# fundamentalvision/BEVFormer

Measured on NVIDIA H100. Metric: BEV queries/sec (bevformer_base 200x200x256, 6 cams) fwd+bwd, higher is better.
Workload: dtype bf16

## Files before the change

### bevformer_b200/_lib.py

```python
from __future__ import annotations

import ctypes
import os
import threading

from . import build as _build

_lock = threading.Lock()
_lib = None

c_void_p, c_int, c_int64 = ctypes.c_void_p, ctypes.c_int, ctypes.c_int64

SIGNATURES = {
    "bevf_version": (c_int, []),
    "bevf_last_error": (ctypes.c_char_p, []),
    "bevf_launch_count": (c_int64, []),
    "bevf_msda_forward": (c_int, [c_void_p, c_int, c_void_p, c_void_p, c_void_p, c_void_p,
                                  c_void_p, c_int] + [c_int] * 7 + [c_void_p]),
    "bevf_msda_backward": (c_int, [c_void_p, c_int, c_void_p, c_void_p, c_void_p, c_void_p,
                                   c_void_p, c_int, c_void_p, c_void_p, c_void_p] + [c_int] * 7
                           + [c_void_p]),
    "bevf_msda_rows_forward": (c_int, [c_void_p, c_int, c_void_p, c_void_p, c_void_p, c_void_p,
                                       c_void_p, c_int, c_void_p] + [c_int] * 7 + [c_void_p]),
    "bevf_msda_rows_backward": (c_int, [c_void_p, c_int, c_void_p, c_void_p, c_void_p, c_void_p,
                                        c_void_p, c_int, c_void_p, c_void_p, c_void_p, c_void_p]
                                + [c_int] * 7 + [c_void_p]),
    "bevf_msda_rows_backward_ordered": (c_int, [c_void_p, c_int, c_void_p, c_void_p, c_void_p, c_void_p,
                                                c_void_p, c_int, c_void_p, c_void_p, c_void_p, c_void_p,
                                                c_void_p] + [c_int] * 7 + [c_void_p]),
    "bevf_msda_set_backward_mode": (c_int, [c_int]),
    "bevf_abs_max": (c_int, [c_void_p, c_int, c_int64, c_void_p, c_void_p]),
    "bevf_msda_rows_backward_f16acc": (c_int, [c_void_p, c_int, c_void_p, c_void_p, c_void_p, c_void_p, c_void_p, c_int,
                                               c_void_p, c_void_p, c_void_p, c_void_p, c_void_p, c_void_p] + [c_int] * 7
                                       + [c_void_p]),
    "bevf_gv16_unscale": (c_int, [c_void_p, c_void_p, c_void_p, c_int64, c_void_p]),
    "bevf_msda_rows_backward_mixed": (c_int, [c_void_p, c_int, c_void_p, c_void_p, c_void_p, c_void_p, c_void_p, c_void_p,
                                              c_int, c_void_p, c_void_p, c_void_p, c_int, c_void_p, c_void_p, c_void_p,
                                              c_void_p] + [c_int] * 7 + [c_void_p]),
    "bevf_msda_rows_backward_mixed_dense": (c_int, [c_void_p, c_int, c_void_p, c_void_p, c_void_p, c_void_p, c_void_p,
                                                    c_void_p, c_int, c_void_p, c_void_p, c_void_p, c_int, c_int,
                                                    c_void_p, c_void_p, c_void_p, c_void_p] + [c_int] * 7 + [c_void_p]),
    "bevf_gv_merge": (c_int, [c_void_p, c_void_p, c_void_p, c_void_p, c_int, c_int, c_int, c_int, c_void_p]),
    "bevf_msda_fx_frac_bits": (c_int, [c_int64, c_int, c_int]),
    "bevf_msda_backward_fx": (c_int, [c_void_p, c_int, c_void_p, c_void_p, c_void_p, c_void_p, c_void_p, c_int,
                                      c_void_p, c_void_p, c_int, c_void_p, c_void_p] + [c_int] * 7 + [c_void_p]),
    "bevf_msda_rows_backward_fx": (c_int, [c_void_p, c_int, c_void_p, c_void_p, c_void_p, c_void_p, c_void_p, c_int,
                                           c_void_p, c_void_p, c_int, c_void_p, c_void_p, c_void_p] + [c_int] * 7
                                   + [c_void_p]),
    "bevf_msda_fx_convert": (c_int, [c_void_p, c_void_p, c_int, c_void_p, c_int, c_int, c_int64, c_void_p]),
    "bevf_msda_rows_backward_dense": (c_int, [c_void_p, c_int, c_void_p, c_void_p, c_void_p, c_void_p, c_void_p,
                                              c_void_p, c_int, c_void_p, c_void_p, c_void_p, c_void_p, c_void_p]
                                      + [c_int] * 7 + [c_void_p]),
    "bevf_msda_set_dense_backward": (c_int, [c_int]),
    "bevf_msda_get_dense_backward": (c_int, []),
    "bevf_msda_dense_plan": (c_int, [c_void_p, c_int, c_int, c_int, c_void_p, c_int, c_void_p]),
    "bevf_sca_plan_workspace_ints": (c_int64, [c_int, c_int]),
    "bevf_sca_plan_build": (c_int, [c_void_p] * 10 + [c_int] * 5 + [c_void_p]),
    "bevf_msda_rows_forward_staged": (c_int, [c_void_p, c_int, c_void_p, c_void_p, c_void_p, c_void_p, c_void_p,
                                              c_void_p, c_int, c_void_p] + [c_int] * 7 + [c_void_p]),
    "bevf_sca_prep_forward": (c_int, [c_void_p] * 7 + [c_int] * 8 + [c_void_p]),
    "bevf_sca_prep_backward": (c_int, [c_void_p] * 6 + [c_int] * 8 + [c_void_p]),
    "bevf_tsa_prep_forward": (c_int, [c_void_p] * 5 + [c_int] * 6 + [c_void_p]),
    "bevf_tsa_prep_backward": (c_int, [c_void_p] * 5 + [c_int] * 7 + [c_void_p]),
    "bevf_layernorm_forward": (c_int, [c_void_p] * 4 + [c_int] + [c_void_p] * 5
                               + [c_int64, c_int, ctypes.c_float, ctypes.c_float, ctypes.c_uint64, c_void_p,
                                  c_int, c_void_p]),
    "bevf_layernorm_backward": (c_int, [c_void_p] * 3 + [c_int] + [c_void_p] * 4 + [c_int64]
                                + [c_void_p] * 4
                                + [c_int64, c_int, ctypes.c_float, ctypes.c_uint64, c_void_p, c_int,
                                   c_void_p]),
    "bevf_layernorm_backward_workspace_bytes": (c_int64, [c_int64, c_int]),
    "bevf_layernorm_backward_det": (c_int, [c_void_p] * 3 + [c_int] + [c_void_p] * 4 + [c_int64]
                                    + [c_void_p] * 5 + [c_int64]
                                    + [c_int64, c_int, ctypes.c_float, ctypes.c_uint64, c_void_p, c_int,
                                       c_void_p]),
    "bevf_sca_combine_forward": (c_int, [c_void_p] * 4 + [c_int] * 6 + [c_void_p]),
    "bevf_sca_combine_backward": (c_int, [c_void_p] * 4 + [c_int] * 5 + [c_void_p]),
    "bevf_linear_forward": (c_int, [c_void_p] * 3 + [c_int] + [c_void_p] * 2
                            + [c_int, c_int64, c_int, c_int, c_int, c_void_p]),
    "bevf_flatten_feats": (c_int, [c_void_p] * 4 + [c_int] * 7 + [c_void_p]),
    "bevf_linear_dgrad": (c_int, [c_void_p] * 3 + [c_int64, c_int, c_int, c_void_p]),
    "bevf_linear_dgrad_acc": (c_int, [c_void_p] * 4 + [c_int64, c_int, c_int, c_void_p]),
    "bevf_linear_wgrad": (c_int, [c_void_p] * 4 + [c_int64, c_int, c_int, c_void_p]),
    "bevf_linear_wgrad_workspace_bytes": (c_int64, [c_int64, c_int, c_int]),
    "bevf_linear_wgrad_out": (c_int, [c_void_p] * 4 + [c_int, c_void_p, c_int64, c_int64, c_int, c_int,
                                                      c_void_p]),
    "bevf_sum_tensors": (c_int, [c_void_p, c_int, c_void_p, c_int64, c_int, c_void_p]),
    "bevf_linear_wgrad_into": (c_int, [c_void_p] * 5 + [c_int64, c_int64, c_int, c_int, c_void_p]),
    "bevf_linear_forward_dt": (c_int, [c_void_p] * 3 + [c_int] + [c_void_p] * 2
                               + [c_int, c_int64, c_int, c_int, c_int, c_int, c_void_p]),
    "bevf_linear_dgrad_dt": (c_int, [c_void_p] * 3 + [c_int64, c_int, c_int, c_int, c_void_p]),
    "bevf_linear_dgrad_acc_dt": (c_int, [c_void_p] * 4 + [c_int64, c_int, c_int, c_int, c_void_p]),
    "bevf_linear_wgrad_dt": (c_int, [c_void_p] * 4 + [c_int64, c_int, c_int, c_int, c_void_p]),
    "bevf_linear_wgrad_out_dt": (c_int, [c_void_p] * 4 + [c_int, c_void_p, c_int64, c_int64, c_int, c_int, c_int,
                                                         c_void_p]),
    "bevf_linear_wgrad_into_dt": (c_int, [c_void_p] * 5 + [c_int64, c_int64, c_int, c_int, c_int, c_void_p]),
    "bevf_colsum": (c_int, [c_void_p, c_void_p, c_int64, c_int, c_int, c_void_p]),
    "bevf_colsum_workspace_bytes": (c_int64, [c_int64, c_int]),
    "bevf_colsum_det": (c_int, [c_void_p, c_void_p, c_void_p, c_int64, c_int64, c_int, c_int, c_void_p]),
    "bevf_dropout_inplace": (c_int, [c_void_p, c_int64, ctypes.c_float, ctypes.c_uint64, c_void_p, c_int,
                                     c_void_p]),
    "bevf_relu_dropout_backward": (c_int, [c_void_p, c_void_p, c_void_p, c_int64, ctypes.c_float, c_int,
                                           c_void_p]),
    "bevf_point_sampling": (c_int, [c_void_p, c_void_p, c_void_p, ctypes.c_float, ctypes.c_float,
                                    c_void_p, c_void_p] + [c_int] * 5 + [c_void_p]),
}


def lib_path() -> str:
    return _build.LIB_PATH


def load(build_if_missing: bool = True):
    global _lib
# ... 39 lines not shown
```

### bevformer_b200/csrc/common.cuh

```cuda
#pragma once

#include <cuda_bf16.h>
#include <cuda_fp16.h>
#include <cuda_runtime.h>
#include <stdint.h>

#include <atomic>
#include <cstdio>
#include <string>

#include "../../include/bevformer_b200.h"

namespace bevf {

std::string &last_error();
extern std::atomic<int64_t> g_launches;

inline int fail(const char *fmt, const char *a = "", long long x = 0, long long y = 0) {
    char buf[512];
    snprintf(buf, sizeof(buf), fmt, a, x, y);
    last_error() = buf;
    return 1;
}

inline int check_launch(const char *what) {
    g_launches.fetch_add(1, std::memory_order_relaxed);
    cudaError_t e = cudaPeekAtLastError();
    if (e != cudaSuccess) {
        cudaGetLastError();
        char buf[512];
        snprintf(buf, sizeof(buf), "%s: launch failed: %s", what, cudaGetErrorString(e));
        last_error() = buf;
        return 2;
    }
    return 0;
}

inline bool aligned16(const void *p) { return (reinterpret_cast<uintptr_t>(p) & 15u) == 0; }

inline int device_sms() {
    static int sms = 0;
    if (sms == 0) {
        int dev = 0, n = 0;
        if (cudaGetDevice(&dev) != cudaSuccess ||
            cudaDeviceGetAttribute(&n, cudaDevAttrMultiProcessorCount, dev) != cudaSuccess || n <= 0) {
            cudaGetLastError();
            return 132;
        }
        sms = n;
    }
    return sms;
}

typedef __nv_bfloat16 bf16;

__device__ __forceinline__ float exp_rn(float x) { return (float)exp((double)x); }

__device__ __forceinline__ float bf16_lo(uint32_t u) { return __uint_as_float(u << 16); }
__device__ __forceinline__ float bf16_hi(uint32_t u) { return __uint_as_float(u & 0xffff0000u); }

__device__ __forceinline__ uint32_t pack_bf16x2(float lo, float hi) {
    uint32_t r;
    asm("cvt.rn.bf16x2.f32 %0, %1, %2;" : "=r"(r) : "f"(hi), "f"(lo));
    return r;
}

__device__ __forceinline__ float f16_lo(uint32_t u) { return __half2float(__ushort_as_half((unsigned short)(u & 0xffffu))); }
__device__ __forceinline__ float f16_hi(uint32_t u) { return __half2float(__ushort_as_half((unsigned short)(u >> 16))); }
__device__ __forceinline__ uint32_t pack_f16x2(float lo, float hi) {
    uint32_t r;
    asm("cvt.rn.f16x2.f32 %0, %1, %2;" : "=r"(r) : "f"(hi), "f"(lo));
    return r;
}

template <typename T> struct St16;
template <> struct St16<bf16> {
    __device__ static __forceinline__ float lo(uint32_t u) { return bf16_lo(u); }
    __device__ static __forceinline__ float hi(uint32_t u) { return bf16_hi(u); }
    __device__ static __forceinline__ uint32_t pack(float lo, float hi) { return pack_bf16x2(lo, hi); }
    __device__ static __forceinline__ float to_f(bf16 v) { return __bfloat162float(v); }
    __device__ static __forceinline__ bf16 from_f(float v) { return __float2bfloat16_rn(v); }
};
template <> struct St16<__half> {
    __device__ static __forceinline__ float lo(uint32_t u) { return f16_lo(u); }
    __device__ static __forceinline__ float hi(uint32_t u) { return f16_hi(u); }
    __device__ static __forceinline__ uint32_t pack(float lo, float hi) { return pack_f16x2(lo, hi); }
    __device__ static __forceinline__ float to_f(__half v) { return __half2float(v); }
    __device__ static __forceinline__ __half from_f(float v) { return __float2half_rn(v); }
};

template <typename T> struct Row;
template <> struct Row<float> {
    static constexpr int kVec = 4;
    __device__ static __forceinline__ void load(const float *p, float (&v)[4]) {
        float4 t = __ldg(reinterpret_cast<const float4 *>(p));
        v[0] = t.x; v[1] = t.y; v[2] = t.z; v[3] = t.w;
    }
    __device__ static __forceinline__ void store(float *p, const float (&v)[4]) {
        *reinterpret_cast<float4 *>(p) = make_float4(v[0], v[1], v[2], v[3]);
    }
    __device__ static __forceinline__ float load1(const float *p) { return __ldg(p); }
    __device__ static __forceinline__ void store1(float *p, float v) { *p = v; }
};
template <typename T> struct Row {
    static constexpr int kVec = 8;
    __device__ static __forceinline__ void load(const T *p, float (&v)[8]) {
        uint4 t = __ldg(reinterpret_cast<const uint4 *>(p));
        v[0] = St16<T>::lo(t.x); v[1] = St16<T>::hi(t.x); v[2] = St16<T>::lo(t.y); v[3] = St16<T>::hi(t.y);
        v[4] = St16<T>::lo(t.z); v[5] = St16<T>::hi(t.z); v[6] = St16<T>::lo(t.w); v[7] = St16<T>::hi(t.w);
// ... 72 lines not shown
```

### bevformer_b200/csrc/encoder_ops.cu

```cuda
#include <curand_kernel.h>

#include "common.cuh"

namespace bevf {

constexpr int kEThreads = 256;


__device__ __forceinline__ float warp_sum(float v) {
#pragma unroll
    for (int s = 16; s > 0; s >>= 1) v += __shfl_xor_sync(0xffffffffu, v, s);
    return v;
}

__global__ void __launch_bounds__(kEThreads)
sca_prep_fwd(const float *__restrict__ raw, const float *__restrict__ ref_cam,
             const int *__restrict__ pair_q, const int *__restrict__ pair_cam,
             const int64_t *__restrict__ level_hw, float *__restrict__ loc, float *__restrict__ attn,
             int B, int Nq, int R, int M, int L, int P, int D, int ncam) {
    const long long t = (long long)blockIdx.x * blockDim.x + threadIdx.x;
    const long long total = (long long)B * R * M;
    if (t >= total) return;
    const int m = (int)(t % M);
    const long long br = t / M;
// ... 33 lines not shown

template <typename TO>
__global__ void __launch_bounds__(kEThreads)
sca_prep_bwd(const float *__restrict__ raw, const float *__restrict__ grad_loc,
             const float *__restrict__ grad_attn, const int *__restrict__ pair_of,
             const int64_t *__restrict__ level_hw, TO *__restrict__ d_raw, int B, int Nq, int R,
             int M, int L, int P, int ncam) {
    const long long t = (long long)blockIdx.x * blockDim.x + threadIdx.x;
    const long long total = (long long)B * Nq * M;
    if (t >= total) return;
    const int m = (int)(t % M);
    const long long bq = t / M;
    const int q = (int)(bq % Nq), b = (int)(bq / Nq);
    const int LP = L * P, nout = M * LP * 3;
    const float *lg = raw + bq * nout + (long long)M * LP * 2 + (long long)m * LP;
    TO *d_off = d_raw + bq * nout + (long long)m * LP * 2;
    TO *d_lg = d_raw + bq * nout + (long long)M * LP * 2 + (long long)m * LP;
    int rows[16];
    int n = 0;
    for (int c = 0; c < ncam && c < 16; ++c) {
        const int r = pair_of[(long long)c * Nq + q];
        if (r >= 0) rows[n++] = r;
    }
    float mx = -INFINITY;
    for (int k = 0; k < LP; ++k) mx = fmaxf(mx, lg[k]);
    float sum = 0.f;
    for (int k = 0; k < LP; ++k) sum += exp_rn(lg[k] - mx);
    const float inv = __frcp_rn(sum);
    float dot = 0.f;
    for (int k = 0; k < LP; ++k) {
        float ga = 0.f;
        for (int i = 0; i < n; ++i) ga += grad_attn[(((long long)b * R + rows[i]) * M + m) * LP + k];
        dot += exp_rn(lg[k] - mx) * inv * ga;
    }
    for (int l = 0; l < L; ++l) {
        const float fw = (float)level_hw[2 * l + 1], fh = (float)level_hw[2 * l];
        for (int p = 0; p < P; ++p) {
            const int k = l * P + p;
            float ga = 0.f, gx = 0.f, gy = 0.f;
            for (int i = 0; i < n; ++i) {
                const long long s = (((long long)b * R + rows[i]) * M + m) * LP + k;
                ga += grad_attn[s];
                const float2 g2 = *reinterpret_cast<const float2 *>(grad_loc + 2 * s);
                gx += g2.x; gy += g2.y;
            }
            const float a = exp_rn(lg[k] - mx) * inv;
            st1(d_lg + k, a * (ga - dot));
            st2(d_off + 2 * k, __fdiv_rn(gx, fw), __fdiv_rn(gy, fh));
        }
    }
}


__device__ __forceinline__ float quad_max(float v) {
    v = fmaxf(v, __shfl_xor_sync(0xffffffffu, v, 1));
    return fmaxf(v, __shfl_xor_sync(0xffffffffu, v, 2));
}
__device__ __forceinline__ float quad_sum(float v) {
    v += __shfl_xor_sync(0xffffffffu, v, 1);
    return v + __shfl_xor_sync(0xffffffffu, v, 2);
}
template <int N> __device__ __forceinline__ void ldv(const float *p, float (&v)[N]) {
    if constexpr (N % 4 == 0) {
#pragma unroll
        for (int i = 0; i < N; i += 4) {
            const float4 t = __ldg(reinterpret_cast<const float4 *>(p + i));
            v[i] = t.x; v[i + 1] = t.y; v[i + 2] = t.z; v[i + 3] = t.w;
        }
    } else if constexpr (N % 2 == 0) {
#pragma unroll
        for (int i = 0; i < N; i += 2) {
            const float2 t = __ldg(reinterpret_cast<const float2 *>(p + i));
            v[i] = t.x; v[i + 1] = t.y;
        }
    } else {
#pragma unroll
        for (int i = 0; i < N; ++i) v[i] = __ldg(p + i);
    }
}
template <int N> __device__ __forceinline__ void stv(float *p, const float (&v)[N]) {
    if constexpr (N % 4 == 0) {
#pragma unroll
        for (int i = 0; i < N; i += 4) *reinterpret_cast<float4 *>(p + i) = make_float4(v[i], v[i + 1], v[i + 2], v[i + 3]);
    } else if constexpr (N % 2 == 0) {
#pragma unroll
        for (int i = 0; i < N; i += 2) *reinterpret_cast<float2 *>(p + i) = make_float2(v[i], v[i + 1]);
    } else {
#pragma unroll
        for (int i = 0; i < N; ++i) p[i] = v[i];
    }
}

template <int N, typename T> __device__ __forceinline__ void stv(T *p, const float (&v)[N]) {
    if constexpr (N % 8 == 0) {
#pragma unroll
        for (int i = 0; i < N; i += 8)
            *reinterpret_cast<uint4 *>(p + i) = make_uint4(St16<T>::pack(v[i], v[i + 1]), St16<T>::pack(v[i + 2], v[i + 3]),
                                                           St16<T>::pack(v[i + 4], v[i + 5]), St16<T>::pack(v[i + 6], v[i + 7]));
    } else if constexpr (N % 4 == 0) {
#pragma unroll
        for (int i = 0; i < N; i += 4)
            *reinterpret_cast<uint2 *>(p + i) = make_uint2(St16<T>::pack(v[i], v[i + 1]), St16<T>::pack(v[i + 2], v[i + 3]));
    } else if constexpr (N % 2 == 0) {
#pragma unroll
        for (int i = 0; i < N; i += 2) *reinterpret_cast<uint32_t *>(p + i) = St16<T>::pack(v[i], v[i + 1]);
    } else {
#pragma unroll
        for (int i = 0; i < N; ++i) p[i] = St16<T>::from_f(v[i]);
    }
}

template <int PPL>
__global__ void __launch_bounds__(kEThreads)
sca_prep_fwd_m8(const float *__restrict__ raw, const float *__restrict__ ref_cam,
                const int *__restrict__ pair_q, const int *__restrict__ pair_cam,
                const int64_t *__restrict__ level_hw, float *__restrict__ loc, float *__restrict__ attn,
                int B, int Nq, int R, int L, int P, int D, int pmagic) {
    constexpr int M = 8;
    __shared__ float s_w[16], s_h[16];
    if ((int)threadIdx.x < L) { s_h[threadIdx.x] = (float)level_hw[2 * threadIdx.x]; s_w[threadIdx.x] = (float)level_hw[2 * threadIdx.x + 1]; }
    __syncthreads();
    const int lane = threadIdx.x & 31, m = lane >> 2, sub = lane & 3;
    const long long t = (long long)blockIdx.x * (kEThreads / 32) + (threadIdx.x >> 5);
    if (t >= (long long)B * R) return;
    const int r = (int)(t % R), b = (int)(t / R);
    const int q = __ldg(pair_q + r), cam = __ldg(pair_cam + r);
    if (q < 0) return;
    const int LP = 4 * PPL, k0 = sub * PPL;
    const float *rq = raw + ((long long)b * Nq + q) * (M * LP * 3);
    float lg[PPL], off[2 * PPL];
    ldv<PPL>(rq + M * LP * 2 + m * LP + k0, lg);
    ldv<2 * PPL>(rq + (m * LP + k0) * 2, off);
    float mx = lg[0];
#pragma unroll
    for (int i = 1; i < PPL; ++i) mx = fmaxf(mx, lg[i]);
    mx = quad_max(mx);
    float sum = 0.f;
#pragma unroll
    for (int i = 0; i < PPL; ++i) { lg[i] = exp_rn(lg[i] - mx); sum += lg[i]; }
    const float inv = __frcp_rn(quad_sum(sum));
    const float *rc = ref_cam + (((long long)cam * B + b) * Nq + q) * D * 2;
#pragma unroll
    for (int i = 0; i < PPL; ++i) {
        const int k = k0 + i;
        const int l = (k * pmagic) >> 16;
        const int z = (k - l * P) % D;
        const float2 rf = __ldg(reinterpret_cast<const float2 *>(rc) + z);
        off[2 * i] = rf.x + __fdiv_rn(off[2 * i], s_w[l]);
        off[2 * i + 1] = rf.y + __fdiv_rn(off[2 * i + 1], s_h[l]);
        lg[i] *= inv;
    }
    stv<2 * PPL>(loc + ((t * M + m) * LP + k0) * 2, off);
    stv<PPL>(attn + (t * M + m) * LP + k0, lg);
}

template <int PPL, typename TO>
__global__ void __launch_bounds__(kEThreads)
sca_prep_bwd_m8(const float *__restrict__ raw, const float *__restrict__ grad_loc,
                const float *__restrict__ grad_attn, const int *__restrict__ pair_of,
                const int64_t *__restrict__ level_hw, TO *__restrict__ d_raw, int B, int Nq, int R,
                int L, int P, int ncam, int pmagic) {
    constexpr int M = 8;
    __shared__ float s_w[16], s_h[16];
    if ((int)threadIdx.x < L) { s_h[threadIdx.x] = (float)level_hw[2 * threadIdx.x]; s_w[threadIdx.x] = (float)level_hw[2 * threadIdx.x + 1]; }
    __syncthreads();
    const int lane = threadIdx.x & 31, m = lane >> 2, sub = lane & 3;
    const long long bq = (long long)blockIdx.x * (kEThreads / 32) + (threadIdx.x >> 5);
    if (bq >= (long long)B * Nq) return;
    const int q = (int)(bq % Nq), b = (int)(bq / Nq);
    const int LP = 4 * PPL, k0 = sub * PPL;
    const long long rbase = bq * (M * LP * 3);
    float a[PPL];
    ldv<PPL>(raw + rbase + M * LP * 2 + m * LP + k0, a);
    float mx = a[0];
#pragma unroll
    for (int i = 1; i < PPL; ++i) mx = fmaxf(mx, a[i]);
    mx = quad_max(mx);
    float sum = 0.f;
#pragma unroll
    for (int i = 0; i < PPL; ++i) { a[i] = exp_rn(a[i] - mx); sum += a[i]; }
    const float inv = __frcp_rn(quad_sum(sum));
    float ga[PPL], gl[2 * PPL];
#pragma unroll
    for (int i = 0; i < PPL; ++i) { ga[i] = 0.f; gl[2 * i] = 0.f; gl[2 * i + 1] = 0.f; }
    constexpr int kCamBatch = 8;
    for (int c0 = 0; c0 < ncam; c0 += kCamBatch) {
        int rid[kCamBatch];
#pragma unroll
        for (int c = 0; c < kCamBatch; ++c)
            rid[c] = (c0 + c < ncam) ? __ldg(pair_of + (long long)(c0 + c) * Nq + q) : -1;
#pragma unroll
        for (int c = 0; c < kCamBatch; ++c) {
            if (rid[c] < 0) continue;
            const long long s = (((long long)b * R + rid[c]) * M + m) * LP + k0;
            float t1[PPL], t2[2 * PPL];
            ldv<PPL>(grad_attn + s, t1);
            ldv<2 * PPL>(grad_loc + 2 * s, t2);
#pragma unroll
            for (int i = 0; i < PPL; ++i) { ga[i] += t1[i]; gl[2 * i] += t2[2 * i]; gl[2 * i + 1] += t2[2 * i + 1]; }
        }
    }
    float dot = 0.f;
#pragma unroll
    for (int i = 0; i < PPL; ++i) { a[i] *= inv; dot += a[i] * ga[i]; }
    dot = quad_sum(dot);
#pragma unroll
    for (int i = 0; i < PPL; ++i) {
        const int k = k0 + i;
        const int l = (k * pmagic) >> 16;
        ga[i] = a[i] * (ga[i] - dot);
        gl[2 * i] = __fdiv_rn(gl[2 * i], s_w[l]);
        gl[2 * i + 1] = __fdiv_rn(gl[2 * i + 1], s_h[l]);
    }
    stv<PPL>(d_raw + rbase + M * LP * 2 + m * LP + k0, ga);
    stv<2 * PPL>(d_raw + rbase + (m * LP + k0) * 2, gl);
}

template <typename T>
__global__ void __launch_bounds__(kEThreads)
colsum_kernel(const T *__restrict__ x, float *__restrict__ out, long long rows, int C, int rows_per_cta,
              float *__restrict__ part = nullptr) {
    constexpr int VEC = (sizeof(T) == 2) ? 8 : 4;
// ... 650 lines not shown
            case 2: sca_prep_fwd_m8<2><<<wgrid, kEThreads, 0, st>>>(raw, ref_cam, pair_q, pair_cam, level_hw, loc, attn, B, Nq, R, L, P, D, pmagic); break;
            case 4: sca_prep_fwd_m8<4><<<wgrid, kEThreads, 0, st>>>(raw, ref_cam, pair_q, pair_cam, level_hw, loc, attn, B, Nq, R, L, P, D, pmagic); break;
            case 8: sca_prep_fwd_m8<8><<<wgrid, kEThreads, 0, st>>>(raw, ref_cam, pair_q, pair_cam, level_hw, loc, attn, B, Nq, R, L, P, D, pmagic); break;
            default: sca_prep_fwd_m8<16><<<wgrid, kEThreads, 0, st>>>(raw, ref_cam, pair_q, pair_cam, level_hw, loc, attn, B, Nq, R, L, P, D, pmagic); break;
        }
    } else {
        sca_prep_fwd<<<blocks_for(total, kEThreads), kEThreads, 0, st>>>(
            raw, ref_cam, pair_q, pair_cam, level_hw, loc, attn, B, Nq, R, M, L, P, D, ncam);
    }
    return check_launch(who);
}

template <typename TO>
static int sca_prep_backward_t(const char *who, const float *raw, const float *grad_loc, const float *grad_attn,
                               const int32_t *pair_of, const int64_t *level_hw, TO *d_raw, int B, int Nq,
                               int R, int M, int L, int P, int ncam, cudaStream_t st) {
    const long long total = (long long)B * Nq * M;
    const int LP = L * P, pmagic = (65536 + P - 1) / P;
    const unsigned wgrid = blocks_for((long long)B * Nq, kEThreads / 32);
    if (M == 8 && L <= 16 && LP * P < 65536 && (LP == 4 || LP == 8 || LP == 16 || LP == 32 || LP == 64)) {
#define BEVF_SCA_CASE(N) sca_prep_bwd_m8<N, TO><<<wgrid, kEThreads, 0, st>>>(raw, grad_loc, grad_attn, pair_of, level_hw, d_raw, B, Nq, R, L, P, ncam, pmagic)
        switch (LP / 4) {
            case 1: BEVF_SCA_CASE(1); break;
            case 2: BEVF_SCA_CASE(2); break;
            case 4: BEVF_SCA_CASE(4); break;
            case 8: BEVF_SCA_CASE(8); break;
            default: BEVF_SCA_CASE(16); break;
        }
#undef BEVF_SCA_CASE
    } else {
        sca_prep_bwd<TO><<<blocks_for(total, kEThreads), kEThreads, 0, st>>>(
            raw, grad_loc, grad_attn, pair_of, level_hw, d_raw, B, Nq, R, M, L, P, ncam);
    }
    return check_launch(who);
}

extern "C" int bevf_sca_prep_backward(const float *raw, const float *grad_loc,
                                      const float *grad_attn, const int32_t *pair_of,
                                      const int64_t *level_hw, void *d_raw, int out_dtype, int B, int Nq,
                                      int R, int M, int L, int P, int ncam, void *stream) {
    const char *who = "bevf_sca_prep_backward";
    BEVF_REQUIRE(B >= 0 && Nq >= 0 && R >= 0 && M > 0 && L > 0 && P > 0 && ncam > 0 && ncam <= 16, who, "bad dimension (ncam <= 16)");
    BEVF_REQUIRE(out_dtype == BEVF_DTYPE_F32 || out_dtype == BEVF_DTYPE_BF16 || out_dtype == BEVF_DTYPE_F16, who, "unsupported dtype code");
    if ((long long)B * Nq * M == 0) return 0;
    BEVF_REQUIRE(raw && pair_of && level_hw && d_raw && (R == 0 || (grad_loc && grad_attn)), who, "null pointer argument");
    cudaStream_t st = (cudaStream_t)stream;
    if (out_dtype == BEVF_DTYPE_BF16)
        return sca_prep_backward_t<bf16>(who, raw, grad_loc, grad_attn, pair_of, level_hw, (bf16 *)d_raw, B, Nq, R, M, L, P, ncam, st);
    if (out_dtype == BEVF_DTYPE_F16)
        return sca_prep_backward_t<__half>(who, raw, grad_loc, grad_attn, pair_of, level_hw, (__half *)d_raw, B, Nq, R, M, L, P, ncam, st);
    return sca_prep_backward_t<float>(who, raw, grad_loc, grad_attn, pair_of, level_hw, (float *)d_raw, B, Nq, R, M, L, P, ncam, st);
}

extern "C" int bevf_tsa_prep_forward(const float *raw, const float *ref2d, const int64_t *level_hw,
                                     float *loc, float *attn, int B, int Nq, int M, int L, int P,
                                     int interleave, void *stream) {
    const char *who = "bevf_tsa_prep_forward";
    BEVF_REQUIRE(B >= 0 && Nq >= 0 && M > 0 && L > 0 && P > 0, who, "bad dimension");
    const long long total = (long long)B * Nq * M * 2;
    if (total == 0) return 0;
    BEVF_REQUIRE(raw && ref2d && level_hw && loc && attn, who, "null pointer argument");
    if (!launch_tsa_prep_m8<false, float>(raw, ref2d, nullptr, nullptr, level_hw, loc, attn, nullptr, B, Nq, M, L, P,
                                   interleave, (cudaStream_t)stream)) {
        if (interleave) return fail("%s: interleaved rows need num_heads == 8 and L*P in {2,4,8,16,32}", who);
        tsa_prep_fwd<<<blocks_for(total, kEThreads), kEThreads, 0, (cudaStream_t)stream>>>(
            raw, ref2d, level_hw, loc, attn, B, Nq, M, L, P);
    }
    return check_launch(who);
}

template <typename TO>
static int tsa_prep_backward_t(const char *who, const float *raw, const float *grad_loc, const float *grad_attn,
                               const int64_t *level_hw, TO *d_raw, int B, int Nq, int M, int L, int P,
                               int interleave, cudaStream_t st) {
    const long long total = (long long)B * Nq * M * 2;
    if (!launch_tsa_prep_m8<true, TO>(raw, nullptr, grad_loc, grad_attn, level_hw, nullptr, nullptr, d_raw, B, Nq, M,
                                      L, P, interleave, st)) {
        if (interleave) return fail("%s: interleaved rows need num_heads == 8 and L*P in {2,4,8,16,32}", who);
        tsa_prep_bwd<TO><<<blocks_for(total, kEThreads), kEThreads, 0, st>>>(
            raw, grad_loc, grad_attn, level_hw, d_raw, B, Nq, M, L, P);
    }
    return check_launch(who);
}

extern "C" int bevf_tsa_prep_backward(const float *raw, const float *grad_loc,
                                      const float *grad_attn, const int64_t *level_hw, void *d_raw,
                                      int out_dtype, int B, int Nq, int M, int L, int P, int interleave,
                                      void *stream) {
    const char *who = "bevf_tsa_prep_backward";
    BEVF_REQUIRE(B >= 0 && Nq >= 0 && M > 0 && L > 0 && P > 0, who, "bad dimension");
    BEVF_REQUIRE(out_dtype == BEVF_DTYPE_F32 || out_dtype == BEVF_DTYPE_BF16 || out_dtype == BEVF_DTYPE_F16, who, "unsupported dtype code");
    if ((long long)B * Nq * M * 2 == 0) return 0;
    BEVF_REQUIRE(raw && grad_loc && grad_attn && level_hw && d_raw, who, "null pointer argument");
    cudaStream_t st = (cudaStream_t)stream;
    if (out_dtype == BEVF_DTYPE_BF16)
        return tsa_prep_backward_t<bf16>(who, raw, grad_loc, grad_attn, level_hw, (bf16 *)d_raw, B, Nq, M, L, P, interleave, st);
    if (out_dtype == BEVF_DTYPE_F16)
        return tsa_prep_backward_t<__half>(who, raw, grad_loc, grad_attn, level_hw, (__half *)d_raw, B, Nq, M, L, P, interleave, st);
    return tsa_prep_backward_t<float>(who, raw, grad_loc, grad_attn, level_hw, (float *)d_raw, B, Nq, M, L, P, interleave, st);
}

template <typename T, typename TP>
static int ln_fwd_t(const char *who, const void *x, const void *res, const void *gamma, const void *beta,
                    const void *pos, void *y, void *y2, float *mean, float *rstd, long long rows, int C,
                    float eps, float drop_p, unsigned long long seed, const unsigned long long *sb,
                    cudaStream_t st) {
// ... 360 lines not shown
```

### bevformer_b200/csrc/msda.cu

```cuda
#include <cuda_fp16.h>

#include <cstdlib>
#include <cstring>
#include <mutex>
#include <type_traits>

#include "msda_common.cuh"

namespace bevf {

template <typename T, typename TO>
__global__ void __launch_bounds__(kThreads)
msda_fwd_d32(const T *__restrict__ value, const int64_t *__restrict__ level_hw,
             const int64_t *__restrict__ level_start, const float *__restrict__ loc,
             const float *__restrict__ attn, TO *__restrict__ out,
             const int *__restrict__ row_map, int S, int M, int Q, int L, int P, int magic,
             int iters, long long rows) {
    constexpr int VEC = Vec<T>::N, LANES = 32 / VEC, G = 32 / LANES;
    constexpr bool kHalf = std::is_same<T, bf16>::value;
    __shared__ LevelTab tab;
    load_level_tab(level_hw, level_start, L, M * 32, tab);

    const int lane = threadIdx.x & 31, warp = threadIdx.x >> 5;
    const int sub = lane % LANES, grp = lane / LANES;
    for (int it = 0; it < iters; ++it) {
    long long row = (((long long)blockIdx.x * (kThreads / 32) + warp) * iters + it) * G + grp;
    if (row - grp >= rows) break;
    bool live = row < rows;
    if (!live) row = rows - 1;
    const int m = (int)(row % M);
    int b = value_map_of(row_map, row, M, Q);
    if (b < 0) { live = false; b = 0; }
    const int pix = M * 32;
    const int LP = L * P;
    const T *vbase = value + ((long long)b * S * M + m) * 32 + sub * VEC;
    const float2 *locp = reinterpret_cast<const float2 *>(loc) + row * LP;
    const float *attp = attn + row * LP;

    float acc[VEC];
#pragma unroll
    for (int i = 0; i < VEC; ++i) acc[i] = 0.f;

    for (int s0 = 0; s0 < LP; s0 += LANES) {
        const int sm = s0 + sub;
        int enc = 0;
        float w00 = 0.f, w01 = 0.f, w10 = 0.f, w11 = 0.f;
        bool valid = false;
        if (sm < LP && live) {
            const int l = level_of(sm, magic);
            const float2 xy = __ldg(locp + sm);
            const float a = __ldg(attp + sm);
            const Corner c = make_corner(xy.x, xy.y, tab.h[l], tab.w[l]);
            enc = (c.pidx * pix) | c.dx | (c.dy << 1);
            valid = c.valid;
            w00 = c.w00 * a; w01 = c.w01 * a; w10 = c.w10 * a; w11 = c.w11 * a;
        }
        uint32_t wa = 0, wb = 0;
        if constexpr (kHalf) { wa = pack_bf16x2(w00, w01); wb = pack_bf16x2(w10, w11); }
        const unsigned vm = __ballot_sync(0xffffffffu, valid);
#pragma unroll
        for (int j = 0; j < LANES; ++j) {
            if (s0 + j >= LP) break;
            if (!(vm & (GroupMask<LANES>::kBits << j))) continue;
            const int src = grp * LANES + j;
            const unsigned e = (unsigned)__shfl_sync(0xffffffffu, enc, src);
            const int l = level_of(s0 + j, magic);
            const T *vl = vbase + tab.lofs[l];
            const unsigned o00 = e & ~3u;
            const unsigned o01 = o00 + ((e & 1u) ? (unsigned)pix : 0u);
            const unsigned oy = (e & 2u) ? (unsigned)tab.rs[l] : 0u;
            Vec<T> v00, v01, v10, v11;
            v00.load(vl + o00); v01.load(vl + o01); v10.load(vl + (o00 + oy)); v11.load(vl + (o01 + oy));
            if constexpr (kHalf) {
                const uint32_t qa = __shfl_sync(0xffffffffu, wa, src);
                const uint32_t qb = __shfl_sync(0xffffffffu, wb, src);
                unsigned short h00, h01, h10, h11;
                split16(qa, h00, h01);
                split16(qb, h10, h11);
                v00.axpy_h(h00, acc); v01.axpy_h(h01, acc); v10.axpy_h(h10, acc); v11.axpy_h(h11, acc);
            } else {
                const float q00 = __shfl_sync(0xffffffffu, w00, src);
                const float q01 = __shfl_sync(0xffffffffu, w01, src);
                const float q10 = __shfl_sync(0xffffffffu, w10, src);
                const float q11 = __shfl_sync(0xffffffffu, w11, src);
                v00.axpy(q00, acc); v01.axpy(q01, acc); v10.axpy(q10, acc); v11.axpy(q11, acc);
            }
        }
    }
    if (live) store_vec<TO, VEC>(out + row * 32 + sub * VEC, acc);
    }
}

template <typename T, typename TG, bool kScatter, typename TV = float>
__global__ void __launch_bounds__(kThreads)
msda_bwd_d32(const T *__restrict__ value, const int64_t *__restrict__ level_hw,
             const int64_t *__restrict__ level_start, const float *__restrict__ loc,
             const float *__restrict__ attn, const TG *__restrict__ grad_out,
             TV *__restrict__ grad_value, float *__restrict__ grad_loc,
             float *__restrict__ grad_attn, const int *__restrict__ row_map, int S, int M, int Q,
             int L, int P, int magic, int iters, long long rows, unsigned red_skip,
             const __grid_constant__ HostLevels host_levels, const unsigned *__restrict__ gv_amax = nullptr,
             __half *__restrict__ gv16 = nullptr, unsigned gv16_mask = 0u, int side_start = 0, int S_side = 0,
             const unsigned *__restrict__ fx_bounds = nullptr, int fx_bits = 0) {
    constexpr int VEC = Vec<T>::N, LANES = 32 / VEC, G = 32 / LANES;
    constexpr bool kHalfDot = std::is_same<T, bf16>::value && std::is_same<TG, bf16>::value;
    __shared__ LevelTab tab;
    __shared__ unsigned s_skip;
    if (threadIdx.x == 0)
        s_skip = (red_skip && host_levels.h[0] > 0 && !host_levels_match(host_levels, level_hw, level_start, L)) ? 0u : red_skip;
    __shared__ unsigned s_mask16;
    if (gv16 != nullptr && threadIdx.x == 32) {
        unsigned mk = 0;
        for (int l = 0; l < L; ++l) {
            const long long a = level_start[l], e = a + level_hw[2 * l] * level_hw[2 * l + 1];
            if (e <= side_start) mk |= 1u << l;
            else if (a < side_start) __trap();
        }
        s_mask16 = mk;
    }
    load_level_tab(level_hw, level_start, L, M * 32, tab);
    red_skip = s_skip;
    if (gv16 != nullptr) gv16_mask = s_mask16;
    const float gv_sc = gv_amax ? gv16_scale(__ldg(gv_amax)) : 1.f;
    constexpr bool kGvFx = sizeof(TV) == 8;
    double fx_sc = 0.0;
    if constexpr (kGvFx) {
        const unsigned ba = __ldg(fx_bounds), bg = __ldg(fx_bounds + 1);
        if (fx_bounds_finite(ba, bg)) fx_sc = fx_pow2(fx_bits - fx_exponent(ba, bg));
        else red_skip = ~0u;
    }

    const int lane = threadIdx.x & 31, warp = threadIdx.x >> 5;
    const int sub = lane % LANES, grp = lane / LANES;
    for (int it = 0; it < iters; ++it) {
    long long row = (((long long)blockIdx.x * (kThreads / 32) + warp) * iters + it) * G + grp;
    if (row - grp >= rows) break;
    bool live = row < rows;
    if (!live) row = rows - 1;
    const int m = (int)(row % M);
    int b = value_map_of(row_map, row, M, Q);
    if (b < 0) { live = false; b = 0; }
    const int pix = M * 32;
    const int LP = L * P;
    const long long voff = ((long long)b * S * M + m) * 32 + sub * VEC;
    const float2 *locp = reinterpret_cast<const float2 *>(loc) + row * LP;
    const float *attp = attn + row * LP;

    float g[VEC];
    load_vec<TG, VEC>(grad_out + row * 32 + sub * VEC, g);
    uint4 gh = make_uint4(0, 0, 0, 0);
    if constexpr (kHalfDot)
        gh = __ldg(reinterpret_cast<const uint4 *>(grad_out + row * 32 + sub * VEC));
    float gx[kGvFx ? VEC : 1];
    if constexpr (kGvFx) {
#pragma unroll
        for (int k = 0; k < VEC; ++k) gx[k] = Row<TG>::load1(grad_out + row * 32 + k * LANES + sub);
    }
    constexpr bool kGvHalf = sizeof(TV) == 2;
    static_assert(!kGvHalf || VEC == 8, "fp16 grad_value needs bf16 value rows (8 channels per lane)");
    constexpr bool kPaired = (VEC == 8) && kScatter && !kGvHalf && !kGvFx;
    const bool hi = kPaired && (grp & 4);
    const long long vrow = voff - sub * VEC;
    long long vrow_a = vrow, vrow_b = vrow;
    float gra[4], grb[4];
    if constexpr (!kPaired) {
        gra[0] = g[0]; gra[1] = g[1]; gra[2] = g[2]; gra[3] = g[3];
        grb[0] = grb[1] = grb[2] = grb[3] = 0.f;
        (void)vrow_a; (void)vrow_b;
    } else {
        const long long row_p = __shfl_xor_sync(0xffffffffu, row, 16);
        const long long vrow_p = __shfl_xor_sync(0xffffffffu, vrow, 16);
        const int chan = (hi ? 16 : 0) + 4 * sub;
        const long long row_a = hi ? row_p : row, row_b = hi ? row : row_p;
        vrow_a = (hi ? vrow_p : vrow) + chan;
        vrow_b = (hi ? vrow : vrow_p) + chan;
        if (gv16 != nullptr) {
            const int b_p = __shfl_xor_sync(0xffffffffu, b, 16);
            const int b_a = hi ? b_p : b, b_b = hi ? b : b_p;
            vrow_a -= ((long long)b_a * (S - S_side) + side_start) * pix;
            vrow_b -= ((long long)b_b * (S - S_side) + side_start) * pix;
        }
        load_vec<TG, 4>(grad_out + row_a * 32 + chan, gra);
        load_vec<TG, 4>(grad_out + row_b * 32 + chan, grb);
    }

    for (int s0 = 0; s0 < LP; s0 += LANES) {
        const int sm = s0 + sub;
        Corner c;
        c.x0 = c.y0 = 0;
        c.pidx = 0; c.dx = c.dy = 0; c.w00 = c.w01 = c.w10 = c.w11 = 0.f; c.lx = c.ly = 0.f;
        c.f00 = c.f01 = c.f10 = c.f11 = 0.f; c.valid = false;
        float a = 0.f;
        int Hm = 1, Wm = 1;
        const bool mine = sm < LP && live;
        if (mine) {
            const int l = level_of(sm, magic);
            Hm = tab.h[l]; Wm = tab.w[l];
            const float2 xy = __ldg(locp + sm);
            a = __ldg(attp + sm);
            c = make_corner(xy.x, xy.y, Hm, Wm);
        }
        const int enc = (c.pidx * pix) | c.dx | (c.dy << 1);
        const float wa00 = c.w00 * a, wa01 = c.w01 * a, wa10 = c.w10 * a, wa11 = c.w11 * a;
        const unsigned vm = __ballot_sync(0xffffffffu, c.valid);
        float d[LANES][4];
#pragma unroll
        for (int j = 0; j < LANES; ++j) { d[j][0] = d[j][1] = d[j][2] = d[j][3] = 0.f; }
#pragma unroll
        for (int j = 0; j < LANES; ++j) {
            if (s0 + j >= LP) break;
            if (!(vm & (GroupMask<LANES>::kBits << j))) continue;
            const int src = grp * LANES + j;
            const int e = __shfl_sync(0xffffffffu, enc, src);
            const float q00 = __shfl_sync(0xffffffffu, wa00, src);
            const float q01 = __shfl_sync(0xffffffffu, wa01, src);
            const float q10 = __shfl_sync(0xffffffffu, wa10, src);
            const float q11 = __shfl_sync(0xffffffffu, wa11, src);
            const int l = level_of(s0 + j, magic);
            const long long o00 = voff + tab.lofs[l] + (long long)((unsigned)e & ~3u);
            const int ox = (e & 1) ? pix : 0, oy = (e & 2) ? tab.rs[l] : 0;
            const T *vp = value + o00;
            Vec<T> v00, v01, v10, v11;
            v00.load(vp); v01.load(vp + ox); v10.load(vp + oy); v11.load(vp + (oy + ox));
            if constexpr (kHalfDot) {
                d[j][0] = v00.dot_h(gh); d[j][1] = v01.dot_h(gh);
                d[j][2] = v10.dot_h(gh); d[j][3] = v11.dot_h(gh);
            } else {
                d[j][0] = v00.dot(g); d[j][1] = v01.dot(g); d[j][2] = v10.dot(g); d[j][3] = v11.dot(g);
            }
            if constexpr (!kScatter) {
            } else if ((red_skip >> l) & 1u) {
            } else if constexpr (kGvFx) {
                long long *gp = reinterpret_cast<long long *>(grad_value) + (o00 - sub * VEC) + sub;
                auto redfx = [&](long long *p, float q) {
#pragma unroll
                    for (int k = 0; k < VEC; ++k) red_add_fx(p + k * LANES, q, gx[k], fx_sc);
                };
                if (q00 != 0.f) redfx(gp, q00);
                if (q01 != 0.f) redfx(gp + ox, q01);
                if (q10 != 0.f) redfx(gp + oy, q10);
                if (q11 != 0.f) redfx(gp + oy + ox, q11);
            } else if constexpr (kGvHalf) {
                TV *gp = grad_value + o00;
                auto red8 = [&](TV *p, float q) {
                    q *= gv_sc;
                    red_add_v4_f16x2(p, pack_f16x2(q * g[0], q * g[1]), pack_f16x2(q * g[2], q * g[3]),
                                     pack_f16x2(q * g[4], q * g[5]), pack_f16x2(q * g[6], q * g[7]));
                };
                if (q00 != 0.f) red8(gp, q00);
                if (q01 != 0.f) red8(gp + ox, q01);
                if (q10 != 0.f) red8(gp + oy, q10);
                if (q11 != 0.f) red8(gp + oy + ox, q11);
// ... 16 lines not shown
                if (q11 != 0.f) red8(gp + oy + ox, q11);
            } else {
                const int ep = __shfl_xor_sync(0xffffffffu, e, 16);
                const float p00 = __shfl_xor_sync(0xffffffffu, q00, 16);
                const float p01 = __shfl_xor_sync(0xffffffffu, q01, 16);
                const float p10 = __shfl_xor_sync(0xffffffffu, q10, 16);
                const float p11 = __shfl_xor_sync(0xffffffffu, q11, 16);
                const int oxp = (ep & 1) ? pix : 0, oyp = (ep & 2) ? tab.rs[l] : 0;
                {
                    const int ea = hi ? ep : e;
                    const int xa = hi ? oxp : ox, ya = hi ? oyp : oy;
                    const float a00 = hi ? p00 : q00, a01 = hi ? p01 : q01, a10 = hi ? p10 : q10,
                                a11 = hi ? p11 : q11;
                    float *gp = grad_value + vrow_a + tab.lofs[l] + (long long)((unsigned)ea & ~3u);
                    if (a00 != 0.f) red_add_v4(gp, a00 * gra[0], a00 * gra[1], a00 * gra[2], a00 * gra[3]);
                    if (a01 != 0.f) red_add_v4(gp + xa, a01 * gra[0], a01 * gra[1], a01 * gra[2], a01 * gra[3]);
                    if (a10 != 0.f) red_add_v4(gp + ya, a10 * gra[0], a10 * gra[1], a10 * gra[2], a10 * gra[3]);
                    if (a11 != 0.f) red_add_v4(gp + ya + xa, a11 * gra[0], a11 * gra[1], a11 * gra[2], a11 * gra[3]);
                }
                {
                    const int eb = hi ? e : ep;
                    const int xb = hi ? ox : oxp, yb = hi ? oy : oyp;
                    const float b00 = hi ? q00 : p00, b01 = hi ? q01 : p01, b10 = hi ? q10 : p10,
                                b11 = hi ? q11 : p11;
                    float *gp = grad_value + vrow_b + tab.lofs[l] + (long long)((unsigned)eb & ~3u);
                    if (b00 != 0.f) red_add_v4(gp, b00 * grb[0], b00 * grb[1], b00 * grb[2], b00 * grb[3]);
                    if (b01 != 0.f) red_add_v4(gp + xb, b01 * grb[0], b01 * grb[1], b01 * grb[2], b01 * grb[3]);
                    if (b10 != 0.f) red_add_v4(gp + yb, b10 * grb[0], b10 * grb[1], b10 * grb[2], b10 * grb[3]);
                    if (b11 != 0.f) red_add_v4(gp + yb + xb, b11 * grb[0], b11 * grb[1], b11 * grb[2], b11 * grb[3]);
                }
            }
        }
#pragma unroll
        for (int step = LANES / 2; step > 0; step >>= 1) {
            const bool upper = (sub & step) != 0;
#pragma unroll
            for (int j = 0; j < step; ++j) {
#pragma unroll
                for (int k = 0; k < 4; ++k) {
                    const float keep = upper ? d[j + step][k] : d[j][k];
                    const float send = upper ? d[j][k] : d[j + step][k];
                    d[j][k] = keep + __shfl_xor_sync(0xffffffffu, send, step);
                }
            }
        }
        if (mine) {
            const float hx = 1.f - c.lx, hy = 1.f - c.ly;
            const float d00 = c.f00 * d[0][0], d01 = c.f01 * d[0][1], d10 = c.f10 * d[0][2],
                        d11 = c.f11 * d[0][3];
            const float ga = hy * (hx * d00 + c.lx * d01) + c.ly * (hx * d10 + c.lx * d11);
            const float gx = a * (hy * (d01 - d00) + c.ly * (d11 - d10));
            const float gy = a * (hx * (d10 - d00) + c.lx * (d11 - d01));
            const long long si = row * LP + sm;
            grad_attn[si] = ga;
            reinterpret_cast<float2 *>(grad_loc)[si] = make_float2((float)Wm * gx, (float)Hm * gy);
        }
    }
    }
}


}
#include "msda_splat.cuh"
namespace bevf {

template <typename T, typename TO>
__global__ void __launch_bounds__(kThreads)
msda_fwd_generic(const T *__restrict__ value, const int64_t *__restrict__ level_hw,
                 const int64_t *__restrict__ level_start, const float *__restrict__ loc,
                 const float *__restrict__ attn, TO *__restrict__ out,
                 const int *__restrict__ row_map, int S, int M, int D, int Q, int L, int P,
                 long long rows) {
    __shared__ int s_h[kMaxLevels], s_w[kMaxLevels], s_start[kMaxLevels];
    load_levels(level_hw, level_start, L, s_h, s_w, s_start);
    const int lane = threadIdx.x & 31;
    const long long row = (long long)blockIdx.x * (kThreads / 32) + (threadIdx.x >> 5);
    if (row >= rows) return;
    const int m = (int)(row % M);
    const int b = value_map_of(row_map, row, M, Q);
    if (b < 0) return;
    const long long pix = (long long)M * D;
    for (int c0 = lane; c0 < D; c0 += 32) {
        float acc = 0.f;
        for (int l = 0; l < L; ++l) {
            const int H = s_h[l], W = s_w[l];
            const T *vl = value + ((long long)b * S + s_start[l]) * pix + (long long)m * D + c0;
            for (int p = 0; p < P; ++p) {
                const long long si = row * L * P + l * P + p;
                const Corner c = make_corner(loc[2 * si], loc[2 * si + 1], H, W);
                const float a = attn[si];
                const T *p00 = vl + c.pidx * pix;
                const long long ox = c.dx ? pix : 0, oy = c.dy ? W * pix : 0;
                acc += a * (c.w00 * Row<T>::load1(p00) + c.w01 * Row<T>::load1(p00 + ox) +
                            c.w10 * Row<T>::load1(p00 + oy) + c.w11 * Row<T>::load1(p00 + oy + ox));
            }
        }
        Row<TO>::store1(out + row * D + c0, acc);
    }
}

template <typename T, typename TG, typename TV = float>
__global__ void __launch_bounds__(kThreads)
msda_bwd_generic(const T *__restrict__ value, const int64_t *__restrict__ level_hw,
                 const int64_t *__restrict__ level_start, const float *__restrict__ loc,
                 const float *__restrict__ attn, const TG *__restrict__ grad_out,
                 TV *__restrict__ grad_value, float *__restrict__ grad_loc,
                 float *__restrict__ grad_attn, const int *__restrict__ row_map, int S, int M,
                 int D, int Q, int L, int P, long long rows,
                 const unsigned *__restrict__ fx_bounds = nullptr, int fx_bits = 0) {
// ... 37 lines not shown
                        if (c.w00 != 0.f) red_add_fx(grad_value + i00 + c0, c.w00 * a, gc, fx_sc);
                        if (c.w01 != 0.f) red_add_fx(grad_value + i01 + c0, c.w01 * a, gc, fx_sc);
                        if (c.w10 != 0.f) red_add_fx(grad_value + i10 + c0, c.w10 * a, gc, fx_sc);
                        if (c.w11 != 0.f) red_add_fx(grad_value + i11 + c0, c.w11 * a, gc, fx_sc);
                    }
                } else {
                    if (c.w00 != 0.f) atomicAdd(grad_value + i00 + c0, c.w00 * t);
                    if (c.w01 != 0.f) atomicAdd(grad_value + i01 + c0, c.w01 * t);
                    if (c.w10 != 0.f) atomicAdd(grad_value + i10 + c0, c.w10 * t);
                    if (c.w11 != 0.f) atomicAdd(grad_value + i11 + c0, c.w11 * t);
                }
                ga += gc * (hy * (hx * v00 + c.lx * v01) + c.ly * (hx * v10 + c.lx * v11));
                gx += t * (hy * (v01 - v00) + c.ly * (v11 - v10));
                gy += t * (hx * (v10 - v00) + c.lx * (v11 - v01));
            }
#pragma unroll
            for (int s = 16; s > 0; s >>= 1) {
                ga += __shfl_xor_sync(0xffffffffu, ga, s);
                gx += __shfl_xor_sync(0xffffffffu, gx, s);
                gy += __shfl_xor_sync(0xffffffffu, gy, s);
            }
            if (lane == 0) {
                grad_attn[si] = ga;
                grad_loc[2 * si] = (float)W * gx;
                grad_loc[2 * si + 1] = (float)H * gy;
            }
        }
    }
}

static int pick_iters(long long rows, int G) {
    static int forced = -1;
    if (forced < 0) {
        const char *e = getenv("BEVF_MSDA_ITERS");
        forced = e ? atoi(e) : 0;
    }
    (void)rows; (void)G;
    return forced > 0 ? forced : 1;
}

static int check_dims(const char *who, int B, int S, int M, int D, int Q, int L, int P) {
    if (B < 0 || S < 0 || M <= 0 || D <= 0 || Q < 0 || L <= 0 || P <= 0)
        return fail("%s: negative or zero dimension", who);
    if (L > kMaxLevels) return fail("%s: at most 16 levels are supported (got %lld)", who, L);
    if ((long long)S * M * D >= (1ll << 31))
        return fail("%s: one batch item of value exceeds 2^31 elements", who);
    if ((long long)L * P * P >= 65536) return fail("%s: num_levels * num_points^2 must be < 65536", who);
    return 0;
}

template <typename T, typename TO>
static int launch_fwd(const char *who, const void *value, const int64_t *hw, const int64_t *ls,
                      const float *loc, const float *attn, void *out, const int *row_map, int S,
                      int M, int D, int Q, int L, int P, long long rows, cudaStream_t st) {
    if (D == 32) {
        constexpr int G = Vec<T>::N;
        const int iters = pick_iters(rows, G);
        const long long per_block = (long long)(kThreads / 32) * G * iters;
        const unsigned grid = (unsigned)((rows + per_block - 1) / per_block);
        msda_fwd_d32<T, TO><<<grid, kThreads, 0, st>>>((const T *)value, hw, ls, loc, attn, (TO *)out,
                                                       row_map, S, M, Q, L, P, (65536 + P - 1) / P, iters,
                                                       rows);
    } else {
        const unsigned grid = (unsigned)((rows + kThreads / 32 - 1) / (kThreads / 32));
        msda_fwd_generic<T, TO><<<grid, kThreads, 0, st>>>((const T *)value, hw, ls, loc, attn,
                                                           (TO *)out, row_map, S, M, D, Q, L, P, rows);
    }
    return check_launch(who);
}

static std::atomic<int> g_bwd_mode{-1};
static int bwd_split_enabled() {
    int v = g_bwd_mode.load(std::memory_order_relaxed);
    if (v < 0) {
        const char *e = getenv("BEVF_MSDA_BWD");
        v = (e && e[0] == 's') ? 1 : 0;
        g_bwd_mode.store(v, std::memory_order_relaxed);
    }
    return v;
}
static unsigned splat_direct_mask() {
    static long v = -1;
    if (v < 0) {
        const char *e = getenv("BEVF_SPLAT_DIRECT");
        v = e ? strtol(e, nullptr, 0) : 0;
    }
    return (unsigned)v;
}

int dense_coarse_backward(const char *who, const int64_t *hw_dev, const int64_t *ls_dev, const int32_t *hw_host,
                          const float *loc, const float *attn, const void *grad_out, float *grad_value,
                          const int32_t *map_range, int NB, int S, int M, int L, int P, cudaStream_t st,
                          unsigned *handled, HostLevels *host_levels, int first_level, unsigned need_mask,
                          int gv_S, int gv_base);

static cudaStream_t g_side_stream = nullptr;
constexpr int kSideEvents = 64;
static cudaEvent_t g_side_events[kSideEvents];
static std::atomic<unsigned> g_side_ev_next{0};

template <typename TG, int kM>
static int launch_splat_km(const char *who, const float *loc, const float *attn, const void *go, float *gv,
                           const int *row_map, const int *order, const int64_t *hw, const int64_t *ls,
                           int S, int M, int Q, int L, int P, long long pairs, unsigned level_mask,
                           cudaStream_t st) {
    static bool attr_done = false;
    if (!attr_done) {
        if (cudaFuncSetAttribute(msda_bwd_splat_d32<TG, kM>, cudaFuncAttributeMaxDynamicSharedMemorySize,
                                 (int)splat_smem_bytes(kSplatMaxHeads, sizeof(TG))) != cudaSuccess) {
            cudaGetLastError();
            return fail("%s: cannot reserve shared memory for the splat kernel", who);
        }
        attr_done = true;
    }
    const unsigned grid = (unsigned)((pairs + kSplatG - 1) / kSplatG);
    msda_bwd_splat_d32<TG, kM><<<grid, 32 * M, splat_smem_bytes(M, sizeof(TG)), st>>>(
        loc, attn, (const TG *)go, gv, row_map, order, hw, ls, S, M, Q, L, P, pairs, splat_direct_mask(),
        level_mask);
    return check_launch(who);
}

template <typename TG>
static int launch_splat(const char *who, const float *loc, const float *attn, const void *go, float *gv,
                        const int *row_map, const int *order, const int64_t *hw, const int64_t *ls,
                        int S, int M, int Q, int L, int P, long long pairs, unsigned level_mask,
                        cudaStream_t st) {
    if constexpr (std::is_same<TG, __half>::value) {
        return fail("%s: the splat kernel takes fp32 or bf16 grad_out", who);
    } else {
        if (M == 8)
            return launch_splat_km<TG, 8>(who, loc, attn, go, gv, row_map, order, hw, ls, S, M, Q, L, P, pairs,
                                          level_mask, st);
        return launch_splat_km<TG, 0>(who, loc, attn, go, gv, row_map, order, hw, ls, S, M, Q, L, P, pairs,
                                      level_mask, st);
    }
}

struct MixedGv {
    const unsigned *amax = nullptr;
    __half *gv16 = nullptr;
    unsigned mask = 0;
    int side_start = 0, S_side = 0;
};

struct FxGv {
    const unsigned *bounds = nullptr;
    int frac_bits = 0;
};

template <typename T, typename TG>
static int launch_bwd(const char *who, const void *value, const int64_t *hw, const int64_t *ls,
                      const float *loc, const float *attn, const void *go, float *gv, float *gl,
                      float *ga, const int *row_map, const int *order, int S, int M, int D, int Q,
                      int L, int P, long long rows, cudaStream_t st, unsigned done_levels = 0,
                      const HostLevels *host_levels = nullptr, bool gv_f16 = false,
                      const MixedGv *mixed = nullptr, const FxGv *fx = nullptr) {
    HostLevels hl;
    if (host_levels) hl = *host_levels; else memset(&hl, 0, sizeof(hl));
    if (fx) {
        long long *gfx = reinterpret_cast<long long *>(gv);
        if (D == 32) {
            constexpr int G = Vec<T>::N;
            const int iters = pick_iters(rows, G);
            const long long per_block = (long long)(kThreads / 32) * G * iters;
            const unsigned grid = (unsigned)((rows + per_block - 1) / per_block);
            msda_bwd_d32<T, TG, true, long long><<<grid, kThreads, 0, st>>>(
                (const T *)value, hw, ls, loc, attn, (const TG *)go, gfx, gl, ga, row_map, S, M, Q, L, P,
                (65536 + P - 1) / P, iters, rows, 0u, hl, nullptr, nullptr, 0u, 0, 0, fx->bounds, fx->frac_bits);
        } else {
            const unsigned grid = (unsigned)((rows + kThreads / 32 - 1) / (kThreads / 32));
            msda_bwd_generic<T, TG, long long><<<grid, kThreads, 0, st>>>(
                (const T *)value, hw, ls, loc, attn, (const TG *)go, gfx, gl, ga, row_map, S, M, D, Q, L, P, rows,
                fx->bounds, fx->frac_bits);
        }
        return check_launch(who);
    }
    if (gv_f16) {
        if constexpr (std::is_same<T, bf16>::value) {
            if (D != 32) return fail("%s: fp16 grad_value needs head_dim 32", who);
            constexpr int G = Vec<T>::N;
            const int iters = pick_iters(rows, G);
            const long long per_block = (long long)(kThreads / 32) * G * iters;
            const unsigned grid = (unsigned)((rows + per_block - 1) / per_block);
            msda_bwd_d32<T, TG, true, __half><<<grid, kThreads, 0, st>>>((const T *)value, hw, ls, loc, attn, (const TG *)go,
                                                                       reinterpret_cast<__half *>(gv), gl, ga, row_map, S, M,
                                                                       Q, L, P, (65536 + P - 1) / P, iters, rows, 0u, hl,
                                                                       mixed ? mixed->amax : nullptr);
            return check_launch(who);
        } else {
            return fail("%s: fp16 grad_value needs a bf16 value tensor", who);
        }
    }
    if (mixed && mixed->gv16) {
        if constexpr (std::is_same<T, bf16>::value) {
            if (D != 32) return fail("%s: mixed accumulation needs head_dim 32", who);
            constexpr int G = Vec<T>::N;
            const int iters = pick_iters(rows, G);
            const long long per_block = (long long)(kThreads / 32) * G * iters;
            const unsigned grid = (unsigned)((rows + per_block - 1) / per_block);
            msda_bwd_d32<T, TG, true><<<grid, kThreads, 0, st>>>((const T *)value, hw, ls, loc, attn, (const TG *)go, gv, gl, ga,
                                                               row_map, S, M, Q, L, P, (65536 + P - 1) / P, iters, rows,
                                                               done_levels, hl, mixed->amax, mixed->gv16, mixed->mask, mixed->side_start,
                                                               mixed->S_side);
            return check_launch(who);
        } else {
            return fail("%s: mixed accumulation needs a bf16 value tensor", who);
        }
    }
    if (D == 32) {
        constexpr int G = Vec<T>::N;
        const int iters = pick_iters(rows, G);
        const long long per_block = (long long)(kThreads / 32) * G * iters;
        const unsigned grid = (unsigned)((rows + per_block - 1) / per_block);
        const int mode = done_levels ? 0 : bwd_split_enabled();
        if (mode != 0 && std::is_same<T, __half>::value)
            return fail("%s: the split / hybrid backward modes take fp32 or bf16 only (fp16 needs mode 0)", who);
        const bool can_split = M <= kSplatMaxHeads && S * (long long)M * 32 < (1ll << 31);
        if (mode == 1 && can_split) {
            if (int e = launch_splat<TG>(who, loc, attn, go, gv, row_map, order, hw, ls, S, M, Q, L, P,
                                         rows / M, 0xffffffffu, st))
                return e;
            msda_bwd_d32<T, TG, false><<<grid, kThreads, 0, st>>>((const T *)value, hw, ls, loc, attn,
                                                                  (const TG *)go, gv, gl, ga, row_map, S, M,
                                                                  Q, L, P, (65536 + P - 1) / P, iters, rows, 0u, hl);
        } else if (mode == 2 && can_split && L >= 2 && g_side_stream) {
            unsigned coarse = 0;
            for (int l = L / 2; l < L; ++l) coarse |= 1u << l;
            cudaEvent_t fork = g_side_events[g_side_ev_next.fetch_add(1) % kSideEvents];
            cudaEvent_t join = g_side_events[g_side_ev_next.fetch_add(1) % kSideEvents];
            cudaEventRecord(fork, st);
            cudaStreamWaitEvent(g_side_stream, fork, 0);
            if (int e = launch_splat<TG>(who, loc, attn, go, gv, row_map, order, hw, ls, S, M, Q, L, P,
                                         rows / M, coarse, g_side_stream))
                return e;
            cudaEventRecord(join, g_side_stream);
            msda_bwd_d32<T, TG, true><<<grid, kThreads, 0, st>>>((const T *)value, hw, ls, loc, attn,
                                                                 (const TG *)go, gv, gl, ga, row_map, S, M,
                                                                 Q, L, P, (65536 + P - 1) / P, iters, rows, coarse, hl);
            cudaStreamWaitEvent(st, join, 0);
        } else {
            msda_bwd_d32<T, TG, true><<<grid, kThreads, 0, st>>>((const T *)value, hw, ls, loc, attn,
                                                                 (const TG *)go, gv, gl, ga, row_map, S, M,
                                                                 Q, L, P, (65536 + P - 1) / P, iters, rows, done_levels, hl);
        }
    } else {
        const unsigned grid = (unsigned)((rows + kThreads / 32 - 1) / (kThreads / 32));
        msda_bwd_generic<T, TG><<<grid, kThreads, 0, st>>>((const T *)value, hw, ls, loc, attn,
                                                           (const TG *)go, gv, gl, ga, row_map, S, M,
                                                           D, Q, L, P, rows);
    }
    return check_launch(who);
}

static int msda_forward_impl(const char *who, const void *value, int value_dtype,
                             const int64_t *level_hw, const int64_t *level_start, const float *loc,
                             const float *attn, void *out, int out_dtype, const int *row_map, int B,
                             int S, int M, int D, int Q, int L, int P, void *stream) {
    if (int e = check_dims(who, B, S, M, D, Q, L, P)) return e;
    const long long rows = (row_map ? 1ll : (long long)B) * Q * M;
    if (rows == 0) return 0;
    if (!value || !level_hw || !level_start || !loc || !attn || !out)
        return fail("%s: null pointer argument", who);
    if (!aligned16(value) || !aligned16(loc) || !aligned16(attn) || !aligned16(out))
        return fail("%s: device pointers must be 16-byte aligned", who);
    cudaStream_t st = (cudaStream_t)stream;
    if (value_dtype == BEVF_DTYPE_F16) {
        if (out_dtype == BEVF_DTYPE_F16) return launch_fwd<__half, __half>(who, value, level_hw, level_start, loc, attn, out, row_map, S, M, D, Q, L, P, rows, st);
        if (out_dtype == BEVF_DTYPE_F32) return launch_fwd<__half, float>(who, value, level_hw, level_start, loc, attn, out, row_map, S, M, D, Q, L, P, rows, st);
        return fail("%s: fp16 value needs an fp16 or fp32 output", who);
    }
    const bool vb = value_dtype == BEVF_DTYPE_BF16, ob = out_dtype == BEVF_DTYPE_BF16;
    if ((value_dtype != BEVF_DTYPE_F32 && !vb) || (out_dtype != BEVF_DTYPE_F32 && !ob))
        return fail("%s: unsupported dtype code", who);
    if (!vb && !ob) return launch_fwd<float, float>(who, value, level_hw, level_start, loc, attn, out, row_map, S, M, D, Q, L, P, rows, st);
    if (vb && ob) return launch_fwd<bf16, bf16>(who, value, level_hw, level_start, loc, attn, out, row_map, S, M, D, Q, L, P, rows, st);
    if (vb && !ob) return launch_fwd<bf16, float>(who, value, level_hw, level_start, loc, attn, out, row_map, S, M, D, Q, L, P, rows, st);
    return fail("%s: fp32 value with bf16 output is not supported", who);
}

static int msda_backward_impl(const char *who, const void *value, int value_dtype,
                              const int64_t *level_hw, const int64_t *level_start, const float *loc,
                              const float *attn, const void *grad_out, int grad_out_dtype,
                              float *grad_value, float *grad_loc, float *grad_attn,
                              const int *row_map, const int *order, int B, int S, int M, int D, int Q,
                              int L, int P, void *stream, unsigned done_levels = 0,
                              const HostLevels *host_levels = nullptr, bool gv_f16 = false,
                              const MixedGv *mixed = nullptr, const FxGv *fx = nullptr) {
    if (int e = check_dims(who, B, S, M, D, Q, L, P)) return e;
    const long long rows = (row_map ? 1ll : (long long)B) * Q * M;
    if (rows == 0) return 0;
    if (!value || !level_hw || !level_start || !loc || !attn || !grad_out || !grad_value ||
        !grad_loc || !grad_attn)
        return fail("%s: null pointer argument", who);
    if (!aligned16(value) || !aligned16(loc) || !aligned16(attn) || !aligned16(grad_out) ||
        !aligned16(grad_value) || !aligned16(grad_loc) || !aligned16(grad_attn))
        return fail("%s: device pointers must be 16-byte aligned", who);
    cudaStream_t st = (cudaStream_t)stream;
    if (value_dtype == BEVF_DTYPE_F16) {
        if (grad_out_dtype == BEVF_DTYPE_F16) return launch_bwd<__half, __half>(who, value, level_hw, level_start, loc, attn, grad_out, grad_value, grad_loc, grad_attn, row_map, order, S, M, D, Q, L, P, rows, st, done_levels, host_levels, gv_f16, mixed, fx);
        if (grad_out_dtype == BEVF_DTYPE_F32) return launch_bwd<__half, float>(who, value, level_hw, level_start, loc, attn, grad_out, grad_value, grad_loc, grad_attn, row_map, order, S, M, D, Q, L, P, rows, st, done_levels, host_levels, gv_f16, mixed, fx);
        return fail("%s: fp16 value needs an fp16 or fp32 grad_out", who);
    }
    const bool vb = value_dtype == BEVF_DTYPE_BF16, gb = grad_out_dtype == BEVF_DTYPE_BF16;
    if ((value_dtype != BEVF_DTYPE_F32 && !vb) || (grad_out_dtype != BEVF_DTYPE_F32 && !gb))
        return fail("%s: unsupported dtype code", who);
    if (!vb && !gb) return launch_bwd<float, float>(who, value, level_hw, level_start, loc, attn, grad_out, grad_value, grad_loc, grad_attn, row_map, order, S, M, D, Q, L, P, rows, st, done_levels, host_levels, gv_f16, mixed, fx);
    if (vb && gb) return launch_bwd<bf16, bf16>(who, value, level_hw, level_start, loc, attn, grad_out, grad_value, grad_loc, grad_attn, row_map, order, S, M, D, Q, L, P, rows, st, done_levels, host_levels, gv_f16, mixed, fx);
    if (vb && !gb) return launch_bwd<bf16, float>(who, value, level_hw, level_start, loc, attn, grad_out, grad_value, grad_loc, grad_attn, row_map, order, S, M, D, Q, L, P, rows, st, done_levels, host_levels, gv_f16, mixed, fx);
    return fail("%s: fp32 value with bf16 grad_out is not supported", who);
}

}

using namespace bevf;

extern "C" int bevf_msda_forward(const void *value, int value_dtype, const int64_t *level_hw,
                                 const int64_t *level_start, const float *loc, const float *attn,
                                 void *out, int out_dtype, int B, int S, int M, int D, int Q, int L,
                                 int P, void *stream) {
    return msda_forward_impl("bevf_msda_forward", value, value_dtype, level_hw, level_start, loc,
                             attn, out, out_dtype, nullptr, B, S, M, D, Q, L, P, stream);
}

extern "C" int bevf_msda_backward(const void *value, int value_dtype, const int64_t *level_hw,
                                  const int64_t *level_start, const float *loc, const float *attn,
                                  const void *grad_out, int grad_out_dtype, float *grad_value,
                                  float *grad_loc, float *grad_attn, int B, int S, int M, int D,
                                  int Q, int L, int P, void *stream) {
    return msda_backward_impl("bevf_msda_backward", value, value_dtype, level_hw, level_start, loc,
                              attn, grad_out, grad_out_dtype, grad_value, grad_loc, grad_attn,
                              nullptr, nullptr, B, S, M, D, Q, L, P, stream);
}

extern "C" int bevf_msda_rows_forward(const void *value, int value_dtype, const int64_t *level_hw,
                                      const int64_t *level_start, const float *loc,
                                      const float *attn, void *out, int out_dtype,
                                      const int32_t *row_map, int B, int S, int M, int D, int R,
                                      int L, int P, void *stream) {
    if (!row_map && R > 0) return fail("%s: row_map is null", "bevf_msda_rows_forward");
    return msda_forward_impl("bevf_msda_rows_forward", value, value_dtype, level_hw, level_start,
                             loc, attn, out, out_dtype, row_map, B, S, M, D, R, L, P, stream);
}

extern "C" int bevf_msda_rows_backward(const void *value, int value_dtype, const int64_t *level_hw,
                                       const int64_t *level_start, const float *loc,
                                       const float *attn, const void *grad_out, int grad_out_dtype,
                                       float *grad_value, float *grad_loc, float *grad_attn,
                                       const int32_t *row_map, int B, int S, int M, int D, int R,
                                       int L, int P, void *stream) {
    if (!row_map && R > 0) return fail("%s: row_map is null", "bevf_msda_rows_backward");
// ... 28 lines not shown
    cudaStream_t s = nullptr;
    if (cudaStreamCreateWithFlags(&s, cudaStreamNonBlocking) != cudaSuccess) {
        cudaGetLastError();
        return fail("%s: cannot create the second stream", who);
    }
    for (int i = 0; i < kSideEvents; ++i) cudaEventCreateWithFlags(&g_side_events[i], cudaEventDisableTiming);
    g_side_stream = s;
    return 0;
}

extern "C" int bevf_msda_set_dense_backward(int mode) {
    if (mode < -1 || mode > 2)
        return fail("%s: mode must be -1 (library default), 0 (off), 1 (same stream) or 2 (second stream)",
                    "bevf_msda_set_dense_backward");
    if (mode == 2)
        if (int e = ensure_side_stream("bevf_msda_set_dense_backward")) return e;
    g_dense_mode.store(mode, std::memory_order_relaxed);
    return 0;
}

extern "C" int bevf_msda_get_dense_backward(void) { return mixed_dense_mode(); }

extern "C" int bevf_msda_rows_backward_dense(const void *value, int value_dtype, const int64_t *level_hw,
                                             const int64_t *level_start, const int32_t *level_hw_host,
                                             const float *loc, const float *attn, const void *grad_out,
                                             int grad_out_dtype, float *grad_value, float *grad_loc,
                                             float *grad_attn, const int32_t *row_map, const int32_t *map_range,
                                             int B, int S, int M, int D, int R, int L, int P, void *stream) {
    const char *who = "bevf_msda_rows_backward_dense";
    if (!row_map && R > 0) return fail("%s: row_map is null", who);
    if (int e = check_dims(who, B, S, M, D, R, L, P)) return e;
    if (R == 0) return 0;
    if (!level_hw_host || !map_range || !level_hw || !level_start || !loc || !attn || !grad_out || !grad_value)
        return fail("%s: null pointer argument", who);
    cudaStream_t st = (cudaStream_t)stream;
    unsigned handled = 0;
    HostLevels hl;
    memset(&hl, 0, sizeof(hl));
    const int mode = dense_setting() < 0 ? 0 : dense_setting();
    cudaEvent_t join = nullptr;
    if (value_dtype == BEVF_DTYPE_F16 || grad_out_dtype == BEVF_DTYPE_F16)
        return fail("%s: fp32 or bf16 only (fp16 runs on bevf_msda_rows_backward)", who);
    if (mode != 0 && D == 32 && grad_out_dtype == BEVF_DTYPE_BF16 && aligned16(loc) && aligned16(attn) &&
        aligned16(grad_out) && aligned16(grad_value)) {
        cudaStream_t ds = st;
        if (mode == 2 && g_side_stream) {
            cudaEvent_t fork = g_side_events[g_side_ev_next.fetch_add(1) % kSideEvents];
            join = g_side_events[g_side_ev_next.fetch_add(1) % kSideEvents];
            cudaEventRecord(fork, st);
            cudaStreamWaitEvent(g_side_stream, fork, 0);
            ds = g_side_stream;
        }
        const int e = dense_coarse_backward(who, level_hw, level_start, level_hw_host, loc, attn, grad_out, grad_value,
                                            map_range, B, S, M, L, P, ds, &handled, &hl, 0, 0u, S, 0);
        if (join) cudaEventRecord(join, g_side_stream);
        if (e) {
            if (join) cudaStreamWaitEvent(st, join, 0);
            return e;
        }
    }
    const int e = msda_backward_impl(who, value, value_dtype, level_hw, level_start, loc, attn, grad_out,
                                     grad_out_dtype, grad_value, grad_loc, grad_attn, row_map, nullptr, B, S, M, D,
                                     R, L, P, stream, handled, &hl);
    if (join) cudaStreamWaitEvent(st, join, 0);
    return e;
}

extern "C" int bevf_msda_rows_backward_f16acc(const void *value, int value_dtype, const int64_t *level_hw,
                                              const int64_t *level_start, const float *loc, const float *attn,
                                              const void *grad_out, int grad_out_dtype, void *grad_value_f16,
                                              const uint32_t *amax_bits, float *grad_loc, float *grad_attn,
                                              const int32_t *row_map, const int32_t *group_order, int B, int S,
                                              int M, int D, int R, int L, int P, void *stream) {
    const char *who = "bevf_msda_rows_backward_f16acc";
    if (!row_map && R > 0) return fail("%s: row_map is null", who);
    if (!grad_value_f16 || !amax_bits) return fail("%s: null pointer argument", who);
    MixedGv mx;
    mx.amax = amax_bits;
    return msda_backward_impl(who, value, value_dtype, level_hw, level_start, loc, attn, grad_out, grad_out_dtype,
                              reinterpret_cast<float *>(grad_value_f16), grad_loc, grad_attn, row_map, group_order, B, S,
                              M, D, R, L, P, stream, 0u, nullptr, true, &mx);
}

static int rows_backward_mixed_impl(const char *who, const void *value, int value_dtype, const int64_t *level_hw,
                                    const int64_t *level_start, const int32_t *level_hw_host, const float *loc,
                                    const float *attn, const void *grad_out, int grad_out_dtype,
                                    void *grad_value_fine_f16, float *grad_value_side, const uint32_t *amax_bits,
                                    int num_f16_levels, int first_dense_level, float *grad_loc, float *grad_attn,
                                    const int32_t *row_map, const int32_t *group_order, const int32_t *map_range,
                                    int B, int S, int M, int D, int R, int L, int P, void *stream) {
    if (!row_map && R > 0) return fail("%s: row_map is null", who);
    if (!level_hw_host || !grad_value_fine_f16 || !grad_value_side || !amax_bits)
        return fail("%s: null pointer argument", who);
    if (L <= 1 || L > kMaxLevels || num_f16_levels < 1 || num_f16_levels >= L)
        return fail("%s: num_f16_levels must be in [1, L - 1]", who);
    if (map_range && (first_dense_level < num_f16_levels || first_dense_level >= L))
        return fail("%s: first_dense_level must be in [num_f16_levels, L - 1]", who);
    if (value_dtype != BEVF_DTYPE_BF16 || D != 32) return fail("%s: needs a bf16 value tensor and head_dim 32", who);
    if (!aligned16(grad_value_fine_f16) || !aligned16(grad_value_side))
        return fail("%s: device pointers must be 16-byte aligned", who);
    HostLevels hl;
    memset(&hl, 0, sizeof(hl));
    long long start = 0;
    for (int l = 0; l < L; ++l) {
        const int h = level_hw_host[2 * l], w = level_hw_host[2 * l + 1];
        if (h <= 0 || w <= 0 || h >= 32768 || w >= 32768) return fail("%s: bad host level shape", who);
        hl.h[l] = h; hl.w[l] = w; hl.start[l] = (int)start;
        start += (long long)h * w;
    }
    if (start != S) return fail("%s: host level shapes do not add up to S (%lld vs %lld)", who, start, S);
    MixedGv mx;
    mx.amax = amax_bits;
    mx.gv16 = reinterpret_cast<__half *>(grad_value_fine_f16);
    mx.mask = (1u << num_f16_levels) - 1u;
    mx.side_start = hl.start[num_f16_levels];
    mx.S_side = S - mx.side_start;
    cudaStream_t st = (cudaStream_t)stream;
    unsigned dense_levels = 0;
    cudaEvent_t join = nullptr;
    const int mode = map_range ? mixed_dense_mode() : 0;
    if (mode != 0 && R > 0 && grad_out_dtype == BEVF_DTYPE_BF16 && aligned16(loc) && aligned16(attn) &&
        aligned16(grad_out)) {
        cudaStream_t ds = st;
        if (mode == 2 && !g_side_stream) {
            cudaStreamCaptureStatus cs = cudaStreamCaptureStatusActive;
            if (cudaStreamIsCapturing(st, &cs) != cudaSuccess) cudaGetLastError();
            else if (cs == cudaStreamCaptureStatusNone && ensure_side_stream(who) != 0) cudaGetLastError();
        }
        if (mode == 2 && g_side_stream) {
            cudaEvent_t fork = g_side_events[g_side_ev_next.fetch_add(1) % kSideEvents];
            join = g_side_events[g_side_ev_next.fetch_add(1) % kSideEvents];
            cudaEventRecord(fork, st);
            cudaStreamWaitEvent(g_side_stream, fork, 0);
            ds = g_side_stream;
        }
        const unsigned suffix = ((1u << L) - 1u) & ~((1u << first_dense_level) - 1u);
        HostLevels dhl;
        const int e = dense_coarse_backward(who, level_hw, level_start, level_hw_host, loc, attn, grad_out,
                                            grad_value_side, map_range, B, S, M, L, P, ds, &dense_levels, &dhl,
                                            first_dense_level, suffix, mx.S_side, mx.side_start);
        if (join) cudaEventRecord(join, g_side_stream);
        if (e) {
            if (join) cudaStreamWaitEvent(st, join, 0);
            return e;
        }
    }
    const int e = msda_backward_impl(who, value, value_dtype, level_hw, level_start, loc, attn, grad_out, grad_out_dtype,
                                     grad_value_side, grad_loc, grad_attn, row_map, group_order, B, S, M, D, R, L, P,
                                     stream, dense_levels, &hl, false, &mx);
    if (join) cudaStreamWaitEvent(st, join, 0);
    return e;
}

extern "C" int bevf_msda_rows_backward_mixed(const void *value, int value_dtype, const int64_t *level_hw,
                                             const int64_t *level_start, const int32_t *level_hw_host,
                                             const float *loc, const float *attn, const void *grad_out,
                                             int grad_out_dtype, void *grad_value_fine_f16, float *grad_value_side,
                                             const uint32_t *amax_bits, int num_f16_levels, float *grad_loc,
                                             float *grad_attn, const int32_t *row_map, const int32_t *group_order,
                                             int B, int S, int M, int D, int R, int L, int P, void *stream) {
    return rows_backward_mixed_impl("bevf_msda_rows_backward_mixed", value, value_dtype, level_hw, level_start,
                                    level_hw_host, loc, attn, grad_out, grad_out_dtype, grad_value_fine_f16,
                                    grad_value_side, amax_bits, num_f16_levels, L, grad_loc, grad_attn, row_map,
                                    group_order, nullptr, B, S, M, D, R, L, P, stream);
}

extern "C" int bevf_msda_rows_backward_mixed_dense(const void *value, int value_dtype, const int64_t *level_hw,
                                                   const int64_t *level_start, const int32_t *level_hw_host,
                                                   const float *loc, const float *attn, const void *grad_out,
                                                   int grad_out_dtype, void *grad_value_fine_f16,
                                                   float *grad_value_side, const uint32_t *amax_bits,
                                                   int num_f16_levels, int first_dense_level, float *grad_loc,
                                                   float *grad_attn, const int32_t *row_map, const int32_t *map_range,
                                                   int B, int S, int M, int D, int R, int L, int P, void *stream) {
    const char *who = "bevf_msda_rows_backward_mixed_dense";
    if (!map_range) return fail("%s: null pointer argument", who);
    return rows_backward_mixed_impl(who, value, value_dtype, level_hw, level_start, level_hw_host, loc, attn, grad_out,
                                    grad_out_dtype, grad_value_fine_f16, grad_value_side, amax_bits, num_f16_levels,
                                    first_dense_level, grad_loc, grad_attn, row_map, nullptr, map_range, B, S, M, D, R,
                                    L, P, stream);
}

namespace bevf {
int fx_bounds_launch(const char *who, const float *attn, const void *grad_out, int grad_out_dtype,
                     const int32_t *row_map, long long qrows, int M, int D, int L, int P, uint32_t *bounds,
                     cudaStream_t st);

static int msda_backward_fx_impl(const char *who, const void *value, int value_dtype, const int64_t *level_hw,
                                 const int64_t *level_start, const float *loc, const float *attn, const void *grad_out,
                                 int grad_out_dtype, int64_t *grad_value_fx, uint32_t *bounds, int frac_bits,
                                 float *grad_loc, float *grad_attn, const int32_t *row_map, int B, int S, int M, int D,
                                 int Q, int L, int P, void *stream) {
    if (int e = check_dims(who, B, S, M, D, Q, L, P)) return e;
    const long long qrows = (row_map ? 1ll : (long long)B) * Q;
    if (qrows == 0) return 0;
    if (!bounds || !grad_value_fx || !attn || !grad_out) return fail("%s: null pointer argument", who);
    const int kmax = bevf_msda_fx_frac_bits(Q, L, P);
    if (frac_bits < 0 || frac_bits > kmax)
        return fail("%s: frac_bits must be in [0, %lld] for this launch (bevf_msda_fx_frac_bits)", who, kmax);
    cudaStream_t st = (cudaStream_t)stream;
    if (int e = fx_bounds_launch(who, attn, grad_out, grad_out_dtype, row_map, qrows, M, D, L, P, bounds, st)) return e;
    FxGv fx;
    fx.bounds = bounds;
    fx.frac_bits = frac_bits;
    return msda_backward_impl(who, value, value_dtype, level_hw, level_start, loc, attn, grad_out, grad_out_dtype,
                              reinterpret_cast<float *>(grad_value_fx), grad_loc, grad_attn, row_map, nullptr, B, S, M,
                              D, Q, L, P, stream, 0u, nullptr, false, nullptr, &fx);
}
}

extern "C" int bevf_msda_backward_fx(const void *value, int value_dtype, const int64_t *level_hw,
                                     const int64_t *level_start, const float *loc, const float *attn,
                                     const void *grad_out, int grad_out_dtype, int64_t *grad_value_fx,
                                     uint32_t *bounds, int frac_bits, float *grad_loc, float *grad_attn, int B, int S,
                                     int M, int D, int Q, int L, int P, void *stream) {
    return msda_backward_fx_impl("bevf_msda_backward_fx", value, value_dtype, level_hw, level_start, loc, attn, grad_out,
                                 grad_out_dtype, grad_value_fx, bounds, frac_bits, grad_loc, grad_attn, nullptr, B, S, M,
                                 D, Q, L, P, stream);
}

extern "C" int bevf_msda_rows_backward_fx(const void *value, int value_dtype, const int64_t *level_hw,
                                          const int64_t *level_start, const float *loc, const float *attn,
                                          const void *grad_out, int grad_out_dtype, int64_t *grad_value_fx,
                                          uint32_t *bounds, int frac_bits, float *grad_loc, float *grad_attn,
                                          const int32_t *row_map, int B, int S, int M, int D, int R, int L, int P,
                                          void *stream) {
    if (!row_map && R > 0) return fail("%s: row_map is null", "bevf_msda_rows_backward_fx");
    return msda_backward_fx_impl("bevf_msda_rows_backward_fx", value, value_dtype, level_hw, level_start, loc, attn,
                                 grad_out, grad_out_dtype, grad_value_fx, bounds, frac_bits, grad_loc, grad_attn, row_map,
                                 B, S, M, D, R, L, P, stream);
}

extern "C" int bevf_msda_set_backward_mode(int mode) {
// ... 27 lines not shown
```

### bevformer_b200/csrc/msda_common.cuh

```cuda
#pragma once

#include "common.cuh"

namespace bevf {

constexpr int kMaxLevels = 16;
constexpr int kThreads = 256;

struct Corner {
    int x0, y0;
    int pidx;
    int dx, dy;
    float w00, w01, w10, w11;
    float lx, ly;
    float f00, f01, f10, f11;
    bool valid;
};

__device__ __forceinline__ Corner make_corner(float locx, float locy, int H, int W) {
    Corner c;
    float x = __fadd_rn(__fmul_rn(locx, (float)W), -0.5f), y = __fadd_rn(__fmul_rn(locy, (float)H), -0.5f);
    c.valid = (x > -1.f) && (y > -1.f) && (x < (float)W) && (y < (float)H);
    if (!c.valid) { x = 0.f; y = 0.f; }
    const float xf = floorf(x), yf = floorf(y);
// ... 99 lines not shown
            d = fhfma(lo, glo, d);
            d = fhfma(hi, ghi, d);
        }
        return d;
    }
    __device__ __forceinline__ float dot(const float (&g)[8]) const {
        const uint32_t u[4] = {v.x, v.y, v.z, v.w};
        float d = 0.f;
#pragma unroll
        for (int i = 0; i < 4; ++i) {
            d = fmaf(g[2 * i], bf16_lo(u[i]), d);
            d = fmaf(g[2 * i + 1], bf16_hi(u[i]), d);
        }
        return d;
    }
};

template <> struct Vec<__half> {
    uint4 v;
    static constexpr int N = 8;
    __device__ __forceinline__ void load(const __half *p) { v = __ldg(reinterpret_cast<const uint4 *>(p)); }
    __device__ __forceinline__ void axpy(float w, float (&acc)[8]) const {
        const uint32_t u[4] = {v.x, v.y, v.z, v.w};
#pragma unroll
        for (int i = 0; i < 4; ++i) {
            acc[2 * i] = fmaf(w, f16_lo(u[i]), acc[2 * i]);
            acc[2 * i + 1] = fmaf(w, f16_hi(u[i]), acc[2 * i + 1]);
        }
    }
    __device__ __forceinline__ float dot(const float (&g)[8]) const {
        const uint32_t u[4] = {v.x, v.y, v.z, v.w};
        float d = 0.f;
#pragma unroll
        for (int i = 0; i < 4; ++i) {
            d = fmaf(g[2 * i], f16_lo(u[i]), d);
            d = fmaf(g[2 * i + 1], f16_hi(u[i]), d);
        }
        return d;
    }
};

template <int LANES> struct GroupMask;
template <> struct GroupMask<4> { static constexpr unsigned kBits = 0x11111111u; };
template <> struct GroupMask<8> { static constexpr unsigned kBits = 0x01010101u; };
template <> struct GroupMask<16> { static constexpr unsigned kBits = 0x00010001u; };

__device__ __forceinline__ int level_of(int s, int magic) { return (s * magic) >> 16; }

__device__ __forceinline__ int value_map_of(const int *row_map, long long row, int M, int Q) {
    return row_map ? __ldg(row_map + row / M) : (int)(row / ((long long)M * Q));
}


template <typename T> __device__ __forceinline__ decltype(Vec<T>::v) vec_bits(const uint4 &u);
template <> __device__ __forceinline__ uint4 vec_bits<bf16>(const uint4 &u) { return u; }
template <> __device__ __forceinline__ float4 vec_bits<float>(const uint4 &u) {
    return make_float4(__uint_as_float(u.x), __uint_as_float(u.y), __uint_as_float(u.z), __uint_as_float(u.w));
}

}
```

### bevformer_b200/csrc/msda_dense.cu

```cuda
#include <cuda.h>

#include <cstdlib>
#include <cstring>
#include <mutex>

#include "msda_common.cuh"

namespace bevf {

constexpr int kDnK = 16;
constexpr int kDnMaxBins = 32;
constexpr int kDnBinLevels = 4;
constexpr int kDnTileBytes = 128 * kDnK * 2;
constexpr int kDnTransposeBytes = 16 * 144;

struct DenseBins {
    int nbins, L;
    int s0[kDnMaxBins], n[kDnMaxBins];
    int nlev[kDnMaxBins];
    int lev[kDnMaxBins][kDnBinLevels];
    HostLevels hl;
};

namespace dn {
// ... 31 lines not shown
    return d;
}
__device__ __forceinline__ void wgmma_m64n32_amn(float (&d)[16], uint64_t da, uint64_t db) {
    asm volatile("wgmma.mma_async.sync.aligned.m64n32k16.f32.bf16.bf16 "
                 "{%0, %1, %2, %3, %4, %5, %6, %7, %8, %9, %10, %11, %12, %13, %14, %15}, %16, %17, 1, 1, 1, 1, 0;\n"
                 : "+f"(d[0]), "+f"(d[1]), "+f"(d[2]), "+f"(d[3]), "+f"(d[4]), "+f"(d[5]), "+f"(d[6]), "+f"(d[7]),
                   "+f"(d[8]), "+f"(d[9]), "+f"(d[10]), "+f"(d[11]), "+f"(d[12]), "+f"(d[13]), "+f"(d[14]), "+f"(d[15])
                 : "l"(da), "l"(db));
}
template <int N> __device__ __forceinline__ void fence_regs(float (&d)[N]) {
#pragma unroll
    for (int i = 0; i < N; ++i) asm volatile("" : "+f"(d[i])::"memory");
}

__device__ __forceinline__ uint32_t slab_off(int row, int k) {
    return ((uint32_t)(row >> 6) << 11) + ((uint32_t)k << 7) + ((((uint32_t)(row >> 3) & 7u) ^ ((uint32_t)k & 7u)) << 4) +
           (((uint32_t)row & 7u) << 1);
}
__device__ __forceinline__ float2 ldg_f2(const float2 *p) {
    float2 v;
    asm volatile("ld.global.nc.v2.f32 {%0, %1}, [%2];" : "=f"(v.x), "=f"(v.y) : "l"(p));
    return v;
}
__device__ __forceinline__ float ldg_f1(const float *p) {
    float v;
    asm volatile("ld.global.nc.f32 %0, [%1];" : "=f"(v) : "l"(p));
    return v;
}
__device__ __forceinline__ uint4 ldg_u4(const uint4 *p) {
    uint4 v;
    asm volatile("ld.global.nc.v4.u32 {%0, %1, %2, %3}, [%4];" : "=r"(v.x), "=r"(v.y), "=r"(v.z), "=r"(v.w) : "l"(p));
    return v;
}
__device__ __forceinline__ unsigned short lds16(uint32_t addr) {
    unsigned short h;
    asm volatile("ld.shared.u16 %0, [%1];" : "=h"(h) : "r"(addr) : "memory");
    return h;
}
__device__ __forceinline__ void sts16(uint32_t addr, unsigned short h) {
    asm volatile("st.shared.u16 [%0], %1;" ::"r"(addr), "h"(h) : "memory");
}
__device__ __forceinline__ unsigned short bf16_add(unsigned short old, float x) {
    const float v = __uint_as_float((uint32_t)old << 16) + x;
    return __bfloat16_as_ushort(__float2bfloat16_rn(v));
}
}

template <int kTiles, int P, int NT>
__global__ void __launch_bounds__(128 * NT + 256, 1)
msda_bwd_dense_tc(const __grid_constant__ DenseBins bins, const int64_t *__restrict__ level_hw,
                  const int64_t *__restrict__ level_start, const float *__restrict__ loc,
                  const float *__restrict__ attn, const bf16 *__restrict__ grad_out,
                  float *__restrict__ grad_value, const int *__restrict__ map_range, int NB, int gv_S, int gv_base,
                  int M, int L, int chunk_rows, int dbg) {
    static_assert(P == 4 || P == 8, "points per level: 4 or 8");
    static_assert(kTiles == 4, "accumulator tiles per bin: 2 per issuer warpgroup");
    static_assert(NT >= 1 && NT <= 3, "scatter teams");
    constexpr int kThreadsAll = 128 * NT + 256;
    constexpr int kSlabBytes = kTiles * kDnTileBytes;
    constexpr int kMine = kTiles / 2;
    constexpr int kColsPerWarp = 32 / P;
    constexpr int kWarpsPerLevel = kDnK / kColsPerWarp;
    constexpr int kLevelsPerPass = 4 / kWarpsPerLevel;
    constexpr int kMaxPass = kDnBinLevels / kLevelsPerPass;
    extern __shared__ __align__(1024) uint8_t smem_raw[];
    uint8_t *smem = reinterpret_cast<uint8_t *>((reinterpret_cast<uintptr_t>(smem_raw) + 1023) & ~uintptr_t(1023));
    uint8_t *slab = smem;
    uint8_t *gtile = smem + NT * kSlabBytes;
    float *tr = reinterpret_cast<float *>(gtile + NT * 4096);
    uint64_t *bar_full = reinterpret_cast<uint64_t *>(reinterpret_cast<uint8_t *>(tr) + 8 * kDnTransposeBytes);
    uint64_t *bar_empty = bar_full + NT;
    uint32_t *s_dirty = reinterpret_cast<uint32_t *>(bar_empty + NT);
    __shared__ int s_h[kMaxLevels], s_w[kMaxLevels], s_start[kMaxLevels];
    __shared__ int s_bad;

    const int tid = threadIdx.x, lane = tid & 31;
    const int team = tid >> 7, tt = tid & 127, tw = tt >> 5;
    const bool is_team = team < NT;

    if (tid == 0) s_bad = 0;
    __syncthreads();
    if (tid < L) {
        s_h[tid] = (int)level_hw[2 * tid];
        s_w[tid] = (int)level_hw[2 * tid + 1];
        s_start[tid] = (int)level_start[tid];
    }
    if (tid == 64 && !host_levels_match(bins.hl, level_hw, level_start, L)) s_bad = 1;
    if (tid == 32) {
        for (int i = 0; i < NT; ++i) { dn::mbar_init(&bar_full[i], 128); dn::mbar_init(&bar_empty[i], 8); }
        asm volatile("fence.mbarrier_init.release.cluster;" ::: "memory");
        for (int i = 0; i < 2 * NT; ++i) s_dirty[i] = 0;
    }
    {
        uint4 *z = reinterpret_cast<uint4 *>(smem);
        const int n16 = (NT * kSlabBytes + NT * 4096) / 16;
        for (int i = tid; i < n16; i += kThreadsAll) z[i] = make_uint4(0, 0, 0, 0);
    }
    __syncthreads();
    if (s_bad) return;
    dn::fence_async_smem();
    __syncthreads();

    const int per_chunk = M * bins.nbins;
    int total = 0;
    for (int b = 0; b < NB; ++b) {
        const int n = __ldg(map_range + 2 * b + 1) - __ldg(map_range + 2 * b);
        total += ((n + chunk_rows - 1) / chunk_rows) * per_chunk;
// ... 1 lines not shown

    const int k = (tw % kWarpsPerLevel) * kColsPerWarp + lane / P, pt = lane % P, lsub = tw / kWarpsPerLevel;
    const uint32_t my_slab = dn::s32(slab + (is_team ? team : 0) * kSlabBytes) + ((uint32_t)k << 7);
    const uint32_t kx = (uint32_t)k & 7u;
    const uint32_t my_gt = dn::s32(gtile + (is_team ? team : 0) * 4096);
    const bool g_role = is_team && tt < 64;
    const int gk = tt & 15, gc = (tt >> 4) & 3;
    uint32_t nuse = 0;
    uint32_t nfull[NT];
#pragma unroll
    for (int i = 0; i < NT; ++i) nfull[i] = 0;
    float acc[kMine][2][16];
    auto unit_bar = [] { asm volatile("bar.sync 1, %0;" ::"n"(kThreadsAll) : "memory"); };

    auto row_off = [&](int row) -> uint32_t {
        return ((uint32_t)(row >> 6) << 11) + ((((uint32_t)(row >> 3) & 7u) ^ kx) << 4) + (((uint32_t)row & 7u) << 1);
    };

    for (int u = blockIdx.x; u < total; u += gridDim.x) {
        int b = 0, rem = u, ps = 0, pe = 0;
        for (; b < NB; ++b) {
            ps = __ldg(map_range + 2 * b); pe = __ldg(map_range + 2 * b + 1);
            const int cnt = ((pe - ps + chunk_rows - 1) / chunk_rows) * per_chunk;
            if (rem < cnt) break;
            rem -= cnt;
        }
        const int chunk = rem / per_chunk, rem2 = rem - chunk * per_chunk;
        const int m = rem2 / bins.nbins, bin = rem2 - m * bins.nbins;
        const int r_begin = ps + chunk * chunk_rows, r_end = min(pe, r_begin + chunk_rows);
        const int nsteps = (r_end - r_begin + kDnK - 1) / kDnK;
        const int s0 = bins.s0[bin], nb = bins.n[bin];

        if (is_team) {
            const int nlev = bins.nlev[bin];
            int lv[kMaxPass], Hq[kMaxPass], Wq[kMaxPass], lb[kMaxPass];
            bool on[kMaxPass];
            uint32_t rec_a[kMaxPass], rec_b[kMaxPass];
#pragma unroll
            for (int q = 0; q < kMaxPass; ++q) {
                const int slot = q * kLevelsPerPass + lsub;
                on[q] = slot < nlev;
                lv[q] = on[q] ? bins.lev[bin][slot] : 0;
                Hq[q] = s_h[lv[q]]; Wq[q] = s_w[lv[q]]; lb[q] = s_start[lv[q]] - s0;
                rec_a[q] = rec_b[q] = 0;
            }
            struct Smp { float x, y, a; };
            auto load_samples = [&](int step, Smp (&q)[kMaxPass]) {
                const int r = r_begin + step * kDnK + k;
                const bool live = step < nsteps && r < r_end;
#pragma unroll
                for (int i = 0; i < kMaxPass; ++i) {
                    q[i].x = q[i].y = q[i].a = 0.f;
                    if (live && on[i]) {
                        const long long e = (((long long)r * M + m) * L + lv[i]) * P + pt;
                        const float2 xy = dn::ldg_f2(reinterpret_cast<const float2 *>(loc) + e);
                        q[i].x = xy.x; q[i].y = xy.y; q[i].a = dn::ldg_f1(attn + e);
                    }
                }
            };
            auto load_gout = [&](int step) -> uint4 {
                const int r = r_begin + step * kDnK + gk;
                if (g_role && step < nsteps && r < r_end)
                    return dn::ldg_u4(reinterpret_cast<const uint4 *>(grad_out + ((long long)r * M + m) * 32 + gc * 8));
                return make_uint4(0, 0, 0, 0);
            };
            auto unscatter = [&]() {
#pragma unroll
                for (int q = 0; q < kMaxPass; ++q) {
                    const uint32_t ra = rec_a[q], rb = rec_b[q];
                    if ((ra | rb) != 0) {
                        if (ra & 0x8000u) dn::sts16(my_slab + ((ra & 0x7fffu) << 1), 0);
                        if (ra & 0x80000000u) dn::sts16(my_slab + (((ra >> 16) & 0x7fffu) << 1), 0);
                        if (rb & 0x8000u) dn::sts16(my_slab + ((rb & 0x7fffu) << 1), 0);
                        if (rb & 0x80000000u) dn::sts16(my_slab + (((rb >> 16) & 0x7fffu) << 1), 0);
                        rec_a[q] = rec_b[q] = 0;
                    }
                }
            };
            auto corner_round = [&](bool act, uint32_t off, float cf, int row, uint32_t &dirty) -> uint32_t {
                const uint32_t key = act ? (my_slab + off) : (0xffffff00u | (uint32_t)lane);
                const unsigned peers = __match_any_sync(0xffffffffu, key);
                float sum = cf;
                if (__any_sync(0xffffffffu, (peers & (peers - 1u)) != 0u)) {
                    sum = 0.f;
                    unsigned rem_set = peers;
                    while (__any_sync(0xffffffffu, rem_set != 0u)) {
                        const int src = rem_set ? (__ffs(rem_set) - 1) : lane;
                        const float t = __shfl_sync(0xffffffffu, cf, src);
                        if (rem_set) { sum += t; rem_set &= rem_set - 1u; }
                    }
                }
                if (act && lane == __ffs(peers) - 1) {
                    dn::sts16(key, dn::bf16_add(dn::lds16(key), sum));
                    dirty |= 1u << (row >> 7);
                    return (off >> 1) | 0x8000u;
                }
                return 0u;
            };
            auto scatter = [&](const Smp (&q)[kMaxPass]) -> uint32_t {
                uint32_t dirty = 0;
#pragma unroll
                for (int i = 0; i < kMaxPass; ++i) {
                    if (i * kLevelsPerPass >= nlev) break;
                    const int H = Hq[i], W = Wq[i], lbase = lb[i];
                    bool p00 = false, p01 = false, p10 = false, p11 = false;
                    int r00 = 0, r01 = 0, r10 = 0, r11 = 0;
                    float c00 = 0.f, c01 = 0.f, c10 = 0.f, c11 = 0.f;
// ... 140 lines not shown
}

namespace bevf {

static long dense_env(const char *name, long dflt) {
    const char *e = getenv(name);
    return e ? strtol(e, nullptr, 0) : dflt;
}

static int plan_dense_bins(const int32_t *hw_host, int L, long max_pix, int cap, DenseBins &bins, long long *total,
                           int first = 0) {
    memset(&bins, 0, sizeof(bins));
    bins.L = L;
    long long start = 0;
    unsigned mask = 0;
    int open = -1;
    for (int l = 0; l < L; ++l) {
        const int h = hw_host[2 * l], w = hw_host[2 * l + 1];
        if (h <= 0 || w <= 0 || h >= 32768 || w >= 32768) return -1;
        const long long n = (long long)h * w;
        bins.hl.h[l] = h; bins.hl.w[l] = w; bins.hl.start[l] = (int)start;
        if (l >= first && n <= max_pix) {
            if (n <= cap && open >= 0 && bins.n[open] + n <= cap && bins.nlev[open] < kDnBinLevels) {
                bins.lev[open][bins.nlev[open]++] = l;
                bins.n[open] += (int)n;
            } else {
                const int parts = (int)((n + cap - 1) / cap);
                if (bins.nbins + parts > kDnMaxBins) return -2;
                long long off = 0;
                for (int i = 0; i < parts; ++i) {
                    const int bi = bins.nbins++;
                    bins.s0[bi] = (int)(start + off);
                    bins.n[bi] = (int)((n - off) < cap ? (n - off) : cap);
                    bins.nlev[bi] = 1;
                    bins.lev[bi][0] = l;
                    off += bins.n[bi];
                }
                open = bins.nbins - 1;
            }
            mask |= 1u << l;
        } else {
            open = -1;
        }
        start += n;
    }
    *total = start;
    return (int)mask;
}

int dense_coarse_backward(const char *who, const int64_t *hw_dev, const int64_t *ls_dev, const int32_t *hw_host,
                          const float *loc, const float *attn, const void *grad_out, float *grad_value,
                          const int32_t *map_range, int NB, int S, int M, int L, int P, cudaStream_t st,
                          unsigned *handled, HostLevels *host_levels, int first_level, unsigned need_mask,
                          int gv_S, int gv_base) {
    *handled = 0;
    static const long max_pix = dense_env("BEVF_DENSE_MAXPIX", 8192);
    static const long tiles = dense_env("BEVF_DENSE_TILES", 4);
    static const long chunk = dense_env("BEVF_DENSE_CHUNK", 512);
    if ((P != 4 && P != 8) || L > kMaxLevels || NB <= 0 || max_pix <= 0) return 0;
    if (tiles != 4) return fail("%s: BEVF_DENSE_TILES must be 4", who);
    if (chunk < kDnK || chunk % kDnK) return fail("%s: BEVF_DENSE_CHUNK must be a positive multiple of 16", who);
    const int cap = (int)tiles * 128;
    DenseBins bins;
    long long start = 0;
    const int pm = plan_dense_bins(hw_host, L, max_pix, cap, bins, &start, first_level);
    if (pm == -1) return fail("%s: bad host level shape", who);
    if (pm == -2) return 0;
    const unsigned mask = (unsigned)pm;
    if (start != S) return fail("%s: host level shapes do not add up to S (%lld vs %lld)", who, start, S);
    if (mask == 0 || (need_mask != 0 && mask != need_mask)) return 0;
    static int sms = 0;
    if (sms == 0) {
        int dev = 0;
        cudaGetDevice(&dev);
        cudaDeviceGetAttribute(&sms, cudaDevAttrMultiProcessorCount, dev);
    }
    static const long teams_env = dense_env("BEVF_DENSE_TEAMS", 0);
    const int teams = teams_env > 0 ? (int)teams_env : 3;
    const size_t smem = 1024 + (size_t)teams * ((size_t)tiles * kDnTileBytes + 4096) + 8 * kDnTransposeBytes + 256;
    static const long dbg = dense_env("BEVF_DENSE_DEBUG", 0);
    auto launch = [&](auto kern) -> int {
        static const void *configured[16];
        static int nconfigured = 0;
        static std::mutex mu;
        {
            std::lock_guard<std::mutex> lock(mu);
            bool seen = false;
            for (int i = 0; i < nconfigured; ++i) seen = seen || configured[i] == (const void *)kern;
            if (!seen) {
                if (cudaFuncSetAttribute(kern, cudaFuncAttributeMaxDynamicSharedMemorySize, (int)smem) != cudaSuccess) {
                    cudaGetLastError();
                    return fail("%s: cannot reserve shared memory for the dense backward", who);
                }
                if (nconfigured < 16) configured[nconfigured++] = (const void *)kern;
            }
        }
        kern<<<(unsigned)sms, 128 * teams + 256, smem, st>>>(bins, hw_dev, ls_dev, loc, attn, (const bf16 *)grad_out,
                                                           grad_value, map_range, NB, gv_S, gv_base, M, L, (int)chunk,
                                                           (int)dbg);
        return check_launch(who);
    };
    int e;
    if (teams == 3) e = (P == 8) ? launch(msda_bwd_dense_tc<4, 8, 3>) : launch(msda_bwd_dense_tc<4, 4, 3>);
    else if (teams == 2) e = (P == 8) ? launch(msda_bwd_dense_tc<4, 8, 2>) : launch(msda_bwd_dense_tc<4, 4, 2>);
    else if (teams == 1) e = (P == 8) ? launch(msda_bwd_dense_tc<4, 8, 1>) : launch(msda_bwd_dense_tc<4, 4, 1>);
    else return fail("%s: BEVF_DENSE_TEAMS must be 1, 2 or 3", who);
    if (e) return e;
    *handled = mask;
    *host_levels = bins.hl;
    return 0;
}

}

extern "C" int bevf_msda_dense_plan(const int32_t *level_hw_host, int L, int max_pix, int tiles, int32_t *bins_out,
                                    int bins_cap, uint32_t *level_mask) {
    using namespace bevf;
    const char *who = "bevf_msda_dense_plan";
    if (!level_hw_host || !bins_out || !level_mask || L <= 0 || L > kMaxLevels || (tiles != 4 && tiles != 8 && tiles != 16))
        return -fail("%s: bad argument", who);
    DenseBins bins;
    long long total = 0;
    const int pm = plan_dense_bins(level_hw_host, L, max_pix, tiles * 128, bins, &total);
    if (pm == -1) return -fail("%s: bad host level shape", who);
    if (pm == -2) { *level_mask = 0; return 0; }
    if (bins.nbins > bins_cap) return -fail("%s: output too small", who);
    for (int i = 0; i < bins.nbins; ++i) {
        int32_t *o = bins_out + i * (3 + kDnBinLevels);
        o[0] = bins.s0[i]; o[1] = bins.n[i]; o[2] = bins.nlev[i];
        for (int j = 0; j < kDnBinLevels; ++j) o[3 + j] = j < bins.nlev[i] ? bins.lev[i][j] : -1;
    }
    *level_mask = (unsigned)pm;
    return bins.nbins;
}
```

### bevformer_b200/ops.py

```python
from __future__ import annotations

import os
import warnings

import torch
from torch.autograd.function import Function, once_differentiable

from . import _lib

F32, BF16, F16 = 0, 1, 2
_DT = {torch.float32: F32, torch.bfloat16: BF16, torch.float16: F16}
TC_DTYPES = (torch.bfloat16, torch.float16)


def deterministic() -> bool:
    return torch.are_deterministic_algorithms_enabled()


def alert_not_deterministic(name: str) -> None:
    if not torch.are_deterministic_algorithms_enabled():
        return
    msg = (f"{name} does not have a deterministic implementation, but you set "
           "'torch.use_deterministic_algorithms(True)'.")
    if torch.is_deterministic_algorithms_warn_only_enabled():
# ... 544 lines not shown
                                                          ctx.group_order, lazy=True)
            if ctx.value_early is not None and ctx.value_early(gv):
                return None, gl, ga, None, None, None, None, None, None
            return gv.materialize(), gl, ga, None, None, None, None, None, None
        gv, gl, ga = msda_rows_backward(value, ss, ls, loc, attn, row_map, grad_out.contiguous(), gv0,
                                        group_order=ctx.group_order, dense=ctx.dense)
        if ctx.value_early is not None and ctx.value_early(gv):
            return None, gl, ga, None, None, None, None, None, None
        return gv.to(value.dtype), gl, ga, None, None, None, None, None, None


def sca_prep_forward(raw, ref_cam, pair_q, pair_cam, level_hw, B, Nq, M, L, P):
    _need_cuda(raw, "raw")
    R, D, ncam = pair_q.numel(), ref_cam.shape[3], ref_cam.shape[0]
    loc = torch.empty((B * R, M, L, P, 2), device=raw.device, dtype=torch.float32)
    attn = torch.empty((B * R, M, L, P), device=raw.device, dtype=torch.float32)
    lib = _lib.load()
    with torch.cuda.device(raw.device):
        st = lib.bevf_sca_prep_forward(raw.data_ptr(), ref_cam.data_ptr(), pair_q.data_ptr(),
                                       pair_cam.data_ptr(), level_hw.data_ptr(), loc.data_ptr(),
                                       attn.data_ptr(), B, Nq, R, M, L, P, D, ncam, _stream_ptr(raw))
    _lib.check(st, lib)
    return loc, attn


def sca_prep_backward(raw, grad_loc, grad_attn, pair_of, level_hw, B, Nq, R, M, L, P,
                      out_dtype=torch.float32):
    ncam = pair_of.shape[0]
    d_raw = torch.empty(raw.shape, device=raw.device, dtype=out_dtype)
    lib = _lib.load()
    with torch.cuda.device(raw.device):
        st = lib.bevf_sca_prep_backward(raw.data_ptr(), grad_loc.data_ptr(), grad_attn.data_ptr(),
                                        pair_of.data_ptr(), level_hw.data_ptr(), d_raw.data_ptr(),
                                        _DT[out_dtype], B, Nq, R, M, L, P, ncam, _stream_ptr(raw))
    _lib.check(st, lib)
    return d_raw


class ScaPrep(Function):
    @staticmethod
    def forward(ctx, raw, ref_cam, pair_q, pair_cam, pair_of, level_hw, B, Nq, M, L, P):
        loc, attn = sca_prep_forward(raw, ref_cam, pair_q, pair_cam, level_hw, B, Nq, M, L, P)
        ctx.save_for_backward(raw, pair_of, level_hw)
        ctx.dims = (B, Nq, pair_q.numel(), M, L, P)
        return loc, attn

    @staticmethod
    @once_differentiable
    def backward(ctx, grad_loc, grad_attn):
        raw, pair_of, level_hw = ctx.saved_tensors
        d_raw = sca_prep_backward(raw, grad_loc.contiguous(), grad_attn.contiguous(), pair_of,
                                  level_hw, *ctx.dims)
        return (d_raw,) + (None,) * 10


def tsa_prep_forward(raw, ref2d, level_hw, B, Nq, M, L, P, interleave=False):
    _need_cuda(raw, "raw")
    shape = (B * Nq * 2, M, L, P) if interleave else (B * 2, Nq, M, L, P)
    loc = torch.empty(shape + (2,), device=raw.device, dtype=torch.float32)
    attn = torch.empty(shape, device=raw.device, dtype=torch.float32)
    lib = _lib.load()
    with torch.cuda.device(raw.device):
        st = lib.bevf_tsa_prep_forward(raw.data_ptr(), ref2d.data_ptr(), level_hw.data_ptr(),
                                       loc.data_ptr(), attn.data_ptr(), B, Nq, M, L, P,
                                       int(interleave), _stream_ptr(raw))
    _lib.check(st, lib)
    return loc, attn


def tsa_prep_backward(raw, grad_loc, grad_attn, level_hw, B, Nq, M, L, P, interleave=0,
                      out_dtype=torch.float32):
    d_raw = torch.empty(raw.shape, device=raw.device, dtype=out_dtype)
    lib = _lib.load()
    with torch.cuda.device(raw.device):
        st = lib.bevf_tsa_prep_backward(raw.data_ptr(), grad_loc.contiguous().data_ptr(),
                                        grad_attn.contiguous().data_ptr(), level_hw.data_ptr(),
                                        d_raw.data_ptr(), _DT[out_dtype], B, Nq, M, L, P,
                                        int(interleave), _stream_ptr(raw))
    _lib.check(st, lib)
    return d_raw


class TsaPrep(Function):
    @staticmethod
    def forward(ctx, raw, ref2d, level_hw, B, Nq, M, L, P, interleave=False):
        loc, attn = tsa_prep_forward(raw, ref2d, level_hw, B, Nq, M, L, P, interleave)
        ctx.save_for_backward(raw, level_hw)
        ctx.dims = (B, Nq, M, L, P, int(interleave))
        return loc, attn

    @staticmethod
    @once_differentiable
    def backward(ctx, grad_loc, grad_attn):
        raw, level_hw = ctx.saved_tensors
        d_raw = tsa_prep_backward(raw, grad_loc, grad_attn, level_hw, *ctx.dims)
        return (d_raw,) + (None,) * 8


def _ptr(t):
    return 0 if t is None else t.data_ptr()


_seed_counter = [0]
_seed_state: dict = {}
_seed_snap: dict = {}

# ... 424 lines not shown
```

### bevformer_b200/plugin/linear.py

```python
from __future__ import annotations

import os

import torch
import torch.nn.functional as F
from torch.autograd.function import Function, once_differentiable

from .. import ops
from ..arena import arena_of


def _use_tc(x: torch.Tensor, weight: torch.Tensor) -> bool:
    return (x.is_cuda and x.dtype in ops.TC_DTYPES and weight.shape[1] % 64 == 0
            and weight.shape[0] % 16 == 0 and os.environ.get("BEVF_GEMM", "tc") != "cublas")


def stacked_head(weights, biases, x):
    from ..arena import stacked
    n, k = sum(w.shape[0] for w in weights), weights[0].shape[1]
    direct = (x.is_cuda and x.dtype in ops.TC_DTYPES and k % 64 == 0 and n % 16 == 0
              and os.environ.get("BEVF_GEMM", "tc") != "cublas")
    return stacked(weights, direct), stacked(biases, direct)


# ... 198 lines not shown
            for l, o in enumerate(outs):
                o.register_hook(lambda g, l=l: (_SharedInputProjections.early(state, l, g), None)[1])
                o._bevf_early = (lambda g, l=l: _SharedInputProjections.early(state, l, g))
        for l, o in enumerate(outs):
            if state.get("ready"):
                o._bevf_ready = state["ready"][l]
        return outs
    return [linear(x, w, b) for w, b in weights_and_biases]


def linear_relu_dropout(x, weight, bias, p: float):
    if _use_tc(x, weight):
        return _LinearReluDropoutTC.apply(x, weight, bias, p)
    y = F.relu(F.linear(x, weight.to(x.dtype), None if bias is None else bias.to(x.dtype)), inplace=True)
    return F.dropout(y, p, training=p > 0.0)


def linear(x: torch.Tensor, weight: torch.Tensor, bias, relu: bool = False) -> torch.Tensor:
    if _use_tc(x, weight):
        return _LinearTC.apply(x, weight, bias, relu, False)
    y = F.linear(x, weight.to(x.dtype), None if bias is None else bias.to(x.dtype))
    return F.relu(y, inplace=True) if relu else y


def linear_fp32_out(x: torch.Tensor, weight: torch.Tensor, bias) -> torch.Tensor:
    if _use_tc(x, weight):
        return _LinearTC.apply(x, weight, bias, False, True)
    y = F.linear(x, weight.to(x.dtype), None if bias is None else bias.to(x.dtype))
    return y.float()


class _HeadTC(Function):
    @staticmethod
    def forward(ctx, x, weight, bias, kind, prep_args):
        w = weight.to(x.dtype)
        xc = x.contiguous()
        raw = ops.linear_tc(xc, w, bias, None, False, torch.float32).reshape(-1, w.shape[0])
        if kind == "sca":
            ref_cam, pair_q, pair_cam, pair_of, ss, bs, nq, m, l, p = prep_args
            loc, attn = ops.sca_prep_forward(raw, ref_cam, pair_q, pair_cam, ss, bs, nq, m, l, p)
        else:
            ref, ss, bs, nq, m, l, p, interleave = prep_args
            loc, attn = ops.tsa_prep_forward(raw, ref, ss, bs, nq, m, l, p, interleave)
        ctx.save_for_backward(xc, w, raw)
        ctx.kind, ctx.prep_args = kind, prep_args
        ctx.meta = (bias is not None, weight.dtype, None if bias is None else bias.dtype)
        ctx.arena = _arena_ctx(weight, bias)
        return loc, attn

    @staticmethod
    @once_differentiable
    def backward(ctx, grad_loc, grad_attn):
        x, w, raw = ctx.saved_tensors
        has_bias, wdt, bdt = ctx.meta
        k, n = w.shape[1], w.shape[0]
        grad_loc, grad_attn = grad_loc.contiguous(), grad_attn.contiguous()
        if ctx.kind == "sca":
            _ref_cam, pair_q, _pair_cam, pair_of, ss, bs, nq, m, l, p = ctx.prep_args
            d_raw = ops.sca_prep_backward(raw, grad_loc, grad_attn, pair_of, ss, bs, nq,
                                          pair_q.numel(), m, l, p, out_dtype=w.dtype)
        else:
            _ref, ss, bs, nq, m, l, p, interleave = ctx.prep_args
            d_raw = ops.tsa_prep_backward(raw, grad_loc, grad_attn, ss, bs, nq, m, l, p, interleave,
                                          out_dtype=w.dtype)
        dx = dw = db = None
        if ctx.needs_input_grad[0]:
            dx = ops.linear_dgrad_tc(d_raw, w).view(x.shape)
        if ctx.needs_input_grad[1]:
            dw, db = _wgrad(d_raw, x.reshape(-1, k), n, k, wdt, bdt if has_bias else None, ctx.arena)
        elif has_bias and ctx.needs_input_grad[2]:
            db = ops.colsum(d_raw).to(bdt)
        return dx, dw, db, None, None


def sca_sampling_head(x, weight, bias, ref_cam, pair_q, pair_cam, pair_of, ss, bs, nq, m, l, p):
    if _use_tc(x, weight):
        return _HeadTC.apply(x, weight, bias, "sca", (ref_cam, pair_q, pair_cam, pair_of, ss, bs, nq, m, l, p))
    raw = linear_fp32_out(x, weight, bias).reshape(bs * nq, -1)
    return ops.ScaPrep.apply(raw, ref_cam, pair_q, pair_cam, pair_of, ss, bs, nq, m, l, p)


def tsa_sampling_head(x, weight, bias, ref, ss, bs, nq, m, l, p, interleave=False):
    if _use_tc(x, weight):
        return _HeadTC.apply(x, weight, bias, "tsa", (ref, ss, bs, nq, m, l, p, bool(interleave)))
    raw = linear_fp32_out(x, weight, bias).reshape(bs * nq, -1)
    return ops.TsaPrep.apply(raw, ref, ss, bs, nq, m, l, p, interleave)
```

### bevformer_b200/plugin/spatial_cross_attention.py

```python
from __future__ import annotations

import os
from dataclasses import dataclass
from typing import Optional

import torch
import torch.nn as nn

from .. import ops, precision
from .linear import linear, sca_sampling_head, stacked_head
from .registry import ATTENTION, _register, build_attention
from .temporal_self_attention import _check_head_dim, ring_offsets_


@dataclass
class ScaPlan:
    pair_cam: torch.Tensor
    pair_q: torch.Tensor
    pair_of: torch.Tensor
    inv_count: torch.Tensor
    row_map: torch.Tensor
    ref_cam: torch.Tensor
    num_pairs: int
    counters: Optional[torch.Tensor] = None
    map_range: Optional[torch.Tensor] = None

    @staticmethod
    def build(bev_mask: torch.Tensor, reference_points_cam: torch.Tensor, bev_hw=None,
              tile: int = 8) -> "ScaPlan":
        ncam, bs, nq, _ = bev_mask.shape
        seen = bev_mask.any(-1)
        hit0 = seen[:, 0]
        nz = hit0.nonzero()
        r = int(nz.shape[0])
        if bev_hw is not None and tile > 1 and os.environ.get("BEVF_SCA_TILE", "1") != "0":
            h, w = bev_hw
            qi, qj = nz[:, 1] // w, nz[:, 1] % w
            tiles_x = (w + tile - 1) // tile
            key = ((nz[:, 0] * ((h + tile - 1) // tile) + qi // tile) * tiles_x + qj // tile) * (tile * tile) \
                + (qi % tile) * tile + qj % tile
            nz = nz[torch.argsort(key)]
        pair_cam = nz[:, 0].to(torch.int32).contiguous()
        pair_q = nz[:, 1].to(torch.int32).contiguous()
        pair_of = torch.full((ncam, nq), -1, dtype=torch.int32, device=bev_mask.device)
        pair_of[pair_cam.long(), pair_q.long()] = torch.arange(r, dtype=torch.int32, device=bev_mask.device)
        inv_count = 1.0 / seen.sum(0).clamp(min=1).to(torch.float32)
        row_map = (torch.arange(bs, device=bev_mask.device, dtype=torch.int32)[:, None] * ncam
                   + pair_cam[None, :]).reshape(-1).contiguous()
        per_cam = torch.bincount(pair_cam.long(), minlength=ncam)
        ends = per_cam.cumsum(0)
        rng = torch.stack([ends - per_cam, ends], 1)
        map_range = (rng[None] + (torch.arange(bs, device=rng.device) * r)[:, None, None]).reshape(-1, 2)
        return ScaPlan(pair_cam, pair_q, pair_of, inv_count.contiguous(), row_map,
                       reference_points_cam.float().contiguous(), r, None,
                       map_range.to(torch.int32).contiguous())


    @staticmethod
    def tile_order(bev_h: int, bev_w: int, device, tile: int = 8) -> torch.Tensor:
        qi = torch.arange(bev_h, device=device).view(bev_h, 1).expand(bev_h, bev_w).reshape(-1)
        qj = torch.arange(bev_w, device=device).view(1, bev_w).expand(bev_h, bev_w).reshape(-1)
        tiles_x = (bev_w + tile - 1) // tile
        key = ((qi // tile) * tiles_x + qj // tile) * (tile * tile) + (qi % tile) * tile + qj % tile
# ... 52 lines not shown
        if not self.batch_first:
            query, value = query.permute(1, 0, 2), value.permute(1, 0, 2)
        bs, nq, _ = query.shape
        nv = value.shape[1]
        m, l, p = self.num_heads, self.num_levels, self.num_points
        if reference_points.shape[-1] == 4:
            raise AssertionError("box-form reference points are not supported here")
        if reference_points.shape[-1] != 2:
            raise ValueError(f"Last dim of reference_points must be 2 or 4, "
                             f"but get {reference_points.shape[-1]} instead.")
        v = linear(value, self.value_proj.weight, self.value_proj.bias)
        if key_padding_mask is not None:
            v = v.masked_fill(key_padding_mask[..., None], 0.0)
        v = v.view(bs, nv, m, -1)
        w, b = self.head_weights(query)
        ss = torch.as_tensor(spatial_shapes).to(device=query.device, dtype=torch.int64)
        lsi = torch.as_tensor(level_start_index).to(device=query.device, dtype=torch.int64)
        d = reference_points.shape[2]
        dev = query.device
        ref = reference_points.reshape(1, bs, nq, d, 2).float().contiguous()
        pair_q = torch.arange(nq, device=dev, dtype=torch.int32)
        pair_cam = torch.zeros(nq, device=dev, dtype=torch.int32)
        pair_of = pair_q.view(1, nq).contiguous()
        loc, attn = sca_sampling_head(query, w, b, ref, pair_q, pair_cam, pair_of, ss.contiguous(),
                                      bs, nq, m, l, p)
        out = ops.MultiScaleDeformableAttnFunction_fp32.apply(
            v, ss, lsi, loc.view(bs, nq, m, l, p, 2), attn.view(bs, nq, m, l, p), self.im2col_step)
        return out if self.batch_first else out.permute(1, 0, 2)


class SpatialCrossAttention(nn.Module):

    def __init__(self, embed_dims=256, num_cams=6, pc_range=None, dropout=0.1, init_cfg=None,
                 batch_first=False,
                 deformable_attention=dict(type="MSDeformableAttention3D", embed_dims=256,
                                           num_levels=4),
                 **kwargs):
        super().__init__()
        self.init_cfg = init_cfg
        self.dropout = nn.Dropout(dropout)
        self.pc_range = pc_range
        self.fp16_enabled = False
        self.deformable_attention = build_attention(deformable_attention)
        self.embed_dims = embed_dims
        self.num_cams = num_cams
        self.output_proj = nn.Linear(embed_dims, embed_dims)
        self.batch_first = batch_first
        self.init_weight()

    def init_weight(self):
        nn.init.xavier_uniform_(self.output_proj.weight)
        nn.init.zeros_(self.output_proj.bias)

    def attend(self, query, value, reference_points_cam, bev_mask, spatial_shapes,
               level_start_index, plan: Optional[ScaPlan] = None, level_hw_host=None, value_pre=None):
        da = self.deformable_attention
        bs, nq, c = query.shape
        ncam, s = value.shape[0], value.shape[1]
        m, l, p = da.num_heads, da.num_levels, da.num_points
        if plan is None:
            plan = ScaPlan.build(bev_mask, reference_points_cam)
        d = plan.ref_cam.shape[3]
        ss = torch.as_tensor(spatial_shapes).to(device=query.device, dtype=torch.int64).contiguous()
        lsi = torch.as_tensor(level_start_index).to(device=query.device, dtype=torch.int64).contiguous()
        if int(s) <= 0 or p % d != 0:
            raise AssertionError("num_points must be a multiple of the pillar anchors")
        w, b = da.head_weights(query)
        loc, attn = sca_sampling_head(query, w, b, plan.ref_cam, plan.pair_q, plan.pair_cam,
                                      plan.pair_of, ss, bs, nq, m, l, p)
        if value_pre is None:
            feats = value.permute(2, 0, 1, 3).reshape(bs * ncam, s, c)
            value_pre = linear(feats, da.value_proj.weight, da.value_proj.bias)
        if getattr(value_pre, "_bevf_ready", None) is not None:
            torch.cuda.current_stream(value_pre.device).wait_event(value_pre._bevf_ready)
        v = value_pre.view(bs * ncam, s, m, -1)
        if hasattr(value_pre, "_bevf_early"):
            v._bevf_early = value_pre._bevf_early
        staged = None
        if level_hw_host is not None and plan.map_range is not None and len(level_hw_host) == l:
            staged = (level_hw_host, plan.map_range)
        gv_mode = None
        if level_hw_host is not None and len(level_hw_host) == l and v.dtype == torch.bfloat16:
            gv_mode = ops.gv_mode_for(plan.row_map.numel() / max(1, bs * ncam), p, level_hw_host)
        out = ops.SamplerRows.apply(v, loc, attn, plan.row_map, ss, lsi, None, staged, gv_mode)
        slots = ops.ScaCombine.apply(out, plan.pair_of, plan.pair_q, plan.inv_count, bs, nq)
        return linear(slots, self.output_proj.weight, self.output_proj.bias)

    @precision.entry("query", "key", "value", "residual", "query_pos")
    def forward(self, query, key, value, residual=None, query_pos=None, key_padding_mask=None,
                reference_points=None, spatial_shapes=None, reference_points_cam=None,
                bev_mask=None, level_start_index=None, flag="encoder", **kwargs):
        if key is None:
            key = query
        if value is None:
            value = key
        inp_residual = query if residual is None else residual
        if query_pos is not None:
            query = query + query_pos
        out = self.attend(query, value, reference_points_cam, bev_mask, spatial_shapes,
                          level_start_index, kwargs.get("sca_plan"))
        return self.dropout(out) + inp_residual


_register(ATTENTION, MSDeformableAttention3D)
_register(ATTENTION, SpatialCrossAttention)
```

### include/bevformer_b200.h

```cpp
#ifndef BEVFORMER_B200_H_
#define BEVFORMER_B200_H_

#include <stdint.h>

#ifdef __cplusplus
extern "C" {
#endif

#define BEVF_ABI_VERSION 1

#if defined(__GNUC__)
#define BEVF_API __attribute__((visibility("default")))
#else
#define BEVF_API
#endif

enum bevf_dtype { BEVF_DTYPE_F32 = 0, BEVF_DTYPE_BF16 = 1, BEVF_DTYPE_F16 = 2 };

BEVF_API int bevf_version(void);

BEVF_API const char *bevf_last_error(void);

BEVF_API int64_t bevf_launch_count(void);

// ... 54 lines not shown
                           int B, int S, int S_fine, int row_elems, void *stream);

BEVF_API int bevf_msda_fx_frac_bits(int64_t rows_per_map, int L, int P);
BEVF_API int bevf_msda_backward_fx(const void *value, int value_dtype, const int64_t *level_hw,
                                   const int64_t *level_start, const float *loc, const float *attn,
                                   const void *grad_out, int grad_out_dtype, int64_t *grad_value_fx, uint32_t *bounds,
                                   int frac_bits, float *grad_loc, float *grad_attn, int B, int S, int M, int D, int Q,
                                   int L, int P, void *stream);
BEVF_API int bevf_msda_rows_backward_fx(const void *value, int value_dtype, const int64_t *level_hw,
                                        const int64_t *level_start, const float *loc, const float *attn,
                                        const void *grad_out, int grad_out_dtype, int64_t *grad_value_fx,
                                        uint32_t *bounds, int frac_bits, float *grad_loc, float *grad_attn,
                                        const int32_t *row_map, int B, int S, int M, int D, int R, int L, int P,
                                        void *stream);
BEVF_API int bevf_msda_fx_convert(const int64_t *grad_value_fx, const uint32_t *bounds, int frac_bits, void *out,
                                  int out_dtype, int accumulate, int64_t n, void *stream);

BEVF_API int bevf_msda_rows_forward_staged(const void *value, int value_dtype, const int64_t *level_hw,
                                           const int64_t *level_start, const int32_t *level_hw_host,
                                           const float *loc, const float *attn, void *out, int out_dtype,
                                           const int32_t *map_range, int B, int S, int M, int D, int R,
                                           int L, int P, void *stream);

BEVF_API int bevf_msda_rows_backward_dense(const void *value, int value_dtype, const int64_t *level_hw,
                                           const int64_t *level_start, const int32_t *level_hw_host,
                                           const float *loc, const float *attn, const void *grad_out,
                                           int grad_out_dtype, float *grad_value, float *grad_loc,
                                           float *grad_attn, const int32_t *row_map, const int32_t *map_range,
                                           int B, int S, int M, int D, int R, int L, int P, void *stream);
BEVF_API int bevf_msda_set_dense_backward(int mode);
BEVF_API int bevf_msda_get_dense_backward(void);
BEVF_API int bevf_msda_dense_plan(const int32_t *level_hw_host, int L, int max_pix, int tiles, int32_t *bins_out,
                                  int bins_cap, uint32_t *level_mask);

BEVF_API int bevf_msda_set_backward_mode(int mode);


BEVF_API int64_t bevf_sca_plan_workspace_ints(int ncam, int Nq);
BEVF_API int bevf_sca_plan_build(const unsigned char *bev_mask, const int32_t *qorder, int32_t *pair_q,
                                 int32_t *pair_cam, int32_t *pair_of, int32_t *row_map, float *inv_count,
                                 int32_t *map_range, int32_t *counters, int32_t *workspace, int B, int ncam,
                                 int Nq, int D, int capacity, void *stream);

BEVF_API int bevf_sca_prep_forward(const float *raw, const float *ref_cam, const int32_t *pair_q,
                                   const int32_t *pair_cam, const int64_t *level_hw, float *loc,
                                   float *attn, int B, int Nq, int R, int M, int L, int P, int D,
                                   int ncam, void *stream);

BEVF_API int bevf_sca_prep_backward(const float *raw, const float *grad_loc, const float *grad_attn,
                                    const int32_t *pair_of, const int64_t *level_hw, void *d_raw,
                                    int out_dtype, int B, int Nq, int R, int M, int L, int P, int ncam,
                                    void *stream);

BEVF_API int bevf_tsa_prep_forward(const float *raw, const float *ref2d, const int64_t *level_hw,
                                   float *loc, float *attn, int B, int Nq, int M, int L, int P,
                                   int interleave, void *stream);

BEVF_API int bevf_tsa_prep_backward(const float *raw, const float *grad_loc, const float *grad_attn,
                                    const int64_t *level_hw, void *d_raw, int out_dtype, int B, int Nq,
                                    int M, int L, int P, int interleave, void *stream);

BEVF_API int bevf_layernorm_forward(const void *x, const void *residual, const void *gamma,
                                    const void *beta, int param_dtype, const void *pos, void *y,
                                    void *y_plus_pos, float *mean, float *rstd, int64_t rows, int C,
                                    float eps, float drop_p, uint64_t seed, const uint64_t *seed_base,
                                    int dtype, void *stream);

BEVF_API int bevf_layernorm_backward(const void *x, const void *residual, const void *gamma,
                                     int param_dtype, const float *mean, const float *rstd,
                                     const void *dy, const void *dy_plus_pos, int64_t dy_plus_pos_ld,
                                     void *dx, void *dres, float *dgamma, float *dbeta, int64_t rows,
                                     int C, float drop_p, uint64_t seed, const uint64_t *seed_base,
                                     int dtype, void *stream);

BEVF_API int64_t bevf_layernorm_backward_workspace_bytes(int64_t rows, int C);
BEVF_API int bevf_layernorm_backward_det(const void *x, const void *residual, const void *gamma,
                                         int param_dtype, const float *mean, const float *rstd,
                                         const void *dy, const void *dy_plus_pos, int64_t dy_plus_pos_ld,
                                         void *dx, void *dres, float *dgamma, float *dbeta, void *workspace,
                                         int64_t workspace_bytes, int64_t rows, int C, float drop_p, uint64_t seed,
                                         const uint64_t *seed_base, int dtype, void *stream);

BEVF_API int bevf_sca_combine_forward(const void *out, const int32_t *pair_of,
                                      const float *inv_count, void *slots, int B, int Nq, int R,
                                      int C, int ncam, int dtype, void *stream);

BEVF_API int bevf_sca_combine_backward(const void *g_slots, const int32_t *pair_q,
                                       const float *inv_count, void *g_out, int B, int Nq, int R,
                                       int C, int dtype, void *stream);

BEVF_API int bevf_flatten_feats(const void *feat, const float *cams_embeds, const float *level_embed,
                                void *out, int bs, int ncam, int C, int hw, int S, int level_start,
                                int dtype, void *stream);

BEVF_API int bevf_point_sampling(const float *lidar2img, const float *pc_range, const float *z_norm,
                                 float img_h, float img_w, float *ref_cam, uint8_t *bev_mask, int B,
                                 int ncam, int bev_h, int bev_w, int D, void *stream);

BEVF_API int bevf_linear_forward(const void *x, const void *w, const void *bias, int bias_dtype,
                                 const void *residual, void *y, int y_dtype, int64_t M, int N, int K,
                                 int relu, void *stream);

BEVF_API int bevf_linear_dgrad(const void *dy, const void *w, void *dx, int64_t M, int N, int K,
                               void *stream);

BEVF_API int bevf_linear_dgrad_acc(const void *dy, const void *w, const void *addend, void *dx, int64_t M,
// ... 46 lines not shown
```

Measured before the change: 1.693 million.

## Fuse SCA sampling-offset/softmax prep into the MSDA row kernels forward and backward

Computes the spatial cross-attention sampling locations and softmax attention weights inside the deformable-attention sampling kernels, straight from the raw projection output. This removes the separate prep kernel and the round trip of loc/attn tensors through global memory. In backward, queries seen by a single camera get their raw-head gradient written directly by the sampler. Only multi-camera queries still go through a reduced prep-backward kernel. The fused path adds per-row softmax statistics, coarse-level loc/attn buffers for the dense backward, and more shared memory and register pressure in the sampler kernels.

```diff
diff --git a/bevformer_b200/_lib.py b/bevformer_b200/_lib.py
--- a/bevformer_b200/_lib.py
+++ b/bevformer_b200/_lib.py
@@ -60,6 +60,12 @@
                                               c_void_p, c_int, c_void_p] + [c_int] * 7 + [c_void_p]),
     "bevf_sca_prep_forward": (c_int, [c_void_p] * 7 + [c_int] * 8 + [c_void_p]),
     "bevf_sca_prep_backward": (c_int, [c_void_p] * 6 + [c_int] * 8 + [c_void_p]),
+    "bevf_sca_rows_forward_fused": (c_int, [c_void_p, c_int] + [c_void_p] * 9 + [c_int, c_void_p, c_int, c_void_p]
+                                    + [c_int] * 12 + [c_void_p]),
+    "bevf_sca_rows_backward_fused": (c_int, [c_void_p, c_int] + [c_void_p] * 7 + [c_int] + [c_void_p] * 5
+                                     + [c_int, c_void_p, c_void_p, c_void_p, c_int, c_int] + [c_void_p] * 5
+                                     + [c_int] * 12 + [c_void_p]),
+    "bevf_sca_prep_backward_multi": (c_int, [c_void_p] * 6 + [c_int] * 8 + [c_void_p]),
     "bevf_tsa_prep_forward": (c_int, [c_void_p] * 5 + [c_int] * 6 + [c_void_p]),
     "bevf_tsa_prep_backward": (c_int, [c_void_p] * 5 + [c_int] * 7 + [c_void_p]),
     "bevf_layernorm_forward": (c_int, [c_void_p] * 4 + [c_int] + [c_void_p] * 5
diff --git a/bevformer_b200/csrc/common.cuh b/bevformer_b200/csrc/common.cuh
--- a/bevformer_b200/csrc/common.cuh
+++ b/bevformer_b200/csrc/common.cuh
@@ -55,6 +55,15 @@
 typedef __nv_bfloat16 bf16;
 
 __device__ __forceinline__ float exp_rn(float x) { return (float)exp((double)x); }
+
+__device__ __forceinline__ float quad_max(float v) {
+    v = fmaxf(v, __shfl_xor_sync(0xffffffffu, v, 1));
+    return fmaxf(v, __shfl_xor_sync(0xffffffffu, v, 2));
+}
+__device__ __forceinline__ float quad_sum(float v) {
+    v += __shfl_xor_sync(0xffffffffu, v, 1);
+    return v + __shfl_xor_sync(0xffffffffu, v, 2);
+}
 
 __device__ __forceinline__ float bf16_lo(uint32_t u) { return __uint_as_float(u << 16); }
 __device__ __forceinline__ float bf16_hi(uint32_t u) { return __uint_as_float(u & 0xffff0000u); }
diff --git a/bevformer_b200/csrc/encoder_ops.cu b/bevformer_b200/csrc/encoder_ops.cu
--- a/bevformer_b200/csrc/encoder_ops.cu
+++ b/bevformer_b200/csrc/encoder_ops.cu
@@ -109,14 +109,6 @@
 }
 
 
-__device__ __forceinline__ float quad_max(float v) {
-    v = fmaxf(v, __shfl_xor_sync(0xffffffffu, v, 1));
-    return fmaxf(v, __shfl_xor_sync(0xffffffffu, v, 2));
-}
-__device__ __forceinline__ float quad_sum(float v) {
-    v += __shfl_xor_sync(0xffffffffu, v, 1);
-    return v + __shfl_xor_sync(0xffffffffu, v, 2);
-}
 template <int N> __device__ __forceinline__ void ldv(const float *p, float (&v)[N]) {
     if constexpr (N % 4 == 0) {
 #pragma unroll
@@ -211,7 +203,7 @@
     stv<PPL>(attn + (t * M + m) * LP + k0, lg);
 }
 
-template <int PPL, typename TO>
+template <int PPL, typename TO, bool kMultiOnly = false>
 __global__ void __launch_bounds__(kEThreads)
 sca_prep_bwd_m8(const float *__restrict__ raw, const float *__restrict__ grad_loc,
                 const float *__restrict__ grad_attn, const int *__restrict__ pair_of,
@@ -225,6 +217,11 @@
     const long long bq = (long long)blockIdx.x * (kEThreads / 32) + (threadIdx.x >> 5);
     if (bq >= (long long)B * Nq) return;
     const int q = (int)(bq % Nq), b = (int)(bq / Nq);
+    if constexpr (kMultiOnly) {
+        int seen = 0;
+        for (int c = 0; c < ncam; ++c) seen += __ldg(pair_of + (long long)c * Nq + q) >= 0 ? 1 : 0;
+        if (seen == 1) return;
+    }
     const int LP = 4 * PPL, k0 = sub * PPL;
     const long long rbase = bq * (M * LP * 3);
     float a[PPL];
@@ -981,6 +978,34 @@
     return sca_prep_backward_t<float>(who, raw, grad_loc, grad_attn, pair_of, level_hw, (float *)d_raw, B, Nq, R, M, L, P, ncam, st);
 }
 
+template <typename TO>
+static void sca_prep_backward_multi_t(const float *raw, const float *grad_loc, const float *grad_attn,
+                                      const int32_t *pair_of, const int64_t *level_hw, TO *d_raw, int B, int Nq,
+                                      int R, int L, int P, int ncam, cudaStream_t st) {
+    const int pmagic = (65536 + P - 1) / P;
+    const unsigned wgrid = blocks_for((long long)B * Nq, kEThreads / 32);
+    sca_prep_bwd_m8<8, TO, true><<<wgrid, kEThreads, 0, st>>>(raw, grad_loc, grad_attn, pair_of, level_hw, d_raw, B,
+                                                              Nq, R, L, P, ncam, pmagic);
+}
+
+extern "C" int bevf_sca_prep_backward_multi(const float *raw, const float *grad_loc,
+                                            const float *grad_attn, const int32_t *pair_of,
+                                            const int64_t *level_hw, void *d_raw, int out_dtype, int B, int Nq,
+                                            int R, int M, int L, int P, int ncam, void *stream) {
+    const char *who = "bevf_sca_prep_backward_multi";
+    BEVF_REQUIRE(B >= 0 && Nq >= 0 && R >= 0 && L > 0 && P > 0 && ncam > 0 && ncam <= 16, who, "bad dimension (ncam <= 16)");
+    BEVF_REQUIRE(M == 8 && L * P == 32 && L <= 16, who, "8 heads and num_levels * num_points == 32 only");
+    BEVF_REQUIRE(out_dtype == BEVF_DTYPE_BF16 || out_dtype == BEVF_DTYPE_F16, who, "bf16 or fp16 d_raw only");
+    if ((long long)B * Nq == 0) return 0;
+    BEVF_REQUIRE(raw && pair_of && level_hw && d_raw && (R == 0 || (grad_loc && grad_attn)), who, "null pointer argument");
+    cudaStream_t st = (cudaStream_t)stream;
+    if (out_dtype == BEVF_DTYPE_BF16)
+        sca_prep_backward_multi_t<bf16>(raw, grad_loc, grad_attn, pair_of, level_hw, (bf16 *)d_raw, B, Nq, R, L, P, ncam, st);
+    else
+        sca_prep_backward_multi_t<__half>(raw, grad_loc, grad_attn, pair_of, level_hw, (__half *)d_raw, B, Nq, R, L, P, ncam, st);
+    return check_launch(who);
+}
+
 extern "C" int bevf_tsa_prep_forward(const float *raw, const float *ref2d, const int64_t *level_hw,
                                      float *loc, float *attn, int B, int Nq, int M, int L, int P,
                                      int interleave, void *stream) {
diff --git a/bevformer_b200/csrc/msda.cu b/bevformer_b200/csrc/msda.cu
--- a/bevformer_b200/csrc/msda.cu
+++ b/bevformer_b200/csrc/msda.cu
@@ -9,15 +9,17 @@
 
 namespace bevf {
 
-template <typename T, typename TO>
+template <typename T, typename TO, bool kFused = false>
 __global__ void __launch_bounds__(kThreads)
 msda_fwd_d32(const T *__restrict__ value, const int64_t *__restrict__ level_hw,
              const int64_t *__restrict__ level_start, const float *__restrict__ loc,
              const float *__restrict__ attn, TO *__restrict__ out,
              const int *__restrict__ row_map, int S, int M, int Q, int L, int P, int magic,
-             int iters, long long rows) {
+             int iters, long long rows, const __grid_constant__ ScaFuse fz = ScaFuse{}) {
     constexpr int VEC = Vec<T>::N, LANES = 32 / VEC, G = 32 / LANES;
+    static_assert(!kFused || LANES == 4, "the fused prep needs 4 lanes per row (16-bit value rows)");
     constexpr bool kHalf = std::is_same<T, bf16>::value;
+    __shared__ __align__(16) float s_fa[kFused ? kThreads / 32 * G : 1][kFuseLP];
     __shared__ LevelTab tab;
     load_level_tab(level_hw, level_start, L, M * 32, tab);
 
@@ -36,6 +38,18 @@
     const T *vbase = value + ((long long)b * S * M + m) * 32 + sub * VEC;
     const float2 *locp = reinterpret_cast<const float2 *>(loc) + row * LP;
     const float *attp = attn + row * LP;
+    ScaRow sr;
+    const int fgrp = warp * G + grp;
+    if constexpr (kFused) {
+        live = live && sca_row(fz, row, sr);
+        float fa[8];
+        const float2 st = sca_row_stats(sr, live, sub, fa);
+        if (live && sub == 0) fz.stats[row] = st;
+        __syncwarp();
+        *reinterpret_cast<float4 *>(&s_fa[fgrp][8 * sub]) = make_float4(fa[0], fa[1], fa[2], fa[3]);
+        *reinterpret_cast<float4 *>(&s_fa[fgrp][8 * sub + 4]) = make_float4(fa[4], fa[5], fa[6], fa[7]);
+        __syncwarp();
+    }
 
     float acc[VEC];
 #pragma unroll
@@ -48,8 +62,20 @@
         bool valid = false;
         if (sm < LP && live) {
             const int l = level_of(sm, magic);
-            const float2 xy = __ldg(locp + sm);
-            const float a = __ldg(attp + sm);
+            float2 xy;
+            float a;
+            if constexpr (kFused) {
+                sca_loc(sr, sm, l, P, fz.Dz, tab.h[l], tab.w[l], xy.x, xy.y);
+                a = s_fa[fgrp][sm];
+                if (l >= fz.coarse_from) {
+                    const long long ci = row * (LP - fz.coarse_from * P) + (sm - fz.coarse_from * P);
+                    fz.coarse_loc[ci] = xy;
+                    fz.coarse_attn[ci] = a;
+                }
+            } else {
+                xy = __ldg(locp + sm);
+                a = __ldg(attp + sm);
+            }
             const Corner c = make_corner(xy.x, xy.y, tab.h[l], tab.w[l]);
             enc = (c.pidx * pix) | c.dx | (c.dy << 1);
             valid = c.valid;
@@ -91,7 +117,7 @@
     }
 }
 
-template <typename T, typename TG, bool kScatter, typename TV = float>
+template <typename T, typename TG, bool kScatter, typename TV = float, bool kFused = false>
 __global__ void __launch_bounds__(kThreads)
 msda_bwd_d32(const T *__restrict__ value, const int64_t *__restrict__ level_hw,
              const int64_t *__restrict__ level_start, const float *__restrict__ loc,
@@ -101,9 +127,14 @@
              int L, int P, int magic, int iters, long long rows, unsigned red_skip,
              const __grid_constant__ HostLevels host_levels, const unsigned *__restrict__ gv_amax = nullptr,
              __half *__restrict__ gv16 = nullptr, unsigned gv16_mask = 0u, int side_start = 0, int S_side = 0,
-             const unsigned *__restrict__ fx_bounds = nullptr, int fx_bits = 0) {
+             const unsigned *__restrict__ fx_bounds = nullptr, int fx_bits = 0,
+             const __grid_constant__ ScaFuse fz = ScaFuse{}) {
     constexpr int VEC = Vec<T>::N, LANES = 32 / VEC, G = 32 / LANES;
     constexpr bool kHalfDot = std::is_same<T, bf16>::value && std::is_same<TG, bf16>::value;
+    static_assert(!kFused || (LANES == 4 && G == kFuseHeads), "the fused prep needs 16-bit value rows");
+    __shared__ float s_fa[kFused ? kThreads / 32 * G : 1][kFuseLP];
+    __shared__ float s_fg[kFused ? kThreads / 32 * G : 1][kFuseLP];
+    __shared__ __align__(16) uint32_t s_fo[kFused ? kThreads / 32 * G : 1][kFuseLP];
     __shared__ LevelTab tab;
     __shared__ unsigned s_skip;
     if (threadIdx.x == 0)
@@ -145,6 +176,19 @@
     const long long voff = ((long long)b * S * M + m) * 32 + sub * VEC;
     const float2 *locp = reinterpret_cast<const float2 *>(loc) + row * LP;
     const float *attp = attn + row * LP;
+    ScaRow sr;
+    float2 st = make_float2(0.f, 0.f);
+    bool single = false;
+    const int fgrp = (threadIdx.x >> 5) * G + grp;
+    if constexpr (kFused) {
+        live = live && sca_row(fz, row, sr);
+        if (live) {
+            st = __ldg(fz.stats + row);
+            int seen = 0;
+            for (int c = 0; c < fz.ncam; ++c) seen += __ldg(fz.pair_of + (long long)c * fz.Nq + sr.q) >= 0 ? 1 : 0;
+            single = seen == 1;
+        }
+    }
 
     float g[VEC];
     load_vec<TG, VEC>(grad_out + row * 32 + sub * VEC, g);
@@ -196,8 +240,14 @@
         if (mine) {
             const int l = level_of(sm, magic);
             Hm = tab.h[l]; Wm = tab.w[l];
-            const float2 xy = __ldg(locp + sm);
-            a = __ldg(attp + sm);
+            float2 xy;
+            if constexpr (kFused) {
+                sca_loc(sr, sm, l, P, fz.Dz, Hm, Wm, xy.x, xy.y);
+                a = sca_attn(sr, sm, st.x, st.y);
+            } else {
+                xy = __ldg(locp + sm);
+                a = __ldg(attp + sm);
+            }
             c = make_corner(xy.x, xy.y, Hm, Wm);
         }
         const int enc = (c.pidx * pix) | c.dx | (c.dy << 1);
@@ -320,9 +370,41 @@
             const float gx = a * (hy * (d01 - d00) + c.ly * (d11 - d10));
             const float gy = a * (hx * (d10 - d00) + c.lx * (d11 - d01));
             const long long si = row * LP + sm;
-            grad_attn[si] = ga;
-            reinterpret_cast<float2 *>(grad_loc)[si] = make_float2((float)Wm * gx, (float)Hm * gy);
-        }
+            const float glx = (float)Wm * gx, gly = (float)Hm * gy;
+            if (!kFused || !single) {
+                grad_attn[si] = ga;
+                reinterpret_cast<float2 *>(grad_loc)[si] = make_float2(glx, gly);
+            } else {
+                s_fa[fgrp][sm] = a;
+                s_fg[fgrp][sm] = 0.f + ga;
+                s_fo[fgrp][sm] = pack_bf16x2(__fdiv_rn(0.f + glx, (float)Wm), __fdiv_rn(0.f + gly, (float)Hm));
+            }
+        }
+    }
+    if constexpr (kFused) {
+        __syncwarp();
+        float fa[8], fg[8], dot = 0.f;
+        const bool fin = live && single;
+#pragma unroll
+        for (int i = 0; i < 8; ++i) {
+            fa[i] = fin ? s_fa[fgrp][8 * sub + i] : 0.f;
+            fg[i] = fin ? s_fg[fgrp][8 * sub + i] : 0.f;
+            dot += fa[i] * fg[i];
+        }
+        dot = quad_sum(dot);
+        if (fin) {
+            bf16 *dr = fz.d_raw + sr.raw_row * (kFuseHeads * kFuseLP * 3);
+#pragma unroll
+            for (int i = 0; i < 8; ++i) fg[i] = fa[i] * (fg[i] - dot);
+            *reinterpret_cast<uint4 *>(dr + kFuseHeads * kFuseLP * 2 + m * kFuseLP + 8 * sub) =
+                make_uint4(pack_bf16x2(fg[0], fg[1]), pack_bf16x2(fg[2], fg[3]), pack_bf16x2(fg[4], fg[5]),
+                           pack_bf16x2(fg[6], fg[7]));
+            const uint4 *so = reinterpret_cast<const uint4 *>(&s_fo[fgrp][8 * sub]);
+            uint4 *dof = reinterpret_cast<uint4 *>(dr + m * kFuseLP * 2 + 16 * sub);
+            dof[0] = so[0];
+            dof[1] = so[1];
+        }
+        __syncwarp();
     }
     }
 }
@@ -466,15 +548,27 @@
 template <typename T, typename TO>
 static int launch_fwd(const char *who, const void *value, const int64_t *hw, const int64_t *ls,
                       const float *loc, const float *attn, void *out, const int *row_map, int S,
-                      int M, int D, int Q, int L, int P, long long rows, cudaStream_t st) {
+                      int M, int D, int Q, int L, int P, long long rows, cudaStream_t st,
+                      const ScaFuse *fz = nullptr) {
     if (D == 32) {
         constexpr int G = Vec<T>::N;
         const int iters = pick_iters(rows, G);
         const long long per_block = (long long)(kThreads / 32) * G * iters;
         const unsigned grid = (unsigned)((rows + per_block - 1) / per_block);
-        msda_fwd_d32<T, TO><<<grid, kThreads, 0, st>>>((const T *)value, hw, ls, loc, attn, (TO *)out,
-                                                       row_map, S, M, Q, L, P, (65536 + P - 1) / P, iters,
-                                                       rows);
+        if (fz) {
+            if constexpr (std::is_same<T, bf16>::value && std::is_same<TO, bf16>::value)
+                msda_fwd_d32<T, TO, true><<<grid, kThreads, 0, st>>>((const T *)value, hw, ls, nullptr, nullptr, (TO *)out,
+                                                                     row_map, S, M, Q, L, P, (65536 + P - 1) / P, iters,
+                                                                     rows, *fz);
+            else
+                return fail("%s: the fused prep needs bf16 value and output", who);
+        } else {
+            msda_fwd_d32<T, TO><<<grid, kThreads, 0, st>>>((const T *)value, hw, ls, loc, attn, (TO *)out,
+                                                           row_map, S, M, Q, L, P, (65536 + P - 1) / P, iters,
+                                                           rows);
+        }
+    } else if (fz) {
+        return fail("%s: the fused prep needs head_dim 32", who);
     } else {
         const unsigned grid = (unsigned)((rows + kThreads / 32 - 1) / (kThreads / 32));
         msda_fwd_generic<T, TO><<<grid, kThreads, 0, st>>>((const T *)value, hw, ls, loc, attn,
@@ -506,7 +600,7 @@
                           const float *loc, const float *attn, const void *grad_out, float *grad_value,
                           const int32_t *map_range, int NB, int S, int M, int L, int P, cudaStream_t st,
                           unsigned *handled, HostLevels *host_levels, int first_level, unsigned need_mask,
-                          int gv_S, int gv_base);
+                          int gv_S, int gv_base, int loc_level0);
 
 static cudaStream_t g_side_stream = nullptr;
 constexpr int kSideEvents = 64;
@@ -568,7 +662,9 @@
                       float *ga, const int *row_map, const int *order, int S, int M, int D, int Q,
                       int L, int P, long long rows, cudaStream_t st, unsigned done_levels = 0,
                       const HostLevels *host_levels = nullptr, bool gv_f16 = false,
-                      const MixedGv *mixed = nullptr, const FxGv *fx = nullptr) {
+                      const MixedGv *mixed = nullptr, const FxGv *fx = nullptr, const ScaFuse *fz = nullptr) {
+    if (fz && (fx || gv_f16 || !mixed || !mixed->gv16))
+        return fail("%s: the fused prep runs with mixed grad_value accumulation only", who);
     HostLevels hl;
     if (host_levels) hl = *host_levels; else memset(&hl, 0, sizeof(hl));
     if (fx) {
@@ -612,6 +708,16 @@
             const int iters = pick_iters(rows, G);
             const long long per_block = (long long)(kThreads / 32) * G * iters;
             const unsigned grid = (unsigned)((rows + per_block - 1) / per_block);
+            if (fz) {
+                if constexpr (std::is_same<TG, bf16>::value)
+                    msda_bwd_d32<T, TG, true, float, true><<<grid, kThreads, 0, st>>>(
+                        (const T *)value, hw, ls, nullptr, nullptr, (const TG *)go, gv, gl, ga, row_map, S, M, Q, L, P,
+                        (65536 + P - 1) / P, iters, rows, done_levels, hl, mixed->amax, mixed->gv16, mixed->mask,
+                        mixed->side_start, mixed->S_side, nullptr, 0, *fz);
+                else
+                    return fail("%s: the fused prep needs a bf16 grad_out", who);
+                return check_launch(who);
+            }
             msda_bwd_d32<T, TG, true><<<grid, kThreads, 0, st>>>((const T *)value, hw, ls, loc, attn, (const TG *)go, gv, gl, ga,
                                                                row_map, S, M, Q, L, P, (65536 + P - 1) / P, iters, rows,
                                                                done_levels, hl, mixed->amax, mixed->gv16, mixed->mask, mixed->side_start,
@@ -669,15 +775,22 @@
 static int msda_forward_impl(const char *who, const void *value, int value_dtype,
                              const int64_t *level_hw, const int64_t *level_start, const float *loc,
                              const float *attn, void *out, int out_dtype, const int *row_map, int B,
-                             int S, int M, int D, int Q, int L, int P, void *stream) {
+                             int S, int M, int D, int Q, int L, int P, void *stream,
+                             const ScaFuse *fz = nullptr) {
     if (int e = check_dims(who, B, S, M, D, Q, L, P)) return e;
     const long long rows = (row_map ? 1ll : (long long)B) * Q * M;
     if (rows == 0) return 0;
-    if (!value || !level_hw || !level_start || !loc || !attn || !out)
+    if (!value || !level_hw || !level_start || ((!loc || !attn) && !fz) || !out)
         return fail("%s: null pointer argument", who);
     if (!aligned16(value) || !aligned16(loc) || !aligned16(attn) || !aligned16(out))
         return fail("%s: device pointers must be 16-byte aligned", who);
     cudaStream_t st = (cudaStream_t)stream;
+    if (fz) {
+        if (value_dtype != BEVF_DTYPE_BF16 || out_dtype != BEVF_DTYPE_BF16)
+            return fail("%s: the fused prep needs bf16 value and output", who);
+        return launch_fwd<bf16, bf16>(who, value, level_hw, level_start, nullptr, nullptr, out, row_map, S, M, D, Q, L, P,
+                                      rows, st, fz);
+    }
     if (value_dtype == BEVF_DTYPE_F16) {
         if (out_dtype == BEVF_DTYPE_F16) return launch_fwd<__half, __half>(who, value, level_hw, level_start, loc, attn, out, row_map, S, M, D, Q, L, P, rows, st);
         if (out_dtype == BEVF_DTYPE_F32) return launch_fwd<__half, float>(who, value, level_hw, level_start, loc, attn, out, row_map, S, M, D, Q, L, P, rows, st);
@@ -699,17 +812,25 @@
                               const int *row_map, const int *order, int B, int S, int M, int D, int Q,
                               int L, int P, void *stream, unsigned done_levels = 0,
                               const HostLevels *host_levels = nullptr, bool gv_f16 = false,
-                              const MixedGv *mixed = nullptr, const FxGv *fx = nullptr) {
+                              const MixedGv *mixed = nullptr, const FxGv *fx = nullptr,
+                              const ScaFuse *fz = nullptr) {
     if (int e = check_dims(who, B, S, M, D, Q, L, P)) return e;
     const long long rows = (row_map ? 1ll : (long long)B) * Q * M;
     if (rows == 0) return 0;
-    if (!value || !level_hw || !level_start || !loc || !attn || !grad_out || !grad_value ||
+    if (!value || !level_hw || !level_start || ((!loc || !attn) && !fz) || !grad_out || !grad_value ||
         !grad_loc || !grad_attn)
         return fail("%s: null pointer argument", who);
     if (!aligned16(value) || !aligned16(loc) || !aligned16(attn) || !aligned16(grad_out) ||
         !aligned16(grad_value) || !aligned16(grad_loc) || !aligned16(grad_attn))
         return fail("%s: device pointers must be 16-byte aligned", who);
     cudaStream_t st = (cudaStream_t)stream;
+    if (fz) {
+        if (value_dtype != BEVF_DTYPE_BF16 || grad_out_dtype != BEVF_DTYPE_BF16)
+            return fail("%s: the fused prep needs bf16 value and grad_out", who);
+        return launch_bwd<bf16, bf16>(who, value, level_hw, level_start, nullptr, nullptr, grad_out, grad_value, grad_loc,
+                                      grad_attn, row_map, order, S, M, D, Q, L, P, rows, st, done_levels, host_levels,
+                                      gv_f16, mixed, fx, fz);
+    }
     if (value_dtype == BEVF_DTYPE_F16) {
         if (grad_out_dtype == BEVF_DTYPE_F16) return launch_bwd<__half, __half>(who, value, level_hw, level_start, loc, attn, grad_out, grad_value, grad_loc, grad_attn, row_map, order, S, M, D, Q, L, P, rows, st, done_levels, host_levels, gv_f16, mixed, fx);
         if (grad_out_dtype == BEVF_DTYPE_F32) return launch_bwd<__half, float>(who, value, level_hw, level_start, loc, attn, grad_out, grad_value, grad_loc, grad_attn, row_map, order, S, M, D, Q, L, P, rows, st, done_levels, host_levels, gv_f16, mixed, fx);
@@ -844,7 +965,7 @@
             ds = g_side_stream;
         }
         const int e = dense_coarse_backward(who, level_hw, level_start, level_hw_host, loc, attn, grad_out, grad_value,
-                                            map_range, B, S, M, L, P, ds, &handled, &hl, 0, 0u, S, 0);
+                                            map_range, B, S, M, L, P, ds, &handled, &hl, 0, 0u, S, 0, 0);
         if (join) cudaEventRecord(join, g_side_stream);
         if (e) {
             if (join) cudaStreamWaitEvent(st, join, 0);
@@ -880,7 +1001,8 @@
                                     void *grad_value_fine_f16, float *grad_value_side, const uint32_t *amax_bits,
                                     int num_f16_levels, int first_dense_level, float *grad_loc, float *grad_attn,
                                     const int32_t *row_map, const int32_t *group_order, const int32_t *map_range,
-                                    int B, int S, int M, int D, int R, int L, int P, void *stream) {
+                                    int B, int S, int M, int D, int R, int L, int P, void *stream,
+                                    const ScaFuse *fz = nullptr) {
     if (!row_map && R > 0) return fail("%s: row_map is null", who);
     if (!level_hw_host || !grad_value_fine_f16 || !grad_value_side || !amax_bits)
         return fail("%s: null pointer argument", who);
@@ -911,8 +1033,11 @@
     unsigned dense_levels = 0;
     cudaEvent_t join = nullptr;
     const int mode = map_range ? mixed_dense_mode() : 0;
-    if (mode != 0 && R > 0 && grad_out_dtype == BEVF_DTYPE_BF16 && aligned16(loc) && aligned16(attn) &&
-        aligned16(grad_out)) {
+    const float *dloc = fz ? reinterpret_cast<const float *>(fz->coarse_loc) : loc;
+    const float *dattn = fz ? fz->coarse_attn : attn;
+    const int loc_level0 = fz ? fz->coarse_from : 0;
+    if (mode != 0 && R > 0 && grad_out_dtype == BEVF_DTYPE_BF16 && aligned16(dloc) && aligned16(dattn) &&
+        aligned16(grad_out) && dloc && dattn && loc_level0 <= first_dense_level) {
         cudaStream_t ds = st;
         if (mode == 2 && !g_side_stream) {
             cudaStreamCaptureStatus cs = cudaStreamCaptureStatusActive;
@@ -928,9 +1053,9 @@
         }
         const unsigned suffix = ((1u << L) - 1u) & ~((1u << first_dense_level) - 1u);
         HostLevels dhl;
-        const int e = dense_coarse_backward(who, level_hw, level_start, level_hw_host, loc, attn, grad_out,
+        const int e = dense_coarse_backward(who, level_hw, level_start, level_hw_host, dloc, dattn, grad_out,
                                             grad_value_side, map_range, B, S, M, L, P, ds, &dense_levels, &dhl,
-                                            first_dense_level, suffix, mx.S_side, mx.side_start);
+                                            first_dense_level, suffix, mx.S_side, mx.side_start, loc_level0);
         if (join) cudaEventRecord(join, g_side_stream);
         if (e) {
             if (join) cudaStreamWaitEvent(st, join, 0);
@@ -939,7 +1064,7 @@
     }
     const int e = msda_backward_impl(who, value, value_dtype, level_hw, level_start, loc, attn, grad_out, grad_out_dtype,
                                      grad_value_side, grad_loc, grad_attn, row_map, group_order, B, S, M, D, R, L, P,
-                                     stream, dense_levels, &hl, false, &mx);
+                                     stream, dense_levels, &hl, false, &mx, nullptr, fz);
     if (join) cudaStreamWaitEvent(st, join, 0);
     return e;
 }
@@ -971,6 +1096,78 @@
                                     grad_out_dtype, grad_value_fine_f16, grad_value_side, amax_bits, num_f16_levels,
                                     first_dense_level, grad_loc, grad_attn, row_map, nullptr, map_range, B, S, M, D, R,
                                     L, P, stream);
+}
+
+static int sca_fuse_args(const char *who, const float *raw, const float *ref_cam, const int32_t *pair_q,
+                         const int32_t *pair_cam, const int32_t *pair_of, const float *stats, const float *coarse_loc,
+                         const float *coarse_attn, int coarse_from, int M, int D, int R, int L, int P, int bs, int Nq,
+                         int pairs, int Dz, int ncam, ScaFuse &fz) {
+    if (M != kFuseHeads || D != 32 || L * P != kFuseLP)
+        return fail("%s: 8 heads, head_dim 32 and num_levels * num_points == 32 only", who);
+    if (bs <= 0 || Nq <= 0 || pairs < 0 || (long long)bs * pairs != R || Dz <= 0 || P % Dz != 0 || ncam <= 0 ||
+        ncam > 16)
+        return fail("%s: bad dimension (rows = bs * pairs, num_points a multiple of the Z anchors, ncam <= 16)", who);
+    if (!raw || !ref_cam || !pair_q || !pair_cam || !stats) return fail("%s: null pointer argument", who);
+    if (!aligned16(raw) || !aligned16(stats) || (reinterpret_cast<uintptr_t>(ref_cam) & 7u))
+        return fail("%s: raw and stats must be 16-byte aligned, ref_cam 8-byte aligned", who);
+    if (coarse_from < 0 || coarse_from > L || (coarse_from < L && (!coarse_loc || !coarse_attn)))
+        return fail("%s: coarse_from must be in [0, L], with coarse_loc / coarse_attn when below L", who);
+    if (!aligned16(coarse_loc) || !aligned16(coarse_attn))
+        return fail("%s: coarse_loc / coarse_attn must be 16-byte aligned", who);
+    fz.coarse_loc = const_cast<float2 *>(reinterpret_cast<const float2 *>(coarse_from < L ? coarse_loc : nullptr));
+    fz.coarse_attn = const_cast<float *>(coarse_from < L ? coarse_attn : nullptr);
+    fz.coarse_from = coarse_from;
+    fz.raw = raw;
+    fz.ref_cam = ref_cam;
+    fz.pair_q = pair_q;
+    fz.pair_cam = pair_cam;
+    fz.pair_of = pair_of;
+    fz.stats = const_cast<float2 *>(reinterpret_cast<const float2 *>(stats));
+    fz.d_raw = nullptr;
+    fz.bs = bs; fz.Nq = Nq; fz.R = pairs; fz.Dz = Dz; fz.ncam = ncam;
+    return 0;
+}
+
+extern "C" int bevf_sca_rows_forward_fused(const void *value, int value_dtype, const int64_t *level_hw,
+                                           const int64_t *level_start, const float *raw, const float *ref_cam,
+                                           const int32_t *pair_q, const int32_t *pair_cam, float *stats,
+                                           float *coarse_loc, float *coarse_attn, int coarse_from, void *out,
+                                           int out_dtype, const int32_t *row_map, int B, int S, int M, int D, int R,
+                                           int L, int P, int bs, int Nq, int pairs, int Dz, int ncam, void *stream) {
+    const char *who = "bevf_sca_rows_forward_fused";
+    if (!row_map && R > 0) return fail("%s: row_map is null", who);
+    if (R == 0) return 0;
+    ScaFuse fz;
+    if (int e = sca_fuse_args(who, raw, ref_cam, pair_q, pair_cam, nullptr, stats, coarse_loc, coarse_attn,
+                              coarse_from, M, D, R, L, P, bs, Nq, pairs, Dz, ncam, fz))
+        return e;
+    return msda_forward_impl(who, value, value_dtype, level_hw, level_start, nullptr, nullptr, out, out_dtype, row_map,
+                             B, S, M, D, R, L, P, stream, &fz);
+}
+
+extern "C" int bevf_sca_rows_backward_fused(const void *value, int value_dtype, const int64_t *level_hw,
+                                            const int64_t *level_start, const int32_t *level_hw_host, const float *raw,
+                                            const float *stats, const float *coarse_loc, const float *coarse_attn,
+                                            int coarse_from, const float *ref_cam, const int32_t *pair_q,
+                                            const int32_t *pair_cam, const int32_t *pair_of, const void *grad_out,
+                                            int grad_out_dtype, void *grad_value_fine_f16, float *grad_value_side,
+                                            const uint32_t *amax_bits, int num_f16_levels, int first_dense_level,
+                                            float *grad_loc, float *grad_attn, void *d_raw, const int32_t *row_map,
+                                            const int32_t *map_range, int B, int S, int M, int D, int R, int L, int P,
+                                            int bs, int Nq, int pairs, int Dz, int ncam, void *stream) {
+    const char *who = "bevf_sca_rows_backward_fused";
+    if (R == 0) return 0;
+    ScaFuse fz;
+    if (int e = sca_fuse_args(who, raw, ref_cam, pair_q, pair_cam, pair_of, stats, coarse_loc, coarse_attn,
+                              coarse_from, M, D, R, L, P, bs, Nq, pairs, Dz, ncam, fz))
+        return e;
+    if (!pair_of) return fail("%s: null pointer argument", who);
+    if (!d_raw || !aligned16(d_raw)) return fail("%s: d_raw must be a 16-byte aligned bf16 buffer", who);
+    fz.d_raw = reinterpret_cast<bf16 *>(d_raw);
+    return rows_backward_mixed_impl(who, value, value_dtype, level_hw, level_start, level_hw_host, nullptr, nullptr,
+                                    grad_out, grad_out_dtype, grad_value_fine_f16, grad_value_side, amax_bits,
+                                    num_f16_levels, map_range ? first_dense_level : L, grad_loc, grad_attn, row_map,
+                                    nullptr, map_range, B, S, M, D, R, L, P, stream, &fz);
 }
 
 namespace bevf {
diff --git a/bevformer_b200/csrc/msda_common.cuh b/bevformer_b200/csrc/msda_common.cuh
--- a/bevformer_b200/csrc/msda_common.cuh
+++ b/bevformer_b200/csrc/msda_common.cuh
@@ -175,6 +175,68 @@
 }
 
 
+struct ScaFuse {
+    const float *raw;
+    const float *ref_cam;
+    const int *pair_q, *pair_cam, *pair_of;
+    float2 *stats;
+    bf16 *d_raw;
+    float2 *coarse_loc;
+    float *coarse_attn;
+    int coarse_from;
+    int bs, Nq, R, Dz, ncam;
+};
+constexpr int kFuseHeads = 8, kFuseLP = 32;
+
+struct ScaRow {
+    const float *lg, *off;
+    const float2 *ref;
+    long long raw_row;
+    int q;
+};
+__device__ __forceinline__ bool sca_row(const ScaFuse &fz, long long row, ScaRow &sr) {
+    const long long t = row / kFuseHeads;
+    const int m = (int)(row - t * kFuseHeads);
+    const int b = (int)(t / fz.R), r = (int)(t - (long long)b * fz.R);
+    const int q = __ldg(fz.pair_q + r), cam = __ldg(fz.pair_cam + r);
+    if (q < 0) return false;
+    sr.q = q;
+    sr.raw_row = (long long)b * fz.Nq + q;
+    const float *rq = fz.raw + sr.raw_row * (kFuseHeads * kFuseLP * 3);
+    sr.off = rq + m * kFuseLP * 2;
+    sr.lg = rq + kFuseHeads * kFuseLP * 2 + m * kFuseLP;
+    sr.ref = reinterpret_cast<const float2 *>(fz.ref_cam) + (((long long)cam * fz.bs + b) * fz.Nq + q) * fz.Dz;
+    return true;
+}
+__device__ __forceinline__ void sca_loc(const ScaRow &sr, int k, int l, int P, int Dz, int H, int W, float &x,
+                                        float &y) {
+    const float2 o = __ldg(reinterpret_cast<const float2 *>(sr.off) + k);
+    const float2 rf = __ldg(sr.ref + (k - l * P) % Dz);
+    x = rf.x + __fdiv_rn(o.x, (float)W);
+    y = rf.y + __fdiv_rn(o.y, (float)H);
+}
+__device__ __forceinline__ float sca_attn(const ScaRow &sr, int k, float mx, float inv) {
+    return exp_rn(__ldg(sr.lg + k) - mx) * inv;
+}
+__device__ __forceinline__ float2 sca_row_stats(const ScaRow &sr, bool live, int sub, float (&a)[8]) {
+#pragma unroll
+    for (int i = 0; i < 8; i += 4) {
+        const float4 v = live ? __ldg(reinterpret_cast<const float4 *>(sr.lg + 8 * sub + i)) : make_float4(0.f, 0.f, 0.f, 0.f);
+        a[i] = v.x; a[i + 1] = v.y; a[i + 2] = v.z; a[i + 3] = v.w;
+    }
+    float mx = a[0];
+#pragma unroll
+    for (int i = 1; i < 8; ++i) mx = fmaxf(mx, a[i]);
+    mx = quad_max(mx);
+    float sum = 0.f;
+#pragma unroll
+    for (int i = 0; i < 8; ++i) { a[i] = exp_rn(a[i] - mx); sum += a[i]; }
+    const float inv = __frcp_rn(quad_sum(sum));
+#pragma unroll
+    for (int i = 0; i < 8; ++i) a[i] *= inv;
+    return make_float2(mx, inv);
+}
+
 template <typename T> __device__ __forceinline__ decltype(Vec<T>::v) vec_bits(const uint4 &u);
 template <> __device__ __forceinline__ uint4 vec_bits<bf16>(const uint4 &u) { return u; }
 template <> __device__ __forceinline__ float4 vec_bits<float>(const uint4 &u) {
diff --git a/bevformer_b200/csrc/msda_dense.cu b/bevformer_b200/csrc/msda_dense.cu
--- a/bevformer_b200/csrc/msda_dense.cu
+++ b/bevformer_b200/csrc/msda_dense.cu
@@ -107,7 +107,7 @@
                   const int64_t *__restrict__ level_start, const float *__restrict__ loc,
                   const float *__restrict__ attn, const bf16 *__restrict__ grad_out,
                   float *__restrict__ grad_value, const int *__restrict__ map_range, int NB, int gv_S, int gv_base,
-                  int M, int L, int chunk_rows, int dbg) {
+                  int M, int L, int chunk_rows, int dbg, int loc_level0) {
     static_assert(P == 4 || P == 8, "points per level: 4 or 8");
     static_assert(kTiles == 4, "accumulator tiles per bin: 2 per issuer warpgroup");
     static_assert(NT >= 1 && NT <= 3, "scatter teams");
@@ -215,7 +215,7 @@
                 for (int i = 0; i < kMaxPass; ++i) {
                     q[i].x = q[i].y = q[i].a = 0.f;
                     if (live && on[i]) {
-                        const long long e = (((long long)r * M + m) * L + lv[i]) * P + pt;
+                        const long long e = (((long long)r * M + m) * (L - loc_level0) + lv[i] - loc_level0) * P + pt;
                         const float2 xy = dn::ldg_f2(reinterpret_cast<const float2 *>(loc) + e);
                         q[i].x = xy.x; q[i].y = xy.y; q[i].a = dn::ldg_f1(attn + e);
                     }
@@ -462,7 +462,7 @@
                           const float *loc, const float *attn, const void *grad_out, float *grad_value,
                           const int32_t *map_range, int NB, int S, int M, int L, int P, cudaStream_t st,
                           unsigned *handled, HostLevels *host_levels, int first_level, unsigned need_mask,
-                          int gv_S, int gv_base) {
+                          int gv_S, int gv_base, int loc_level0) {
     *handled = 0;
     static const long max_pix = dense_env("BEVF_DENSE_MAXPIX", 8192);
     static const long tiles = dense_env("BEVF_DENSE_TILES", 4);
@@ -507,14 +507,14 @@
         }
         kern<<<(unsigned)sms, 128 * teams + 256, smem, st>>>(bins, hw_dev, ls_dev, loc, attn, (const bf16 *)grad_out,
                                                            grad_value, map_range, NB, gv_S, gv_base, M, L, (int)chunk,
-                                                           (int)dbg);
+                                                           (int)dbg, loc_level0);
         return check_launch(who);
     };
     int e;
+    if (teams < 1 || teams > 3) return fail("%s: BEVF_DENSE_TEAMS must be 1, 2 or 3", who);
     if (teams == 3) e = (P == 8) ? launch(msda_bwd_dense_tc<4, 8, 3>) : launch(msda_bwd_dense_tc<4, 4, 3>);
     else if (teams == 2) e = (P == 8) ? launch(msda_bwd_dense_tc<4, 8, 2>) : launch(msda_bwd_dense_tc<4, 4, 2>);
-    else if (teams == 1) e = (P == 8) ? launch(msda_bwd_dense_tc<4, 8, 1>) : launch(msda_bwd_dense_tc<4, 4, 1>);
-    else return fail("%s: BEVF_DENSE_TEAMS must be 1, 2 or 3", who);
+    else e = (P == 8) ? launch(msda_bwd_dense_tc<4, 8, 1>) : launch(msda_bwd_dense_tc<4, 4, 1>);
     if (e) return e;
     *handled = mask;
     *host_levels = bins.hl;
diff --git a/bevformer_b200/ops.py b/bevformer_b200/ops.py
--- a/bevformer_b200/ops.py
+++ b/bevformer_b200/ops.py
@@ -620,6 +620,80 @@
         d_raw = sca_prep_backward(raw, grad_loc.contiguous(), grad_attn.contiguous(), pair_of,
                                   level_hw, *ctx.dims)
         return (d_raw,) + (None,) * 10
+
+
+def sca_rows_forward_fused(value, spatial_shapes, level_start_index, raw, ref_cam, pair_q, pair_cam, row_map, bs, nq,
+                           coarse_from=None):
+    for t, n in ((value, "value"), (raw, "raw"), (ref_cam, "ref_cam"), (pair_q, "pair_q"), (pair_cam, "pair_cam"),
+                 (row_map, "row_map")):
+        _need_cuda(t, n)
+    NB, S, M, D = value.shape
+    L = int(torch.as_tensor(spatial_shapes).shape[0])
+    P = raw.shape[1] // (3 * M * L)
+    R = row_map.numel()
+    ss, ls = _level_tensors(value, spatial_shapes, level_start_index)
+    out = torch.empty((R, M * D), device=value.device, dtype=value.dtype)
+    stats = torch.empty((R * M, 2), device=value.device, dtype=torch.float32)
+    coarse = None
+    if coarse_from is not None and 0 <= coarse_from < L:
+        nl = L - coarse_from
+        coarse = (torch.empty((R, M, nl, P, 2), device=value.device, dtype=torch.float32),
+                  torch.empty((R, M, nl, P), device=value.device, dtype=torch.float32), int(coarse_from))
+    lib = _lib.load()
+    with torch.cuda.device(value.device), _timed("msda_rows_forward", value.device, (R, L)):
+        st = lib.bevf_sca_rows_forward_fused(value.data_ptr(), _DT[value.dtype], ss.data_ptr(), ls.data_ptr(),
+                                             raw.data_ptr(), ref_cam.data_ptr(), pair_q.data_ptr(), pair_cam.data_ptr(),
+                                             stats.data_ptr(), _ptr(coarse and coarse[0]), _ptr(coarse and coarse[1]),
+                                             L if coarse is None else coarse[2], out.data_ptr(), _DT[value.dtype],
+                                             row_map.data_ptr(), NB, S, M, D, R, L, P, bs, nq, pair_q.numel(),
+                                             ref_cam.shape[3], ref_cam.shape[0], _stream_ptr(value))
+    _lib.check(st, lib)
+    return out, stats, coarse
+
+
+def sca_rows_backward_fused(value, spatial_shapes, level_start_index, level_hw_host, num_f16_levels, raw, stats,
+                            ref_cam, pair_q, pair_cam, pair_of, row_map, grad_output, bs, nq, map_range=None,
+                            first_dense_level=None, coarse=None):
+    import ctypes
+    for t, n in ((value, "value"), (raw, "raw"), (stats, "stats"), (ref_cam, "ref_cam"), (pair_of, "pair_of"),
+                 (row_map, "row_map"), (grad_output, "grad_output")):
+        _need_cuda(t, n)
+    alert_not_deterministic("sca_rows_backward_fused (grad_value summed with fp16 / fp32 atomics)")
+    NB, S, M, D = value.shape
+    L = len(level_hw_host)
+    P = raw.shape[1] // (3 * M * L)
+    R = row_map.numel()
+    if not (1 <= num_f16_levels < L):
+        raise RuntimeError("fused SCA backward: num_f16_levels does not fit the pyramid")
+    ss, ls = _level_tensors(value, spatial_shapes, level_start_index)
+    s_fine = sum(int(h) * int(w) for h, w in level_hw_host[:num_f16_levels])
+    grad_output = grad_output.contiguous()
+    grad_loc = torch.empty((R, M, L, P, 2), device=value.device, dtype=torch.float32)
+    grad_attn = torch.empty((R, M, L, P), device=value.device, dtype=torch.float32)
+    d_raw = torch.empty(raw.shape, device=value.device, dtype=torch.bfloat16)
+    hw = (ctypes.c_int32 * (2 * L))(*[int(v) for hw_ in level_hw_host for v in hw_])
+    lib = _lib.load()
+    with torch.cuda.device(value.device), _timed("msda_rows_backward", value.device, (R, L)):
+        amax = abs_max_bits(grad_output)
+        fine = torch.zeros((NB, s_fine, M, D), device=value.device, dtype=torch.float16)
+        side = torch.zeros((NB, S - s_fine, M, D), device=value.device, dtype=torch.float32)
+        kd = num_f16_levels if first_dense_level is None else int(first_dense_level)
+        st = lib.bevf_sca_rows_backward_fused(value.data_ptr(), _DT[value.dtype], ss.data_ptr(), ls.data_ptr(),
+                                              ctypes.addressof(hw), raw.data_ptr(), stats.data_ptr(),
+                                              _ptr(coarse and coarse[0]), _ptr(coarse and coarse[1]),
+                                              L if coarse is None else coarse[2], ref_cam.data_ptr(),
+                                              pair_q.data_ptr(), pair_cam.data_ptr(), pair_of.data_ptr(),
+                                              grad_output.data_ptr(), _DT[grad_output.dtype], fine.data_ptr(),
+                                              side.data_ptr(), amax.data_ptr(), int(num_f16_levels), kd,
+                                              grad_loc.data_ptr(), grad_attn.data_ptr(), d_raw.data_ptr(),
+                                              row_map.data_ptr(), _ptr(map_range), NB, S, M, D, R, L, P, bs, nq,
+                                              pair_q.numel(), ref_cam.shape[3], ref_cam.shape[0], _stream_ptr(value))
+        _lib.check(st, lib)
+    st = lib.bevf_sca_prep_backward_multi(raw.data_ptr(), grad_loc.data_ptr(), grad_attn.data_ptr(), pair_of.data_ptr(),
+                                          ss.data_ptr(), d_raw.data_ptr(), BF16, bs, nq, pair_q.numel(), M, L, P,
+                                          pair_of.shape[0], _stream_ptr(value))
+    _lib.check(st, lib)
+    return LazyGradValue(value.shape, fine, side, amax), d_raw
 
 
 def tsa_prep_forward(raw, ref2d, level_hw, B, Nq, M, L, P, interleave=False):
diff --git a/bevformer_b200/plugin/linear.py b/bevformer_b200/plugin/linear.py
--- a/bevformer_b200/plugin/linear.py
+++ b/bevformer_b200/plugin/linear.py
@@ -274,8 +274,6 @@
     @once_differentiable
     def backward(ctx, grad_loc, grad_attn):
         x, w, raw = ctx.saved_tensors
-        has_bias, wdt, bdt = ctx.meta
-        k, n = w.shape[1], w.shape[0]
         grad_loc, grad_attn = grad_loc.contiguous(), grad_attn.contiguous()
         if ctx.kind == "sca":
             _ref_cam, pair_q, _pair_cam, pair_of, ss, bs, nq, m, l, p = ctx.prep_args
@@ -285,14 +283,60 @@
             _ref, ss, bs, nq, m, l, p, interleave = ctx.prep_args
             d_raw = ops.tsa_prep_backward(raw, grad_loc, grad_attn, ss, bs, nq, m, l, p, interleave,
                                           out_dtype=w.dtype)
-        dx = dw = db = None
-        if ctx.needs_input_grad[0]:
-            dx = ops.linear_dgrad_tc(d_raw, w).view(x.shape)
-        if ctx.needs_input_grad[1]:
-            dw, db = _wgrad(d_raw, x.reshape(-1, k), n, k, wdt, bdt if has_bias else None, ctx.arena)
-        elif has_bias and ctx.needs_input_grad[2]:
-            db = ops.colsum(d_raw).to(bdt)
-        return dx, dw, db, None, None
+        return (*_head_grads(ctx, d_raw, x, w), None, None)
+
+
+def _head_grads(ctx, d_raw, x, w):
+    has_bias, wdt, bdt = ctx.meta
+    k, n = w.shape[1], w.shape[0]
+    dx = dw = db = None
+    if ctx.needs_input_grad[0]:
+        dx = ops.linear_dgrad_tc(d_raw, w).view(x.shape)
+    if ctx.needs_input_grad[1]:
+        dw, db = _wgrad(d_raw, x.reshape(-1, k), n, k, wdt, bdt if has_bias else None, ctx.arena)
+    elif has_bias and ctx.needs_input_grad[2]:
+        db = ops.colsum(d_raw).to(bdt)
+    return dx, dw, db
+
+
+class _ScaHeadSamplerTC(Function):
+
+    @staticmethod
+    def forward(ctx, x, weight, bias, value, fuse):
+        ref_cam, pair_q, pair_cam, _pair_of, row_map, ss, lsi, bs, nq, hw_host, nfine, map_range = fuse
+        w = weight.to(x.dtype)
+        xc = x.contiguous()
+        raw = ops.linear_tc(xc, w, bias, None, False, torch.float32).reshape(-1, w.shape[0])
+        kd = None
+        if any(ctx.needs_input_grad) and map_range is not None and ops._lib.load().bevf_msda_get_dense_backward():
+            kd = ops.dense_levels_for(row_map.numel() / max(1, value.shape[0]), raw.shape[1] // (3 * 8 * len(hw_host)),
+                                      hw_host)
+            kd = None if kd is None else max(kd, nfine)
+        out, stats, coarse = ops.sca_rows_forward_fused(value, ss, lsi, raw, ref_cam, pair_q, pair_cam, row_map, bs,
+                                                        nq, coarse_from=kd)
+        ctx.save_for_backward(xc, w, raw, stats, value)
+        ctx.fuse, ctx.coarse = fuse, coarse
+        ctx.meta = (bias is not None, weight.dtype, None if bias is None else bias.dtype)
+        ctx.arena = _arena_ctx(weight, bias)
+        ctx.value_early = getattr(value, "_bevf_early", None)
+        return out
+
+    @staticmethod
+    @once_differentiable
+    def backward(ctx, grad_out):
+        x, w, raw, stats, value = ctx.saved_tensors
+        ref_cam, pair_q, pair_cam, pair_of, row_map, ss, lsi, bs, nq, hw_host, nfine, map_range = ctx.fuse
+        coarse = ctx.coarse
+        dense = coarse is not None and ops._lib.load().bevf_msda_get_dense_backward()
+        gv, d_raw = ops.sca_rows_backward_fused(value, ss, lsi, hw_host, nfine, raw, stats, ref_cam, pair_q, pair_cam,
+                                                pair_of, row_map, grad_out, bs, nq,
+                                                map_range=map_range if dense else None,
+                                                first_dense_level=coarse[2] if dense else None, coarse=coarse)
+        ctx.coarse = None
+        gvalue = None
+        if ctx.needs_input_grad[3] and not (ctx.value_early is not None and ctx.value_early(gv)):
+            gvalue = gv.materialize()
+        return (*_head_grads(ctx, d_raw, x, w), gvalue, None)
 
 
 def sca_sampling_head(x, weight, bias, ref_cam, pair_q, pair_cam, pair_of, ss, bs, nq, m, l, p):
@@ -302,6 +346,10 @@
     return ops.ScaPrep.apply(raw, ref_cam, pair_q, pair_cam, pair_of, ss, bs, nq, m, l, p)
 
 
+def sca_head_sampler(x, weight, bias, value, fuse):
+    return _ScaHeadSamplerTC.apply(x, weight, bias, value, fuse)
+
+
 def tsa_sampling_head(x, weight, bias, ref, ss, bs, nq, m, l, p, interleave=False):
     if _use_tc(x, weight):
         return _HeadTC.apply(x, weight, bias, "tsa", (ref, ss, bs, nq, m, l, p, bool(interleave)))
diff --git a/bevformer_b200/plugin/spatial_cross_attention.py b/bevformer_b200/plugin/spatial_cross_attention.py
--- a/bevformer_b200/plugin/spatial_cross_attention.py
+++ b/bevformer_b200/plugin/spatial_cross_attention.py
@@ -8,7 +8,7 @@
 import torch.nn as nn
 
 from .. import ops, precision
-from .linear import linear, sca_sampling_head, stacked_head
+from .linear import _use_tc as use_tc, linear, sca_head_sampler, sca_sampling_head, stacked_head
 from .registry import ATTENTION, _register, build_attention
 from .temporal_self_attention import _check_head_dim, ring_offsets_
 
@@ -167,6 +167,14 @@
         nn.init.xavier_uniform_(self.output_proj.weight)
         nn.init.zeros_(self.output_proj.bias)
 
+    def _fused_prep(self, query, w, v, gv_mode, staged) -> bool:
+        da = self.deformable_attention
+        return (isinstance(gv_mode, tuple) and staged is not None and not ops.deterministic()
+                and da.num_heads == 8 and v.shape[-1] == 32 and da.num_levels * da.num_points == 32
+                and use_tc(query, w) and sum(h * w_ for h, w_ in gv_mode[1]) == v.shape[1]
+                and os.environ.get("BEVF_MSDA_FWD", "plain") != "staged"
+                and os.environ.get("BEVF_AUX_FILL", "0") != "1")
+
     def attend(self, query, value, reference_points_cam, bev_mask, spatial_shapes,
                level_start_index, plan: Optional[ScaPlan] = None, level_hw_host=None, value_pre=None):
         da = self.deformable_attention
@@ -181,8 +189,6 @@
         if int(s) <= 0 or p % d != 0:
             raise AssertionError("num_points must be a multiple of the pillar anchors")
         w, b = da.head_weights(query)
-        loc, attn = sca_sampling_head(query, w, b, plan.ref_cam, plan.pair_q, plan.pair_cam,
-                                      plan.pair_of, ss, bs, nq, m, l, p)
         if value_pre is None:
             feats = value.permute(2, 0, 1, 3).reshape(bs * ncam, s, c)
             value_pre = linear(feats, da.value_proj.weight, da.value_proj.bias)
@@ -197,7 +203,14 @@
         gv_mode = None
         if level_hw_host is not None and len(level_hw_host) == l and v.dtype == torch.bfloat16:
             gv_mode = ops.gv_mode_for(plan.row_map.numel() / max(1, bs * ncam), p, level_hw_host)
-        out = ops.SamplerRows.apply(v, loc, attn, plan.row_map, ss, lsi, None, staged, gv_mode)
+        if self._fused_prep(query, w, v, gv_mode, staged):
+            fuse = (plan.ref_cam, plan.pair_q, plan.pair_cam, plan.pair_of, plan.row_map, ss, lsi, bs, nq,
+                    gv_mode[1], gv_mode[2], plan.map_range)
+            out = sca_head_sampler(query, w, b, v, fuse)
+        else:
+            loc, attn = sca_sampling_head(query, w, b, plan.ref_cam, plan.pair_q, plan.pair_cam,
+                                          plan.pair_of, ss, bs, nq, m, l, p)
+            out = ops.SamplerRows.apply(v, loc, attn, plan.row_map, ss, lsi, None, staged, gv_mode)
         slots = ops.ScaCombine.apply(out, plan.pair_of, plan.pair_q, plan.inv_count, bs, nq)
         return linear(slots, self.output_proj.weight, self.output_proj.bias)
 
diff --git a/include/bevformer_b200.h b/include/bevformer_b200.h
--- a/include/bevformer_b200.h
+++ b/include/bevformer_b200.h
@@ -130,6 +130,29 @@
                                     int out_dtype, int B, int Nq, int R, int M, int L, int P, int ncam,
                                     void *stream);
 
+BEVF_API int bevf_sca_rows_forward_fused(const void *value, int value_dtype, const int64_t *level_hw,
+                                         const int64_t *level_start, const float *raw, const float *ref_cam,
+                                         const int32_t *pair_q, const int32_t *pair_cam, float *stats,
+                                         float *coarse_loc, float *coarse_attn, int coarse_from, void *out,
+                                         int out_dtype, const int32_t *row_map, int B, int S, int M, int D, int R,
+                                         int L, int P, int bs, int Nq, int pairs, int Dz, int ncam, void *stream);
+
+BEVF_API int bevf_sca_rows_backward_fused(const void *value, int value_dtype, const int64_t *level_hw,
+                                          const int64_t *level_start, const int32_t *level_hw_host, const float *raw,
+                                          const float *stats, const float *coarse_loc, const float *coarse_attn,
+                                          int coarse_from, const float *ref_cam, const int32_t *pair_q,
+                                          const int32_t *pair_cam, const int32_t *pair_of, const void *grad_out,
+                                          int grad_out_dtype, void *grad_value_fine_f16, float *grad_value_side,
+                                          const uint32_t *amax_bits, int num_f16_levels, int first_dense_level,
+                                          float *grad_loc, float *grad_attn, void *d_raw, const int32_t *row_map,
+                                          const int32_t *map_range, int B, int S, int M, int D, int R, int L, int P,
+                                          int bs, int Nq, int pairs, int Dz, int ncam, void *stream);
+
+BEVF_API int bevf_sca_prep_backward_multi(const float *raw, const float *grad_loc, const float *grad_attn,
+                                          const int32_t *pair_of, const int64_t *level_hw, void *d_raw,
+                                          int out_dtype, int B, int Nq, int R, int M, int L, int P, int ncam,
+                                          void *stream);
+
 BEVF_API int bevf_tsa_prep_forward(const float *raw, const float *ref2d, const int64_t *level_hw,
                                    float *loc, float *attn, int B, int Nq, int M, int L, int P,
                                    int interleave, void *stream);
```

New measurement: 1.751 million (median of 6 runs). 1.03x the previous value.
